# osmr/pytorchcv

Hardware: AMD Instinct MI355X
Metric: images/sec @224x224 (resnet50 bs=256/GPU) (higher is better)
Workload: dtype bf16; 1 GPU; resnet50_bs256; per_gpu_batch=256, global_batch=256, input=fp32 NCHW 224x224 resident in HBM, parallelism=batch-sharded replicas x1, launcher_choice=timed at capture on this GPU

## Files before the change

include/pcv_amd.h:

```cpp
#ifndef PCV_AMD_H
#define PCV_AMD_H

#include <stddef.h>
#include <stdint.h>

#ifdef __cplusplus
extern "C" {
#endif

#define PCV_ABI_VERSION 5

typedef struct pcv_ctx pcv_ctx;

typedef enum pcv_status {
    PCV_OK = 0,
    PCV_ERR_INVALID = -1,
    PCV_ERR_HIP = -2,
    PCV_ERR_NO_DEVICE = -3,
    PCV_ERR_TOO_LARGE = -4
} pcv_status;

typedef enum pcv_dtype { PCV_F32 = 0, PCV_BF16 = 1, PCV_F16 = 2 } pcv_dtype;

typedef enum pcv_act {
    PCV_ACT_NONE = 0, PCV_ACT_RELU = 1, PCV_ACT_RELU6 = 2, PCV_ACT_SIGMOID = 3,
    PCV_ACT_SWISH = 4, PCV_ACT_HSIGMOID = 5, PCV_ACT_HSWISH = 6
} pcv_act;

typedef struct pcv_conv_desc {
    int32_t struct_size;
    int32_t N, H, W;
    int32_t Cin, Cout;
    int32_t kh, kw;
    int32_t stride_h, stride_w;
    int32_t pad_t, pad_l, pad_b, pad_r;
    int32_t dil_h, dil_w;
    int32_t groups;
    int32_t act;
    int32_t post_act;
    int32_t has_residual;
    int32_t dtype;
    int32_t out_dtype;
    int32_t x_cpitch;
    int32_t x_wpitch;
    int32_t y_cpitch;
} pcv_conv_desc;

int pcv_abi_version(void);
size_t pcv_conv_desc_size(void);
int pcv_create(pcv_ctx** out, int device);
int pcv_destroy(pcv_ctx* ctx);
const char* pcv_last_error(const pcv_ctx* ctx);
int pcv_set_tuning(pcv_ctx* ctx, const char* key, int value);

int pcv_fp16_guard_begin(pcv_ctx* ctx, unsigned* slot, void* stream);
int pcv_fp16_guard_end(pcv_ctx* ctx, const unsigned* slot, float* y, long count, void* stream);
int pcv_fp16_overflow_count(pcv_ctx* ctx, unsigned* count, void* stream);

int pcv_nchw_to_nhwc(pcv_ctx* ctx, const float* x, void* y, int N, int C, int H, int W,
                     int cpitch, int wpitch, int dtype, void* stream);
int pcv_nhwc_to_nchw(pcv_ctx* ctx, const void* x, float* y, int N, int C, int H, int W, int cpitch, int dtype,
                     void* stream);

int pcv_preprocess_u8(pcv_ctx* ctx, const unsigned char* x, void* y, int N, int Hs, int Ws, int C, int top, int left,
                      int H, int W, int wpitch, const float* mean, const float* inv_std, int dtype, void* stream);

int pcv_resize_plan_bytes(int N, const int* hs, const int* ws, int C, int size, int H, int W, size_t* bytes);
int pcv_resize_plan(const void* const* frames, int N, const int* hs, const int* ws, int C, int size, int H, int W, void* blob,
                    size_t bytes);
int pcv_resize_crop_u8(pcv_ctx* ctx, const void* plan_host, const void* plan_dev, size_t bytes, void* y, int wpitch,
                       const float* mean, const float* inv_std, int dtype, void* stream);

int pcv_classify_f32(pcv_ctx* ctx, const float* logits, int N, int J, int k,
                     int* top_idx, float* top_val, float* top_prob,
                     const long long* labels, int* rank, float* nll,
                     void* stream);

int pcv_conv_packed_bytes(const pcv_conv_desc* d, size_t* bytes);
int pcv_conv_pack(pcv_ctx* ctx, const pcv_conv_desc* d, const float* w, void* packed, void* stream);
int pcv_dwconv_packed_bytes(const pcv_conv_desc* d, size_t* bytes);
int pcv_dwconv_pack(pcv_ctx* ctx, const pcv_conv_desc* d, const float* w, void* packed, void* stream);
int pcv_bn_fold(pcv_ctx* ctx, int C, const float* gamma, const float* beta, const float* mean, const float* var,
                float eps, const float* conv_bias, float* scale, float* shift, void* stream);

int pcv_conv2d_fused(pcv_ctx* ctx, const pcv_conv_desc* d, const void* x, const void* packed,
                     const float* scale, const float* shift, const void* residual, void* y, void* stream);

int pcv_conv2d_gated_fused(pcv_ctx* ctx, const pcv_conv_desc* d, const void* x, const void* packed, const float* scale,
                           const float* shift, const float* gate, const void* residual, void* y, void* stream);
int pcv_fc_f32(pcv_ctx* ctx, const float* in, const float* w, const float* b, float* out, int N, int K, int J, int act,
               void* stream);
int pcv_conv2d_maxpool_supported(const pcv_conv_desc* d, int k, int s, int p, int ceil_mode);
int pcv_conv2d_maxpool_fused(pcv_ctx* ctx, const pcv_conv_desc* d, const void* x, const void* packed, const float* scale,
                             const float* shift, void* y, int k, int s, int p, int ceil_mode, void* stream);

int pcv_conv2d_nchw_stem_supported(const pcv_conv_desc* d, int pool);
int pcv_conv2d_nchw_stem_fused(pcv_ctx* ctx, const pcv_conv_desc* d, const float* x_nchw, const void* packed, const float* scale,
                               const float* shift, void* y, int pool, void* stream);
int pcv_dwconv2d_fused(pcv_ctx* ctx, const pcv_conv_desc* d, const void* x, const void* packed,
                       const float* scale, const float* shift, const void* residual, void* y, void* stream);
int pcv_maxpool2d(pcv_ctx* ctx, const void* x, void* y, int N, int H, int W, int C, int k, int s, int p,
                  int ceil_mode, int dtype, void* stream);
int pcv_channel_slice(pcv_ctx* ctx, const void* x, void* y, long rows, int C, int offset, int x_cpitch, int y_cpitch,
                      int dtype, void* stream);
int pcv_channel_interleave2(pcv_ctx* ctx, const void* a, const void* b, void* y, long rows, int Ch, int a_cpitch,
                            int b_cpitch, int y_cpitch, int dtype, void* stream);
int pcv_channel_concat(pcv_ctx* ctx, const void* x, void* y, long rows, int C, int x_cpitch, int y_cpitch, int y_offset,
                       int dtype, void* stream);
int pcv_interpolate(pcv_ctx* ctx, const void* x, void* y, int N, int H, int W, int C, int Ho, int Wo, int bilinear,
                    int align_corners, int dtype, void* stream);
int pcv_avgpool2d(pcv_ctx* ctx, const void* x, void* y, int N, int H, int W, int C, int k, int s,
                  int dtype, int out_dtype, void* stream);
int pcv_global_avgpool(pcv_ctx* ctx, const void* x, void* y, int N, int HW, int C, int dtype, int out_dtype,
                       void* stream);
int pcv_gemm_bias(pcv_ctx* ctx, const void* x, const void* packed, const float* bias, void* y,
                  int N, int Cin, int Cout, int dtype, int out_dtype, void* stream);
int pcv_se_squeeze(pcv_ctx* ctx, const void* x, float* mean, int N, int HW, int C, int dtype, void* stream);
int pcv_se_excite(pcv_ctx* ctx, const float* mean, const float* w1, const float* b1, const float* w2,
                  const float* b2, float* mid, float* gate, int N, int C, int M, int mid_act, int out_act,
                  void* stream);
int pcv_se_scale(pcv_ctx* ctx, const void* x, const float* gate, const void* residual, void* y,
                 int N, int HW, int C, int post_act, int dtype, void* stream);

int pcv_splat_squeeze(pcv_ctx* ctx, const void* x, float* s, int N, int HW, int C, int radix, int dtype, void* stream);
int pcv_splat_excite(pcv_ctx* ctx, const float* s, const float* w1, const float* b1, const float* w2, const float* b2, float* mid,
                     float* logits, float* att, int N, int C, int M, int radix, int groups, void* stream);
int pcv_splat_combine(pcv_ctx* ctx, const void* x, const float* att, const void* residual, void* y, int N, int HW, int C, int radix,
                      int post_act, int dtype, void* stream);
int pcv_avgpool2d_pad(pcv_ctx* ctx, const void* x, void* y, int N, int H, int W, int C, int k, int s, int p, int ceil_mode,
                      int count_include_pad, int dtype, int out_dtype, void* stream);

int pcv_cbam_pool(pcv_ctx* ctx, const void* x, float* s, int N, int HW, int C, int dtype, void* stream);
int pcv_cbam_excite(pcv_ctx* ctx, const float* s, const float* w1, const float* b1, const float* w2, const float* b2, float* mid,
                    float* gate, int N, int C, int M, void* stream);
int pcv_cbam_spatial_pool(pcv_ctx* ctx, const void* x, const float* gate, float* p, int N, int HW, int C, int dtype, void* stream);
int pcv_cbam_apply(pcv_ctx* ctx, const void* x, const float* gate, const float* p, const float* w7, const float* scale,
                   const float* shift, const void* residual, void* y, int N, int H, int W, int C, int post_act, int dtype,
                   void* stream);

int pcv_conv1x1_pair_supported(const pcv_conv_desc* d1, const pcv_conv_desc* d2);
int pcv_conv1x1_pair_fused(pcv_ctx* ctx, const pcv_conv_desc* d1, const pcv_conv_desc* d2, const void* x,
                           const void* packed1, const float* scale1, const float* shift1, const void* residual, void* y1,
                           const void* packed2, const float* scale2, const float* shift2, void* y2, void* stream);

int pcv_conv1x1_pair_gated_supported(const pcv_conv_desc* d1, const pcv_conv_desc* d2);
int pcv_conv1x1_pair_gated_fused(pcv_ctx* ctx, const pcv_conv_desc* d1, const pcv_conv_desc* d2, const void* x,
                                 const void* packed1, const float* scale1, const float* shift1, const float* gate,
                                 const void* residual, void* y1, const void* packed2, const float* scale2, const float* shift2,
                                 void* y2, void* stream);

int pcv_conv1x1_pair_idconv_supported(const pcv_conv_desc* d_id, const pcv_conv_desc* d1, const pcv_conv_desc* d2);
int pcv_conv1x1_pair_idconv_fused(pcv_ctx* ctx, const pcv_conv_desc* d_id, const pcv_conv_desc* d1, const pcv_conv_desc* d2,
                                  const void* x0, const void* packed_id, const float* scale_id, const float* shift_id,
                                  const void* x, const void* packed1, const float* scale1, const float* shift1, void* y1,
                                  const void* packed2, const float* scale2, const float* shift2, void* y2, void* stream);

int pcv_mbconv_supported(const pcv_conv_desc* d_exp, const pcv_conv_desc* d_dw, const pcv_conv_desc* d_proj);
int pcv_mbconv_fused(pcv_ctx* ctx, const pcv_conv_desc* d_exp, const pcv_conv_desc* d_dw, const pcv_conv_desc* d_proj,
                     const void* x, const void* packed_exp, const float* scale_e, const float* shift_e,
                     const void* packed_dw, const float* scale_d, const float* shift_d, const void* packed_proj,
                     const float* scale_p, const float* shift_p, const void* residual, void* y, void* stream);

int pcv_bn_act(pcv_ctx* ctx, const void* x, const float* scale, const float* shift, void* y, long rows, int C,
               int x_cpitch, int act, int dtype, void* stream);

int pcv_rccl_available(void);
int pcv_rccl_broadcast(pcv_ctx* ctx, void* comm, void* const* bufs, const size_t* bytes, int count, int root, void* stream);
int pcv_rccl_allgather(pcv_ctx* ctx, void* comm, const void* send, void* recv, size_t bytes_per_rank, void* stream);

#ifdef __cplusplus
}
#endif
#endif
```

pytorchcv_amd/_lib.py:

```python

__all__ = ['lib', 'ctx_for', 'check', 'ConvDesc', 'LIB_PATH', 'PcvError', 'PCV_ERR_TOO_LARGE']

import os
import ctypes
import threading

LIB_PATH = os.path.join(os.path.dirname(os.path.abspath(__file__)), "csrc", "libpcv_amd.so")
PCV_ERR_TOO_LARGE = -4

_c = ctypes
_VP = ctypes.c_void_p
_I = ctypes.c_int


class PcvError(RuntimeError):
    def __init__(self, code, msg):
        super(PcvError, self).__init__("pcv_amd error {}: {}".format(code, msg))
        self.code = code


PCV_ABI_VERSION = 5


class ConvDesc(ctypes.Structure):
    _fields_ = [(n, ctypes.c_int32) for n in (
        "struct_size", "N", "H", "W", "Cin", "Cout", "kh", "kw", "stride_h", "stride_w", "pad_t", "pad_l", "pad_b", "pad_r",
        "dil_h", "dil_w", "groups", "act", "post_act", "has_residual", "dtype", "out_dtype", "x_cpitch", "x_wpitch",
        "y_cpitch")]


    def __init__(self, *args, **kw):
        super(ConvDesc, self).__init__(*args, **kw)
        self.struct_size = ctypes.sizeof(ConvDesc)


_SIGS = {
    "pcv_abi_version": (_I, []),
    "pcv_conv_desc_size": (ctypes.c_size_t, []),
    "pcv_create": (_I, [ctypes.POINTER(_VP), _I]),
    "pcv_destroy": (_I, [_VP]),
    "pcv_last_error": (ctypes.c_char_p, [_VP]),
    "pcv_set_tuning": (_I, [_VP, ctypes.c_char_p, _I]),
    "pcv_fp16_guard_begin": (_I, [_VP, _VP, _VP]),
    "pcv_fp16_guard_end": (_I, [_VP, _VP, _VP, ctypes.c_long, _VP]),
    "pcv_fp16_overflow_count": (_I, [_VP, ctypes.POINTER(ctypes.c_uint), _VP]),
    "pcv_rccl_available": (_I, []),
    "pcv_rccl_broadcast": (_I, [_VP, _VP, ctypes.POINTER(_VP), ctypes.POINTER(ctypes.c_size_t), _I, _I, _VP]),
    "pcv_rccl_allgather": (_I, [_VP, _VP, _VP, _VP, ctypes.c_size_t, _VP]),
    "pcv_nchw_to_nhwc": (_I, [_VP, _VP, _VP, _I, _I, _I, _I, _I, _I, _I, _VP]),
    "pcv_nhwc_to_nchw": (_I, [_VP, _VP, _VP, _I, _I, _I, _I, _I, _I, _VP]),
    "pcv_preprocess_u8": (_I, [_VP, _VP, _VP, _I, _I, _I, _I, _I, _I, _I, _I, _I, _VP, _VP, _I, _VP]),
    "pcv_resize_plan_bytes": (_I, [_I, ctypes.POINTER(_I), ctypes.POINTER(_I), _I, _I, _I, _I, ctypes.POINTER(ctypes.c_size_t)]),
    "pcv_resize_plan": (_I, [ctypes.POINTER(_VP), _I, ctypes.POINTER(_I), ctypes.POINTER(_I), _I, _I, _I, _I, _VP, ctypes.c_size_t]),
    "pcv_resize_crop_u8": (_I, [_VP, _VP, _VP, ctypes.c_size_t, _VP, _I, _VP, _VP, _I, _VP]),
    "pcv_classify_f32": (_I, [_VP, _VP, _I, _I, _I, _VP, _VP, _VP, _VP, _VP, _VP, _VP]),
    "pcv_conv_packed_bytes": (_I, [ctypes.POINTER(ConvDesc), ctypes.POINTER(ctypes.c_size_t)]),
    "pcv_conv_pack": (_I, [_VP, ctypes.POINTER(ConvDesc), _VP, _VP, _VP]),
    "pcv_dwconv_packed_bytes": (_I, [ctypes.POINTER(ConvDesc), ctypes.POINTER(ctypes.c_size_t)]),
    "pcv_dwconv_pack": (_I, [_VP, ctypes.POINTER(ConvDesc), _VP, _VP, _VP]),
    "pcv_bn_fold": (_I, [_VP, _I, _VP, _VP, _VP, _VP, ctypes.c_float, _VP, _VP, _VP, _VP]),
    "pcv_conv2d_fused": (_I, [_VP, ctypes.POINTER(ConvDesc), _VP, _VP, _VP, _VP, _VP, _VP, _VP]),
    "pcv_dwconv2d_fused": (_I, [_VP, ctypes.POINTER(ConvDesc), _VP, _VP, _VP, _VP, _VP, _VP, _VP]),
    "pcv_maxpool2d": (_I, [_VP, _VP, _VP, _I, _I, _I, _I, _I, _I, _I, _I, _I, _VP]),
    "pcv_channel_slice": (_I, [_VP, _VP, _VP, ctypes.c_long, _I, _I, _I, _I, _I, _VP]),
    "pcv_channel_interleave2": (_I, [_VP, _VP, _VP, _VP, ctypes.c_long, _I, _I, _I, _I, _I, _VP]),
    "pcv_channel_concat": (_I, [_VP, _VP, _VP, ctypes.c_long, _I, _I, _I, _I, _I, _VP]),
    "pcv_interpolate": (_I, [_VP, _VP, _VP, _I, _I, _I, _I, _I, _I, _I, _I, _I, _VP]),
    "pcv_avgpool2d": (_I, [_VP, _VP, _VP, _I, _I, _I, _I, _I, _I, _I, _I, _VP]),
    "pcv_global_avgpool": (_I, [_VP, _VP, _VP, _I, _I, _I, _I, _I, _VP]),
    "pcv_gemm_bias": (_I, [_VP, _VP, _VP, _VP, _VP, _I, _I, _I, _I, _I, _VP]),
    "pcv_se_squeeze": (_I, [_VP, _VP, _VP, _I, _I, _I, _I, _VP]),
    "pcv_se_excite": (_I, [_VP, _VP, _VP, _VP, _VP, _VP, _VP, _VP, _I, _I, _I, _I, _I, _VP]),
    "pcv_conv2d_gated_fused": (_I, [_VP, ctypes.POINTER(ConvDesc), _VP, _VP, _VP, _VP, _VP, _VP, _VP, _VP]),
    "pcv_fc_f32": (_I, [_VP, _VP, _VP, _VP, _VP, _I, _I, _I, _I, _VP]),
    "pcv_conv2d_maxpool_supported": (_I, [ctypes.POINTER(ConvDesc), _I, _I, _I, _I]),
    "pcv_conv2d_maxpool_fused": (_I, [_VP, ctypes.POINTER(ConvDesc), _VP, _VP, _VP, _VP, _VP, _I, _I, _I, _I, _VP]),
    "pcv_conv2d_nchw_stem_supported": (_I, [ctypes.POINTER(ConvDesc), _I]),
    "pcv_conv2d_nchw_stem_fused": (_I, [_VP, ctypes.POINTER(ConvDesc), _VP, _VP, _VP, _VP, _VP, _I, _VP]),
    "pcv_conv1x1_pair_supported": (_I, [ctypes.POINTER(ConvDesc), ctypes.POINTER(ConvDesc)]),
    "pcv_conv1x1_pair_fused": (_I, [_VP, ctypes.POINTER(ConvDesc), ctypes.POINTER(ConvDesc), _VP, _VP, _VP, _VP, _VP, _VP, _VP,
                                    _VP, _VP, _VP, _VP]),
    "pcv_conv1x1_pair_gated_supported": (_I, [ctypes.POINTER(ConvDesc), ctypes.POINTER(ConvDesc)]),
    "pcv_conv1x1_pair_gated_fused": (_I, [_VP, ctypes.POINTER(ConvDesc), ctypes.POINTER(ConvDesc), _VP, _VP, _VP, _VP, _VP, _VP, _VP,
                                          _VP, _VP, _VP, _VP, _VP]),
    "pcv_conv1x1_pair_idconv_supported": (_I, [ctypes.POINTER(ConvDesc), ctypes.POINTER(ConvDesc), ctypes.POINTER(ConvDesc)]),
    "pcv_conv1x1_pair_idconv_fused": (_I, [_VP, ctypes.POINTER(ConvDesc), ctypes.POINTER(ConvDesc), ctypes.POINTER(ConvDesc),
                                           _VP, _VP, _VP, _VP, _VP, _VP, _VP, _VP, _VP, _VP, _VP, _VP, _VP, _VP]),
    "pcv_mbconv_supported": (_I, [ctypes.POINTER(ConvDesc), ctypes.POINTER(ConvDesc), ctypes.POINTER(ConvDesc)]),
    "pcv_mbconv_fused": (_I, [_VP, ctypes.POINTER(ConvDesc), ctypes.POINTER(ConvDesc), ctypes.POINTER(ConvDesc), _VP, _VP, _VP, _VP,
                              _VP, _VP, _VP, _VP, _VP, _VP, _VP, _VP, _VP]),
    "pcv_bn_act": (_I, [_VP, _VP, _VP, _VP, _VP, ctypes.c_long, _I, _I, _I, _I, _VP]),
    "pcv_se_scale": (_I, [_VP, _VP, _VP, _VP, _VP, _I, _I, _I, _I, _I, _VP]),
    "pcv_splat_squeeze": (_I, [_VP, _VP, _VP, _I, _I, _I, _I, _I, _VP]),
    "pcv_splat_excite": (_I, [_VP, _VP, _VP, _VP, _VP, _VP, _VP, _VP, _VP, _I, _I, _I, _I, _I, _VP]),
    "pcv_splat_combine": (_I, [_VP, _VP, _VP, _VP, _VP, _I, _I, _I, _I, _I, _I, _VP]),
    "pcv_avgpool2d_pad": (_I, [_VP, _VP, _VP, _I, _I, _I, _I, _I, _I, _I, _I, _I, _I, _I, _VP]),
    "pcv_cbam_pool": (_I, [_VP, _VP, _VP, _I, _I, _I, _I, _VP]),
    "pcv_cbam_excite": (_I, [_VP, _VP, _VP, _VP, _VP, _VP, _VP, _VP, _I, _I, _I, _VP]),
    "pcv_cbam_spatial_pool": (_I, [_VP, _VP, _VP, _VP, _I, _I, _I, _I, _VP]),
    "pcv_cbam_apply": (_I, [_VP, _VP, _VP, _VP, _VP, _VP, _VP, _VP, _VP, _I, _I, _I, _I, _I, _I, _VP]),
}

_lib = None
_ctxs = {}
_lock = threading.RLock()


def lib():
    global _lib
    if _lib is None:
        with _lock:
            if _lib is None:
                if not os.path.exists(LIB_PATH):
                    raise RuntimeError(
                        "pytorchcv_amd: HIP extension {} is missing - build it with `python -c 'import __graft_entry__ as g; "
                        "g.build()'` or `make -C pytorchcv_amd/csrc`. There is no CPU fallback.".format(LIB_PATH))
                L = ctypes.CDLL(LIB_PATH)
                for name, (res, args) in _SIGS.items():
                    fn = getattr(L, name)
                    fn.restype = res
                    fn.argtypes = args
                if L.pcv_abi_version() != PCV_ABI_VERSION or L.pcv_conv_desc_size() != ctypes.sizeof(ConvDesc):
                    raise RuntimeError("pytorchcv_amd: {} has ABI version {} / a {}-byte pcv_conv_desc, this binding expects "
                                       "version {} / {} bytes - rebuild the library".format(
                                           LIB_PATH, L.pcv_abi_version(), L.pcv_conv_desc_size(), PCV_ABI_VERSION,
                                           ctypes.sizeof(ConvDesc)))
                _lib = L
    return _lib


def exported_symbols():
    return sorted(_SIGS.keys())


def ctx_for(device_index: int):
    c = _ctxs.get(device_index)
    if c is None:
        with _lock:
            c = _ctxs.get(device_index)
            if c is None:
                L = lib()
                h = _VP()
                rc = L.pcv_create(ctypes.byref(h), int(device_index))
                if rc != 0:
                    raise PcvError(rc, (L.pcv_last_error(None) or b"").decode())
                c = h
                _ctxs[device_index] = c
    return c


def check(rc: int, ctx):
    if rc != 0:
        raise PcvError(rc, (lib().pcv_last_error(ctx) or b"").decode())
```

pytorchcv_amd/csrc/pair1x1.hpp:

```cpp
#pragma once
#include "pcv_common.hpp"
#include <type_traits>
#include "igemm_conv.hpp"

struct PairParams {
    const void* x;
    const void* w1;
    const void* res;
    void* y1;
    const void* w2;
    void* y2;
    const float* scale1;
    const float* shift1;
    const float* scale2;
    const float* shift2;
    uint32_t x_bytes, res_bytes, y1_bytes, y2_bytes, w1_bytes, w2_bytes;
    int M, nTiles;
    int act1, post1, act2;
    const void* x0;
    const void* wid;
    const float* scale_id;
    const float* shift_id;
    uint32_t x0_bytes, wid_bytes;
    const float* gate;
    FastDiv div_hw;
    uint32_t* ovf;
};

template <int N> __device__ __forceinline__ void pair_wait_vmcnt() {
    asm volatile("s_waitcnt vmcnt(%0)" ::"n"(N) : "memory");
}

template <int DT, int PB, bool IDC = false, bool GATE = false>
__global__ __launch_bounds__(256, PB == 4 ? 1 : 2) void pair1x1_kernel(const PairParams p) {
#if defined(__HIP_DEVICE_COMPILE__)
    constexpr int K1 = 64, C1 = 256, C2 = 64, P = 16 * PB;
    constexpr int NXQ = PB / 2;
    constexpr int NIP = PB / 2;
    constexpr int XB = P * K1 * 2;
    typedef typename Mma<DT>::frag frag;
    extern __shared__ __attribute__((aligned(16))) char smem[];
    char* const x0ring = smem + 3 * XB;
    char* const red = smem + (IDC ? 6 : 3) * XB;

    const int tid = threadIdx.x;
    const int lane = tid & 63;
    const int wave = __builtin_amdgcn_readfirstlane(tid >> 6);
    const int fr = lane & 15, fq = lane >> 4;

    int tile = blockIdx.x;
    const int tstride = gridDim.x;
    if (tile >= p.nTiles) return;

    const __amdgpu_buffer_rsrc_t xrsrc = __builtin_amdgcn_make_buffer_rsrc(const_cast<void*>(p.x), 0, p.x_bytes, 0x00020000);
    const __amdgpu_buffer_rsrc_t rrsrc = __builtin_amdgcn_make_buffer_rsrc(const_cast<void*>(p.res), 0, p.res_bytes, 0x00020000);
    const __amdgpu_buffer_rsrc_t y1rsrc = __builtin_amdgcn_make_buffer_rsrc(p.y1, 0, p.y1_bytes, 0x00020000);
    const __amdgpu_buffer_rsrc_t y2rsrc = __builtin_amdgcn_make_buffer_rsrc(p.y2, 0, p.y2_bytes, 0x00020000);
    const __amdgpu_buffer_rsrc_t w1rsrc = __builtin_amdgcn_make_buffer_rsrc(const_cast<void*>(p.w1), 0, p.w1_bytes, 0x00020000);
    const __amdgpu_buffer_rsrc_t w2rsrc = __builtin_amdgcn_make_buffer_rsrc(const_cast<void*>(p.w2), 0, p.w2_bytes, 0x00020000);
    const __amdgpu_buffer_rsrc_t x0rsrc = __builtin_amdgcn_make_buffer_rsrc(const_cast<void*>(IDC ? p.x0 : p.x), 0, IDC ? p.x0_bytes : p.x_bytes, 0x00020000);
    const __amdgpu_buffer_rsrc_t widrsrc = __builtin_amdgcn_make_buffer_rsrc(const_cast<void*>(IDC ? p.wid : p.w1), 0, IDC ? p.wid_bytes : p.w1_bytes, 0x00020000);

    frag a1[4][2];
    frag a2[4][2];
#pragma unroll
    for (int i = 0; i < 4; ++i)
#pragma unroll
        for (int ks = 0; ks < 2; ++ks) {
            const u32x4 v1 = __builtin_amdgcn_raw_buffer_load_b128(
                w1rsrc, (uint32_t)(((64 * wave + 16 * i + fr) * K1 + ks * 32 + 8 * fq) * 2), 0, 0);
            const u32x4 v2 = __builtin_amdgcn_raw_buffer_load_b128(
                w2rsrc, (uint32_t)(((16 * i + fr) * C1 + (2 * wave + ks) * 32 + 8 * fq) * 2), 0, 0);
            a1[i][ks] = __builtin_bit_cast(frag, v1);
            a2[i][ks] = __builtin_bit_cast(frag, v2);
        }
    frag aid[IDC ? 4 : 1][2];
    if constexpr (IDC) {
#pragma unroll
        for (int i = 0; i < 4; ++i)
#pragma unroll
            for (int ks = 0; ks < 2; ++ks)
                aid[i][ks] = __builtin_bit_cast(frag, __builtin_amdgcn_raw_buffer_load_b128(
                    widrsrc, (uint32_t)(((64 * wave + 16 * i + fr) * K1 + ks * 32 + 8 * fq) * 2), 0, 0));
    }
    float sc1[2][8], sf1[2][8], sc2[NIP][8], sf2[NIP][8];
    float* const tscid = reinterpret_cast<float*>(red + 16 * 1024 * PB);
    float* const tsfid = tscid + C1;
    float* const tsc1 = tsfid + C1;
    float* const tsf1 = tsc1 + C1;
    if constexpr (IDC) {
        for (int i = tid; i < C1; i += 256) {
            tscid[i] = p.scale_id[i]; tsfid[i] = p.shift_id[i];
            tsc1[i] = p.scale1[i]; tsf1[i] = p.shift1[i];
        }
        __syncthreads();
    }
#pragma unroll
    for (int ip = 0; ip < 2; ++ip)
#pragma unroll
        for (int e = 0; e < 8; ++e) {
            const int c1 = 64 * wave + 32 * ip + 8 * fq + e;
            sc1[ip][e] = IDC ? 0.f : p.scale1[c1];
            sf1[ip][e] = IDC ? 0.f : p.shift1[c1];
        }
#pragma unroll
    for (int k = 0; k < NIP; ++k)
#pragma unroll
        for (int e = 0; e < 8; ++e) {
            const int c2 = 32 * ((wave / PB) * NIP + k) + 8 * fq + e;
            sc2[k][e] = p.scale2[c2];
            sf2[k][e] = p.shift2[c2];
        }
    const ActClamp act1 = make_act(p.act1), post1 = make_act(p.post1), act2 = make_act(p.act2);

    int xrow[NXQ], xchunk[NXQ];
#pragma unroll
    for (int q = 0; q < NXQ; ++q) {
        const int pc = NXQ * wave + q;
        xrow[q] = 8 * pc + (lane >> 3);
        xchunk[q] = (lane & 7) ^ ((xrow[q] >> 1) & 7);
    }
    auto issue_x = [&](int t, int slot) {
#pragma unroll
        for (int q = 0; q < NXQ; ++q) {
            const long pix = (long)t * P + xrow[q];
            const uint32_t off = (t < p.nTiles && pix < p.M) ? (uint32_t)((pix * K1 + xchunk[q] * 8) * 2) : 0x80000000u;
            __builtin_amdgcn_raw_ptr_buffer_load_lds(xrsrc, PCV_LDS(smem + slot * XB + (NXQ * wave + q) * 1024), 16, off, 0, 0, 0);
            if constexpr (IDC)
                __builtin_amdgcn_raw_ptr_buffer_load_lds(x0rsrc, PCV_LDS(x0ring + slot * XB + (NXQ * wave + q) * 1024), 16, off, 0, 0, 0);
        }
    };
    auto off_c1 = [&](int t, int ip, int j) -> uint32_t {
        const long pix = (long)t * P + 16 * j + fr;
        return (t < p.nTiles && pix < p.M) ? (uint32_t)((pix * C1 + 64 * wave + 32 * ip + 8 * fq) * 2) : 0x80000000u;
    };
    auto load_res = [&](int t, u32x4 (&r)[2][PB]) {
        if constexpr (IDC) return;
#pragma unroll
        for (int ip = 0; ip < 2; ++ip)
#pragma unroll
            for (int j = 0; j < PB; ++j) r[ip][j] = __builtin_amdgcn_raw_buffer_load_b128(rrsrc, off_c1(t, ip, j), 0, 0);
    };
    int xfrag[PB][2];
#pragma unroll
    for (int j = 0; j < PB; ++j)
#pragma unroll
        for (int ks = 0; ks < 2; ++ks) {
            const int row = 16 * j + fr;
            xfrag[j][ks] = row * 128 + (((4 * ks + fq) ^ ((row >> 1) & 7)) << 4);
        }

    u32x4 resr[3][2][PB];
    issue_x(tile, 0);
    issue_x(tile + tstride, 1);
    load_res(tile, resr[0]);
    load_res(tile + tstride, resr[1]);
    pair_wait_vmcnt<0>();
    bool first = true;

    F16Guard<DT> guard;
    auto step = [&](auto KC) -> bool {
        constexpr int slot = decltype(KC)::value;
        constexpr int slot2 = (slot + 2) % 3;
        u32x4 (&resc)[2][PB] = resr[slot];
        if (!first) pair_wait_vmcnt<IDC ? (7 * PB) / 2 : 5 * PB>();
        first = false;
        __syncthreads();

        if constexpr (IDC) {
            f32x4 accd[4][PB];
#pragma unroll
            for (int i = 0; i < 4; ++i)
#pragma unroll
                for (int j = 0; j < PB; ++j) accd[i][j] = (f32x4){0.f, 0.f, 0.f, 0.f};
            const char* x0b = x0ring + slot * XB;
#pragma unroll
            for (int ks = 0; ks < 2; ++ks) {
                frag b[PB];
#pragma unroll
                for (int j = 0; j < PB; ++j) b[j] = *reinterpret_cast<const frag*>(x0b + xfrag[j][ks]);
#pragma unroll
                for (int i = 0; i < 4; ++i)
#pragma unroll
                    for (int j = 0; j < PB; ++j) accd[i][j] = Mma<DT>::run(aid[i][ks], b[j], accd[i][j]);
            }
#pragma unroll
            for (int ip = 0; ip < 2; ++ip) {
                const int ch = 64 * wave + 32 * ip + 8 * fq;
                const f32x4 s0 = *reinterpret_cast<const f32x4*>(tscid + ch), s1 = *reinterpret_cast<const f32x4*>(tscid + ch + 4);
                const f32x4 h0 = *reinterpret_cast<const f32x4*>(tsfid + ch), h1 = *reinterpret_cast<const f32x4*>(tsfid + ch + 4);
#pragma unroll
                for (int j = 0; j < PB; ++j)
#pragma unroll
                    for (int e = 0; e < 2; ++e) {
                        const float a0 = accd[2 * ip][j][2 * e] * s0[2 * e] + h0[2 * e];
                        const float a1 = accd[2 * ip][j][2 * e + 1] * s0[2 * e + 1] + h0[2 * e + 1];
                        const float b0 = accd[2 * ip + 1][j][2 * e] * s1[2 * e] + h1[2 * e];
                        const float b1 = accd[2 * ip + 1][j][2 * e + 1] * s1[2 * e + 1] + h1[2 * e + 1];
                        guard.see2(a0, a1);
                        guard.see2(b0, b1);
                        resc[ip][j][e] = pack2<DT>(a0, a1);
                        resc[ip][j][2 + e] = pack2<DT>(b0, b1);
                    }
            }
        }

        f32x4 acc[4][PB];
#pragma unroll
        for (int i = 0; i < 4; ++i)
#pragma unroll
            for (int j = 0; j < PB; ++j) acc[i][j] = (f32x4){0.f, 0.f, 0.f, 0.f};
        const char* xb = smem + slot * XB;
#pragma unroll
        for (int ks = 0; ks < 2; ++ks) {
            frag b[PB];
#pragma unroll
            for (int j = 0; j < PB; ++j) b[j] = *reinterpret_cast<const frag*>(xb + xfrag[j][ks]);
#pragma unroll
            for (int i = 0; i < 4; ++i)
#pragma unroll
                for (int j = 0; j < PB; ++j) acc[i][j] = Mma<DT>::run(a1[i][ks], b[j], acc[i][j]);
        }

        issue_x(tile + 2 * tstride, slot2);
        load_res(tile + 2 * tstride, resr[slot2]);

        u32x4 o[2][PB];
#pragma unroll
        for (int ip = 0; ip < 2; ++ip)
#pragma unroll
            for (int j = 0; j < PB; ++j) {
                float v[8], r8[8];
                if constexpr (IDC) {
                    const int ch = 64 * wave + 32 * ip + 8 * fq;
                    const f32x4 s0 = *reinterpret_cast<const f32x4*>(tsc1 + ch), s1 = *reinterpret_cast<const f32x4*>(tsc1 + ch + 4);
                    const f32x4 h0 = *reinterpret_cast<const f32x4*>(tsf1 + ch), h1 = *reinterpret_cast<const f32x4*>(tsf1 + ch + 4);
#pragma unroll
                    for (int e = 0; e < 4; ++e) {
                        v[e] = acc[2 * ip][j][e] * s0[e] + h0[e];
                        v[4 + e] = acc[2 * ip + 1][j][e] * s1[e] + h1[e];
                    }
                } else {
#pragma unroll
                    for (int e = 0; e < 4; ++e) {
                        v[e] = acc[2 * ip][j][e] * sc1[ip][e] + sf1[ip][e];
                        v[4 + e] = acc[2 * ip + 1][j][e] * sc1[ip][4 + e] + sf1[ip][4 + e];
                    }
                }
                apply_act8(v, act1);
                if constexpr (GATE) {
#pragma clang fp contract(off)
                    const long pix = (long)tile * P + 16 * j + fr;
                    const uint32_t n = fastdiv((uint32_t)(pix < p.M ? pix : p.M - 1), p.div_hw);
                    const float* gp = p.gate + (size_t)n * C1 + 64 * wave + 32 * ip + 8 * fq;
                    const f32x4 g0 = *reinterpret_cast<const f32x4*>(gp), g1 = *reinterpret_cast<const f32x4*>(gp + 4);
#pragma unroll
                    for (int e = 0; e < 4; ++e) { v[e] *= g0[e]; v[4 + e] *= g1[e]; }
                }
#pragma unroll
                for (int e = 0; e < 4; ++e) unpack2<DT>(resc[ip][j][e], r8[2 * e], r8[2 * e + 1]);
#pragma unroll
                for (int e = 0; e < 8; ++e) v[e] += r8[e];
                apply_act8(v, post1);
                guard.see(v);
#pragma unroll
                for (int e = 0; e < 4; ++e) o[ip][j][e] = pack2<DT>(v[2 * e], v[2 * e + 1]);
            }
#pragma unroll
        for (int ip = 0; ip < 2; ++ip)
#pragma unroll
            for (int j = 0; j < PB; ++j) __builtin_amdgcn_raw_buffer_store_b128(o[ip][j], y1rsrc, off_c1(tile, ip, j), 0, 0);

#pragma unroll
        for (int i = 0; i < 4; ++i)
#pragma unroll
            for (int j = 0; j < PB; ++j) acc[i][j] = (f32x4){0.f, 0.f, 0.f, 0.f};
#pragma unroll
        for (int ip = 0; ip < 2; ++ip)
#pragma unroll
            for (int i = 0; i < 4; ++i)
#pragma unroll
                for (int j = 0; j < PB; ++j)
                    acc[i][j] = Mma<DT>::run(a2[i][ip], __builtin_bit_cast(frag, o[ip][j]), acc[i][j]);

#pragma unroll
        for (int i = 0; i < 4; ++i)
#pragma unroll
            for (int j = 0; j < PB; ++j)
                *reinterpret_cast<f32x4*>(red + (((wave * 4 + i) * PB + j) * 64 + lane) * 16) = acc[i][j];
        __syncthreads();
        const int jz = wave % PB, ip0 = (wave / PB) * NIP;
        f32x4 z[2 * NIP];
#pragma unroll
        for (int k = 0; k < 2 * NIP; ++k) {
            const int i = 2 * ip0 + k;
            z[k] = *reinterpret_cast<const f32x4*>(red + (((0 * 4 + i) * PB + jz) * 64 + lane) * 16);
#pragma unroll
            for (int v = 1; v < 4; ++v) {
                const f32x4 t = *reinterpret_cast<const f32x4*>(red + (((v * 4 + i) * PB + jz) * 64 + lane) * 16);
                z[k] += t;
            }
        }
        __syncthreads();

#pragma unroll
        for (int k = 0; k < NIP; ++k) {
            const int ip = ip0 + k;
            float v[8];
#pragma unroll
            for (int e = 0; e < 4; ++e) {
                v[e] = z[2 * k][e] * sc2[k][e] + sf2[k][e];
                v[4 + e] = z[2 * k + 1][e] * sc2[k][4 + e] + sf2[k][4 + e];
            }
            apply_act8(v, act2);
            guard.see(v);
            u32x4 q;
#pragma unroll
            for (int e = 0; e < 4; ++e) q[e] = pack2<DT>(v[2 * e], v[2 * e + 1]);
            const long pix = (long)tile * P + 16 * jz + fr;
            const uint32_t off = pix < p.M ? (uint32_t)((pix * C2 + 32 * ip + 8 * fq) * 2) : 0x80000000u;
            __builtin_amdgcn_raw_buffer_store_b128(q, y2rsrc, off, 0, 0);
        }
        guard.commit(p.ovf);
        tile += tstride;
        return tile < p.nTiles;
    };
    while (true) {
        if (!step(std::integral_constant<int, 0>{})) break;
        if (!step(std::integral_constant<int, 1>{})) break;
        if (!step(std::integral_constant<int, 2>{})) break;
    }
#endif
}
```

pytorchcv_amd/csrc/pcv_api.hip:

```cpp
#include <hip/hip_runtime.h>
#include <string>
#include <vector>
#include <cstring>
#include <algorithm>
#include <cstdio>
#include <cstdlib>
#include <dlfcn.h>
#include "pcv_common.hpp"
#include "igemm_inst.hpp"
#include "d3q_inst.hpp"
#include "d3w_inst.hpp"
#include "d3c_conv.hpp"
#include "d3k_conv.hpp"
#include "d3i_conv.hpp"
#include "d1i_conv.hpp"
#include "p1r_conv.hpp"
#include "stem_conv.hpp"
#include "pair1x1.hpp"
#include "wpair1x1.hpp"
#include "gconv3x3.hpp"
#include "gconv3x3r.hpp"
#include "mbconv.hpp"
#include "mbw_inst.hpp"
#include "mbr_inst.hpp"
MBW_SHAPES(MBW_DECLARE, PCV_BF16)
MBW_SHAPES(MBW_DECLARE, PCV_F16)
MBW2_SHAPES(MBW2_DECLARE, PCV_BF16)
MBW2_SHAPES(MBW2_DECLARE, PCV_F16)
MBW3_SHAPES(MBW3_DECLARE, PCV_BF16)
MBW3_SHAPES(MBW3_DECLARE, PCV_F16)
MBR_SHAPES(MBR_DECLARE, PCV_BF16)
MBR_SHAPES(MBR_DECLARE, PCV_F16)
#include "dwconv.hpp"
#include "aux_kernels.hpp"
#include "cbam_kernels.hpp"
#include "resize_kernel.hpp"
#include "classify_kernel.hpp"
#include "head_gemm.hpp"


IGEMM_INSTANCES(IGEMM_DECLARE, PCV_BF16)
IGEMM_INSTANCES(IGEMM_DECLARE, PCV_F16)
IGEMM_INSTANCES_SAMETYPE(IGEMM_DECLARE, PCV_F32)
D3Q_SHAPES(D3Q_DECLARE, PCV_BF16)
D3Q_SHAPES(D3Q_DECLARE, PCV_F16)
D3Q1_SHAPES(D3Q1_DECLARE, PCV_BF16)
D3Q1_SHAPES(D3Q1_DECLARE, PCV_F16)
D3W_SHAPES(D3W_DECLARE, PCV_BF16)
D3W_SHAPES(D3W_DECLARE, PCV_F16)
D3WT_SHAPES(D3WT_DECLARE, PCV_BF16)
D3WT_SHAPES(D3WT_DECLARE, PCV_F16)
extern template __global__ void d3c_kernel<PCV_BF16>(const D3Params);
extern template __global__ void d3c_kernel<PCV_F16>(const D3Params);
extern template __global__ void d3k_kernel<PCV_BF16>(const D3Params);
extern template __global__ void d3k_kernel<PCV_F16>(const D3Params);
extern template __global__ void d3i_kernel<PCV_BF16, 256>(const D3Params);
extern template __global__ void d3i_kernel<PCV_F16, 256>(const D3Params);
extern template __global__ void d3i_kernel<PCV_BF16, 512>(const D3Params);
extern template __global__ void d3i_kernel<PCV_F16, 512>(const D3Params);
extern template __global__ void d1i_kernel<PCV_BF16, 1024>(const D3Params);
extern template __global__ void d1i_kernel<PCV_F16, 1024>(const D3Params);
extern template __global__ void d1i_kernel<PCV_BF16, 2048>(const D3Params);
extern template __global__ void d1i_kernel<PCV_F16, 2048>(const D3Params);
#define P1R_DECLARE(CW, CIN)                                                       \
    extern template __global__ void p1r_kernel<PCV_BF16, CW, CIN>(const D3Params); \
    extern template __global__ void p1r_kernel<PCV_F16, CW, CIN>(const D3Params);
P1R_DECLARE(64, 256)
P1R_DECLARE(32, 512)
P1R_DECLARE(32, 256)

enum TileCfg { TILE_C32 = 0, TILE_C64 = 1, TILE_C128 = 2, TILE_C256 = 3, TILE_C64S = 4, TILE_C128S = 5, TILE_COUNT = 6 };

struct pcv_ctx {
    int device = 0;
    std::string err;
    int num_cu = 256;
    int persist_mode = 1;
    int force_tile = -1;
    int use_wstat = 1;
    int use_mbr = 1;
    int use_mbr_xl = 1;
    int use_mbw = 1;
    int use_gconvr = 1;
    int use_d1x1 = -1;
    int use_head = 1;
    int use_stem32 = 1;
    int use_d3x3 = -1;
    unsigned long long dbg_ptr = 0;
    int use_p1r = -1;
    int use_d3k = -1;
    int use_d3i = -1;
    int use_d1i = -1;
    int use_d3c = -1;
    int use_d3w = -1;
    int dbg_flags = 0;
    int dw_flags = 0;
    int dw_th = 0;
    int max_blocks = 0;
    int pair_pb = 2;
    int persist_max_nk = 4;
    uint32_t* ovf = nullptr;
    int igemm_bpc[3][2][TILE_COUNT][3] = {};
    int gconv_bpc[3] = {2, 2, 2};
    int stem_bpc[2] = {1, 1};
    int pair_bpc[2] = {1, 1};
    int pair_idc_bpc = 1;
    int wpair_bpc[4] = {1, 1, 1, 1};
};

static thread_local std::string g_create_err;

static int fail(pcv_ctx* ctx, int code, const std::string& msg) {
    if (ctx) ctx->err = msg; else g_create_err = msg;
    return code;
}
#define HIP_TRY(ctx, expr)                                                                          \
    do {                                                                                            \
        hipError_t e__ = (expr);                                                                    \
        if (e__ != hipSuccess)                                                                      \
            return fail(ctx, PCV_ERR_HIP, std::string(#expr) + ": " + hipGetErrorString(e__));      \
    } while (0)

struct DeviceGuard {
    int prev = -1;
    bool switched = false;
    explicit DeviceGuard(int want) {
        if (hipGetDevice(&prev) == hipSuccess && prev != want) switched = hipSetDevice(want) == hipSuccess;
    }
    ~DeviceGuard() {
        if (switched) (void)hipSetDevice(prev);
    }
};

static inline int round_up(int v, int m) { return (v + m - 1) / m * m; }
static inline long long block_slots(const pcv_ctx* ctx, int per_cu) {
    const long long n = (long long)ctx->num_cu * per_cu;
    return (ctx->max_blocks > 0 && ctx->max_blocks < n) ? ctx->max_blocks : n;
}
static inline int esize(int dt) { return dt == PCV_F32 ? 4 : 2; }
static inline bool dtype_ok(int dt) { return dt == PCV_F32 || dt == PCV_BF16 || dt == PCV_F16; }
static inline bool aligned16(const void* p) { return (reinterpret_cast<uintptr_t>(p) & 15u) == 0; }
static inline bool in_window(unsigned long long bytes) { return bytes < 0x80000000ull; }
static int too_large(pcv_ctx* ctx, const char* fn, const char* what) {
    return fail(ctx, PCV_ERR_TOO_LARGE, std::string(fn) + ": " + what + " exceeds the 2 GiB window of one launch; split the batch");
}
static const char* const kTensorTooLarge = "tensor exceeds the 2 GiB window";

struct Kernel { const void* fn; int threads, lds, BM, BP; };
template <class F> static Kernel kernel_of(F* fn, int threads, int lds, int BM = 0, int BP = 0) {
    return Kernel{reinterpret_cast<const void*>(fn), threads, lds, BM, BP};
}
template <class Params> static int launch(pcv_ctx* ctx, const Kernel& k, unsigned grid, hipStream_t stream, Params& q) {
    void* args[] = {&q};
    HIP_TRY(ctx, hipLaunchKernel(k.fn, dim3(grid), dim3((unsigned)k.threads), args, (size_t)k.lds, stream));
    return PCV_OK;
}
static int blocks_per_cu(pcv_ctx* ctx, const Kernel& k, int* nb) {
    HIP_TRY(ctx, hipOccupancyMaxActiveBlocksPerMultiprocessor(nb, k.fn, k.threads, k.lds));
    if (*nb < 1) *nb = 1;
    return PCV_OK;
}

struct ConvPlan {
    bool stem = false;
    bool conv3 = false;
    int ES = 2, CE = 8;
    bool pair = false;
    int Ho = 0, Wo = 0;
    int ngb = 1;
    int Cg_in = 0, Cg_out = 0;
    int cin_blk = 0, cout_blk = 0;
    int nR = 1, nQ = 1;
    int dy[IGEMM_MAX_TAPS], dx[IGEMM_MAX_TAPS];
    int nchunks = 0, nk = 0, Kpad = 0;
    int wrows = 0;
    size_t ktab_bytes = 0, w_bytes = 0, total_bytes = 0;
    int gconv_kt = 5;
    bool gconv = false;
    bool d3i = false;
    bool d1i = false;
    size_t d3i_off = 0;
    size_t gconv_off = 0;
    std::vector<uint32_t> ktab;
    std::vector<uint32_t> ksrc;
};

static const char* const kStaleDesc = "pcv_conv_desc.struct_size does not match this library (stale binding: compare pcv_conv_desc_size() / PCV_ABI_VERSION)";
static inline bool desc_stale(const pcv_conv_desc& d) { return d.struct_size != (int32_t)sizeof(pcv_conv_desc); }

static const char* plan_conv(const pcv_conv_desc& d, ConvPlan& P, bool tables) {
    if (desc_stale(d)) return kStaleDesc;
    if (!dtype_ok(d.dtype) || !dtype_ok(d.out_dtype)) return "unknown dtype";
    if (d.out_dtype != d.dtype && d.out_dtype != PCV_F32) return "out_dtype must equal dtype or be fp32";
    if (d.Cin <= 0 || d.Cout <= 0 || d.kh <= 0 || d.kw <= 0 || d.groups <= 0) return "non-positive conv dimension";
    constexpr int kMaxChannels = 1 << 20, kMaxExtent = 1 << 24, kMaxGeom = 1 << 12;
    if (d.Cin > kMaxChannels || d.Cout > kMaxChannels || d.groups > kMaxChannels) return "channel count out of range (> 2^20)";
    if (d.N < 0 || d.H < 0 || d.W < 0 || d.N > kMaxExtent || d.H > kMaxExtent || d.W > kMaxExtent) return "N / H / W out of range (> 2^24)";
    if (d.stride_h > kMaxGeom || d.stride_w > kMaxGeom || d.dil_h > kMaxGeom || d.dil_w > kMaxGeom) return "stride / dilation out of range";
    if (d.pad_t < 0 || d.pad_l < 0 || d.pad_b < 0 || d.pad_r < 0 || d.pad_t > kMaxGeom || d.pad_l > kMaxGeom || d.pad_b > kMaxGeom ||
        d.pad_r > kMaxGeom)
        return "padding out of range";
    if (d.x_cpitch < 0 || d.x_cpitch > 8 * kMaxChannels || d.x_wpitch < 0 || d.x_wpitch > 2 * kMaxExtent || d.y_cpitch < 0 ||
        d.y_cpitch > 8 * kMaxChannels)
        return "pitch out of range";
    if (d.kh >= IGEMM_MAX_TAPS || d.kw >= IGEMM_MAX_TAPS) return "kernel size > 15 unsupported";
    if (d.stride_h <= 0 || d.stride_w <= 0 || d.dil_h <= 0 || d.dil_w <= 0) return "non-positive stride/dilation";
    if (d.Cin % d.groups || d.Cout % d.groups) return "channels not divisible by groups";
    P.ES = esize(d.dtype);
    P.CE = 16 / P.ES;
    P.Cg_in = d.Cin / d.groups;
    P.Cg_out = d.Cout / d.groups;
    const int cpitch = d.x_cpitch > 0 ? d.x_cpitch : d.Cin;
    if (cpitch < d.Cin) return "x_cpitch < Cin";
    P.pair = (d.groups == 1 && cpitch == 4 && P.ES == 2);
    if (!P.pair && cpitch % P.CE != 0) return "x_cpitch must be a multiple of 16 bytes (or 4 for a padded 16-bit stem)";

    int gpb = 1;
    if (d.groups > 1) {
        while (gpb < d.groups && ((gpb * P.Cg_out) % 8 != 0 || (gpb * P.Cg_in) % P.CE != 0 || gpb * P.Cg_out < 32)) ++gpb;
        while (gpb < d.groups && d.groups % gpb != 0) ++gpb;
        if (d.groups % gpb != 0 || (gpb * P.Cg_out) % 8 != 0 || (gpb * P.Cg_in) % P.CE != 0)
            return "unsupported group shape (channels per group block not 16-byte aligned)";
    }
    P.ngb = d.groups / gpb;
    P.cin_blk = gpb * P.Cg_in;
    P.cout_blk = gpb * P.Cg_out;
    if (d.groups == 1) P.cin_blk = d.Cin;
    P.wrows = round_up(P.cout_blk, 32);

    P.conv3 = d.groups == 1 && d.kh == 3 && d.kw == 3 && d.stride_h == 1 && d.stride_w == 1 && d.dil_h == 1 && d.dil_w == 1 &&
              d.pad_t == 1 && d.pad_l == 1 && d.pad_b == 1 && d.pad_r == 1 && d.Cin % (8 * P.CE) == 0 && cpitch == d.Cin &&
              (d.x_wpitch <= 0 || d.x_wpitch == d.W) && d.out_dtype == d.dtype && d.Cout % 8 == 0;

    P.stem = P.pair && d.stride_h == 2 && d.stride_w == 2 && d.dil_h == 1 && d.Cout <= 64 && d.Cout % 8 == 0 && d.kh <= 7 &&
             d.kw + (d.pad_l & 1) <= 8 && d.out_dtype == d.dtype;

    if (P.pair) {
        if (d.stride_w % 2 != 0 || d.dil_w != 1) return "padded 4-channel stem needs even stride_w and dilation 1";
        const int wp = d.x_wpitch > 0 ? d.x_wpitch : d.W;
        if (wp % 2 != 0) return "padded 4-channel stem needs an even x_wpitch";
        const int dxs = -(d.pad_l & 1);
        P.nQ = (d.kw - dxs + 1) / 2;
        P.nR = d.kh;
        if (P.nQ >= IGEMM_MAX_TAPS) return "stem too wide";
        for (int r = 0; r < P.nR; ++r) P.dy[r] = r * d.dil_h;
        for (int q = 0; q < P.nQ; ++q) P.dx[q] = dxs + 2 * q;
        P.nchunks = P.nR * P.nQ;
    } else {
        P.nR = d.kh;
        P.nQ = d.kw;
        for (int r = 0; r < P.nR; ++r) P.dy[r] = r * d.dil_h;
        for (int q = 0; q < P.nQ; ++q) P.dx[q] = q * d.dil_w;
        const int cchunks = (P.cin_blk + P.CE - 1) / P.CE;
        if (d.groups == 1 && cchunks * P.CE > cpitch) return "x_cpitch too small for the channel chunks";
        P.nchunks = P.nR * P.nQ * cchunks;
    }
    for (int i = P.nR; i < IGEMM_MAX_TAPS; ++i) P.dy[i] = 0;
    for (int i = P.nQ; i < IGEMM_MAX_TAPS; ++i) P.dx[i] = 0;
    P.nk = (P.nchunks + 7) / 8;
// ... 87 lines not shown
struct TileInfo { int BM, BP, threads, lds; };
static const TileInfo kTiles[TILE_COUNT] = {
    {32, 256, 256, 2 * (32 + 256) * 128},
    {64, 256, 256, 2 * (64 + 256) * 128},
    {128, 128, 256, 2 * (128 + 128) * 128},
    {256, 64, 256, 2 * (256 + 64) * 128},
    {64, 128, 256, 2 * (64 + 128) * 128},
    {128, 64, 256, 2 * (128 + 64) * 128},
};
typedef void (*igemm_fn)(const IgemmParams);

template <int DT, int KHW> static igemm_fn igemm_for_tile(int tile) {
    switch (tile) {
        case TILE_C32: return igemm_conv_kernel<DT, DT, 2, 4, 1, 4, false, KHW>;
        case TILE_C64: return igemm_conv_kernel<DT, DT, 4, 4, 1, 4, false, KHW>;
        case TILE_C128: return igemm_conv_kernel<DT, DT, 4, 4, 2, 2, false, KHW>;
        case TILE_C256: return igemm_conv_kernel<DT, DT, 4, 4, 4, 1, false, KHW>;
        case TILE_C64S: if constexpr (KHW == 1) return igemm_conv_kernel<DT, DT, 4, 2, 1, 4, false, 1>; else return nullptr;
        case TILE_C128S: if constexpr (KHW == 1) return igemm_conv_kernel<DT, DT, 4, 2, 2, 2, false, 1>; else return nullptr;
        default: return nullptr;
    }
}
template <int DT> static igemm_fn igemm_for_taps(int tile, int khw) {
    if (khw == 1) return igemm_for_tile<DT, 1>(tile);
    if (khw == 9) return igemm_for_tile<DT, 9>(tile);
    return igemm_for_tile<DT, 0>(tile);
}
static igemm_fn igemm_fn_for(int dt, int ot, bool ragged, int tile, int khw) {
    if (!ragged && ot == dt) {
        if (dt == PCV_BF16) return igemm_for_taps<PCV_BF16>(tile, khw);
        if (dt == PCV_F16) return igemm_for_taps<PCV_F16>(tile, khw);
        return igemm_for_taps<PCV_F32>(tile, khw);
    }
    if (tile != TILE_C128) return nullptr;
    if (ot == PCV_F32) {
        if (dt == PCV_BF16) return igemm_conv_kernel<PCV_BF16, PCV_F32, 4, 4, 2, 2, true, 0>;
        if (dt == PCV_F16) return igemm_conv_kernel<PCV_F16, PCV_F32, 4, 4, 2, 2, true, 0>;
        return igemm_conv_kernel<PCV_F32, PCV_F32, 4, 4, 2, 2, true, 0>;
    }
    if (dt == PCV_BF16) return igemm_conv_kernel<PCV_BF16, PCV_BF16, 4, 4, 2, 2, true, 0>;
    if (dt == PCV_F16) return igemm_conv_kernel<PCV_F16, PCV_F16, 4, 4, 2, 2, true, 0>;
    return nullptr;
}

static Kernel igemm_kernel(int dt, int ot, bool ragged, int tile, int khw) {
    const TileInfo& T = kTiles[tile];
    return kernel_of(igemm_fn_for(dt, ot, ragged, tile, khw), T.threads, T.lds, T.BM, T.BP);
}
static inline int khw_slot(int khw) { return khw == 1 ? 1 : (khw == 9 ? 2 : 0); }

static inline int gconv_slot(int W) { return W + 1 <= 16 ? 0 : (W + 1 <= 32 ? 1 : 2); }
static Kernel gconv_kernel(int dt, int slot) {
    const bool bf = dt == PCV_BF16;
    if (slot == 0) return kernel_of(bf ? gconv3x3_kernel<PCV_BF16, 16> : gconv3x3_kernel<PCV_F16, 16>, 256, GConvCfg<16>::LDS);
    if (slot == 1) return kernel_of(bf ? gconv3x3_kernel<PCV_BF16, 32> : gconv3x3_kernel<PCV_F16, 32>, 256, GConvCfg<32>::LDS);
    return kernel_of(bf ? gconv3x3_kernel<PCV_BF16, 64> : gconv3x3_kernel<PCV_F16, 64>, 256, GConvCfg<64>::LDS);
}
static const int kGconvRMaxLds = 160 * 1024;
static Kernel gconvr_kernel(int dt, int stride, int kt, int lds = kGconvRMaxLds) {
    const bool bf = dt == PCV_BF16;
    if (stride == 2) {
        if (kt == 9) return kernel_of(bf ? gconv3x3r_kernel<PCV_BF16, 2, 9> : gconv3x3r_kernel<PCV_F16, 2, 9>, 256, lds);
        return kernel_of(bf ? gconv3x3r_kernel<PCV_BF16, 2, 5> : gconv3x3r_kernel<PCV_F16, 2, 5>, 256, lds);
    }
    return kernel_of(bf ? gconv3x3r_kernel<PCV_BF16, 1, 9> : gconv3x3r_kernel<PCV_F16, 1, 9>, 256, lds);
}
struct GConvRPlan { int R, XH, xl, win; };
static bool plan_gconvr(int stride, int H, int W, int Ho, int Wo, GConvRPlan& g) {
    if (stride == 2 && ((H | W) & 1)) return false;
    if (Wo > 64 || Ho <= 0) return false;
    for (int R = 64 / Wo; R >= 1; --R) {
        const int win = stride == 2 ? (2 * R + 1) * W + 2 : (R + 2) * W + 2;
        const int XH = stride == 2 ? ((win + 1) / 2 + 7) / 8 * 8 : 0;
        const int rows = ((stride == 2 ? 2 * XH : win) + 31) / 32 * 32;
        const int lds = 2 * rows * 128;
        if (lds * 2 <= kGconvRMaxLds || (R == 1 && lds <= kGconvRMaxLds)) {
            g.R = R; g.XH = XH; g.xl = rows / 32; g.win = win;
            return true;
        }
    }
    return false;
}
template <class Cfg, class F> static Kernel tile_kernel(F* fn, int threads) { return kernel_of(fn, threads, Cfg::LDS, Cfg::BM, Cfg::BP); }
#define D3Q_ROW(DT, WC, WP, CBW, PBW, KS)                                                                   \
    {tile_kernel<D3Cfg<WC, WP, CBW, PBW, KS>>(d3q_kernel<PCV_BF16, WC, WP, CBW, PBW, KS>, 768),             \
     tile_kernel<D3Cfg<WC, WP, CBW, PBW, KS>>(d3q_kernel<PCV_F16, WC, WP, CBW, PBW, KS>, 768)},
static const Kernel kD3[][2] = {D3Q_SHAPES(D3Q_ROW, 0)};
static const int kD3Count = (int)(sizeof(kD3) / sizeof(kD3[0]));
#define D3Q1_ROW(DT, WC, WP, CBW, PBW, KS)                                                                  \
    {tile_kernel<D3Cfg<WC, WP, CBW, PBW, KS, true>>(d3q_kernel<PCV_BF16, WC, WP, CBW, PBW, KS, true>, 768), \
     tile_kernel<D3Cfg<WC, WP, CBW, PBW, KS, true>>(d3q_kernel<PCV_F16, WC, WP, CBW, PBW, KS, true>, 768)},
static const Kernel kD1[][2] = {D3Q1_SHAPES(D3Q1_ROW, 0)};
static const int kD1Count = (int)(sizeof(kD1) / sizeof(kD1[0]));
#define D3W_ROW(DT, WC, WP, CBW, PBW, KS, NSA)                                                              \
    {tile_kernel<D3WCfg<WC, WP, CBW, PBW, KS, NSA>>(d3w_kernel<PCV_BF16, WC, WP, CBW, PBW, KS, NSA>, 512),  \
     tile_kernel<D3WCfg<WC, WP, CBW, PBW, KS, NSA>>(d3w_kernel<PCV_F16, WC, WP, CBW, PBW, KS, NSA>, 512)},
#define D3WT_ROW(DT, WC, WP, CBW, PBW, KS, NSA, TRIM)                                                                   \
    {tile_kernel<D3WCfg<WC, WP, CBW, PBW, KS, NSA, TRIM>>(d3w_kernel<PCV_BF16, WC, WP, CBW, PBW, KS, NSA, TRIM>, 512),  \
     tile_kernel<D3WCfg<WC, WP, CBW, PBW, KS, NSA, TRIM>>(d3w_kernel<PCV_F16, WC, WP, CBW, PBW, KS, NSA, TRIM>, 512)},
static const Kernel kD3W[][2] = {D3W_SHAPES(D3W_ROW, 0) D3WT_SHAPES(D3WT_ROW, 0)};
static const int kD3WCount = (int)(sizeof(kD3W) / sizeof(kD3W[0]));
static const Kernel kD3C[1][2] = {{tile_kernel<D3CCfg>(d3c_kernel<PCV_BF16>, 256), tile_kernel<D3CCfg>(d3c_kernel<PCV_F16>, 256)}};
static const Kernel kD3K[1][2] = {{tile_kernel<D3KCfg>(d3k_kernel<PCV_BF16>, 256), tile_kernel<D3KCfg>(d3k_kernel<PCV_F16>, 256)}};
#define D3I_ROW(CIN)                                                                              \
    {kernel_of(d3i_kernel<PCV_BF16, CIN>, D3ICfg::THREADS, D3ICfgT<CIN>::LDS, D3ICfg::BM),        \
     kernel_of(d3i_kernel<PCV_F16, CIN>, D3ICfg::THREADS, D3ICfgT<CIN>::LDS, D3ICfg::BM)}
static const Kernel kD3I[2][2] = {D3I_ROW(256), D3I_ROW(512)};
static const Kernel kD1I[2][2] = {
    {tile_kernel<D1ICfgT<1024>>(d1i_kernel<PCV_BF16, 1024>, 256), tile_kernel<D1ICfgT<1024>>(d1i_kernel<PCV_F16, 1024>, 256)},
    {tile_kernel<D1ICfgT<1024>>(d1i_kernel<PCV_BF16, 2048>, 256), tile_kernel<D1ICfgT<1024>>(d1i_kernel<PCV_F16, 2048>, 256)}};
#define P1R_ROW(CW, CIN) \
    {tile_kernel<P1RCfg<CW, CIN>>(p1r_kernel<PCV_BF16, CW, CIN>, 512), tile_kernel<P1RCfg<CW, CIN>>(p1r_kernel<PCV_F16, CW, CIN>, 512)}
static const Kernel kP1R[3][2] = {P1R_ROW(64, 256), P1R_ROW(32, 512), P1R_ROW(32, 256)};
static const struct { const Kernel (*rows)[2]; int n; } kD3Tables[] = {{kD3, kD3Count}, {kD1, kD1Count}, {kD3W, kD3WCount}, {kD3C, 1},
                                                                       {kD3K, 1},       {kD3I, 2},       {kD1I, 2},         {kP1R, 3}};
static int pick_d1x1(long long M, int Cout, int Cin, long long slots) {
    if (Cin < 256 || Cout < 128) return -1;
    const int shape = Cout % 256 == 0 ? 1 : 0;
    const long long tiles = (long long)((Cout + kD1[shape][0].BM - 1) / kD1[shape][0].BM) * ((M + kD1[shape][0].BP - 1) / kD1[shape][0].BP);
    return tiles * 2 >= slots ? shape : -1;
}
static int pick_d3x3(long long M, int Cout, int nk, long long slots) {
    (void)nk;
    const int wide = Cout <= 64 ? 2 : 1, narrow = Cout <= 64 ? 5 : 4;
    auto tiles = [&](int i) { return ((Cout + kD3[i][0].BM - 1) / kD3[i][0].BM) * ((M + kD3[i][0].BP - 1) / kD3[i][0].BP); };
    if (Cout % 256 == 0 && tiles(0) * 2 >= slots) return 0;
    if (tiles(wide) * 2 >= slots) return wide;
    if (tiles(narrow) * 4 >= slots) return narrow;
    return -1;
}
static int pick_d3w(long long M, int Cout, long long slots) {
    const int shape = Cout % 256 == 0 ? 1 : (Cout % 128 == 0 ? 2 : -1);
    if (shape < 0) return -1;
    const long long tiles = (long long)(Cout / kD3W[shape][0].BM) * ((M + kD3W[shape][0].BP - 1) / kD3W[shape][0].BP);
    return tiles * 4 >= slots * 3 ? shape : -1;
}

static const int kStemLds = 7 * 64 * 64 + 2 * 768 * 16 + 3 * 2 * 64 * 16;
enum StemForm { STEM_PLAIN = 0, STEM_POOLED = 1, STEM_NARROW = 2 };
#define STEM_ROWS(DT)                                                                                                          \
    {{kernel_of(stem_conv_kernel<DT, false>, 256, kStemLds), kernel_of(stem_conv_kernel<DT, true>, 256, kStemLds),             \
      kernel_of(stem_conv_kernel<DT, false, false, 2>, 256, kStemLds)},                                                        \
     {kernel_of(stem_conv_kernel<DT, false, true>, 256, kStemLds + kStemStageBytes),                                           \
      kernel_of(stem_conv_kernel<DT, true, true>, 256, kStemLds + kStemStageBytes),                                            \
      kernel_of(stem_conv_kernel<DT, false, true, 2>, 256, kStemLds + kStemStageBytes)}}
static const Kernel kStem[2][2][3] = {STEM_ROWS(PCV_BF16), STEM_ROWS(PCV_F16)};

static int pair_lds(int pb, bool idc = false) { return (idc ? 6 : 3) * 16 * pb * 64 * 2 + 16 * 1024 * pb + (idc ? 4096 : 0); }
enum PairForm { PAIR_PB4 = 0, PAIR_PB2 = 1, PAIR_GATED = 2, PAIR_IDCONV = 3 };
#define PAIR_ROW(DT)                                                                                                          \
    {kernel_of(pair1x1_kernel<DT, 4>, 256, pair_lds(4)), kernel_of(pair1x1_kernel<DT, 2>, 256, pair_lds(2)),                  \
     kernel_of(pair1x1_kernel<DT, 2, false, true>, 256, pair_lds(2)), kernel_of(pair1x1_kernel<DT, 2, true>, 256, pair_lds(2, true))}
static const Kernel kPair[2][4] = {PAIR_ROW(PCV_BF16), PAIR_ROW(PCV_F16)};
static int g_wpair_mask = 3;
static int g_mbw_wide = 1;
struct WPairLaunch { Kernel k; int tileP; bool gate_in_lds; };
template <int CM, int C1> static WPairLaunch wpair_launch_for(int dt, bool gated) {
    typedef WPairCfg<CM, C1> G;
    const bool bf = dt == PCV_BF16;
    const int lds = gated ? G::LDS_GATED : G::LDS;
    const Kernel k = gated ? kernel_of(bf ? wpair1x1_kernel<PCV_BF16, CM, C1, true> : wpair1x1_kernel<PCV_F16, CM, C1, true>, 64 * G::NW, lds)
                           : kernel_of(bf ? wpair1x1_kernel<PCV_BF16, CM, C1, false> : wpair1x1_kernel<PCV_F16, CM, C1, false>, 64 * G::NW, lds);
    return WPairLaunch{k, G::P, gated && G::GATE_LDS};
}
static WPairLaunch wpair_launch(int cfg, int dt, bool gated = false) {
    switch (cfg) {
        case 0: return wpair_launch_for<128, 512>(dt, gated);
        case 1: return wpair_launch_for<256, 1024>(dt, gated);
        case 2: return wpair_launch_for<128, 256>(dt, gated);
        default: return wpair_launch_for<256, 512>(dt, gated);
    }
}
static int wpair_cfg(int cm, int c1) {
    if (cm == 128 && c1 == 512) return 0;
    if (cm == 256 && c1 == 1024) return 1;
    if (cm == 128 && c1 == 256) return 2;
    if (cm == 256 && c1 == 512) return 3;
    return -1;
}
static bool plain_1x1(const pcv_conv_desc& d) {
    return d.kh == 1 && d.kw == 1 && d.stride_h == 1 && d.stride_w == 1 && d.pad_t == 0 && d.pad_l == 0 && d.pad_b == 0 &&
           d.pad_r == 0 && d.groups == 1 && d.dil_h == 1 && d.dil_w == 1 && d.out_dtype == d.dtype &&
           (d.x_cpitch == 0 || d.x_cpitch == d.Cin) && (d.x_wpitch == 0 || d.x_wpitch == d.W) &&
           (d.y_cpitch == 0 || d.y_cpitch == d.Cout);
}
static const char* pair_unsupported(const pcv_conv_desc& a, const pcv_conv_desc& b) {
    if (desc_stale(a) || desc_stale(b)) return kStaleDesc;
    if (!plain_1x1(a) || !plain_1x1(b)) return "both convolutions must be plain 1x1 stride 1";
    if (a.dtype != b.dtype || (a.dtype != PCV_BF16 && a.dtype != PCV_F16)) return "16-bit storage only";
    if (a.N != b.N || a.H != b.H || a.W != b.W || a.Cout != b.Cin) return "shapes do not chain";
    const bool narrow = a.Cin == 64 && a.Cout == 256 && b.Cout == 64;
    const bool wide = ((a.Cin == 128 && (g_wpair_mask & 1)) || (a.Cin == 256 && (g_wpair_mask & 2))) &&
                      wpair_cfg(a.Cin, a.Cout) >= 0 && b.Cout == a.Cin;
    if (!narrow && !wide) return "only 64 -> 256 -> 64, 128 -> 512|256 -> 128 and 256 -> 1024|512 -> 256 are instantiated";
    if (!a.has_residual || b.has_residual || b.post_act != PCV_ACT_NONE) return "first conv must carry the residual, second must not";
    if ((long)a.N * a.H * a.W * a.Cout * 2 >= (1L << 31)) return kTensorTooLarge;
    return nullptr;
}

typedef void (*mbconv_fn)(const MbParams);
template <int DT, int RT> static mbconv_fn mbconv_for(int stride, bool expand) {
    if (stride == 1) return expand ? mbconv_kernel<DT, 1, true, RT> : mbconv_kernel<DT, 1, false, RT>;
    return expand ? mbconv_kernel<DT, 2, true, RT> : mbconv_kernel<DT, 2, false, RT>;
}
static const int kMbMaxLds = 150 * 1024, kMbwMaxLds = 160 * 1024;
static Kernel mbconv_kernel(int dt, int stride, bool expand, int nrowt, int lds = kMbMaxLds) {
    if (dt == PCV_BF16) return kernel_of(nrowt <= 2 ? mbconv_for<PCV_BF16, 2>(stride, expand) : mbconv_for<PCV_BF16, 6>(stride, expand), 256, lds);
    return kernel_of(nrowt <= 2 ? mbconv_for<PCV_F16, 2>(stride, expand) : mbconv_for<PCV_F16, 6>(stride, expand), 256, lds);
}
struct MbwEntry { int dt, s, nrt, act, tw, ka, rb; mbconv_fn fn; };
#define MBW_ROW(DT, S, NRT, ACT, TW) {DT, S, NRT, ACT, TW, 1, 0, mbw_kernel<DT, S, NRT, ACT, TW>},
#define MBW2_ROW(DT, S, NRT, ACT, TW, KA) {DT, S, NRT, ACT, TW, KA, 0, mbw_kernel<DT, S, NRT, ACT, TW, KA>},
#define MBW3_ROW(DT, S, NRT, ACT, TW, KA, RB) {DT, S, NRT, ACT, TW, KA, RB, mbw_kernel<DT, S, NRT, ACT, TW, KA, RB>},
static const MbwEntry kMbw[] = {MBW_SHAPES(MBW_ROW, PCV_BF16) MBW_SHAPES(MBW_ROW, PCV_F16) MBW2_SHAPES(MBW2_ROW, PCV_BF16)
                                MBW2_SHAPES(MBW2_ROW, PCV_F16) MBW3_SHAPES(MBW3_ROW, PCV_BF16) MBW3_SHAPES(MBW3_ROW, PCV_F16)};
static const MbwEntry* pick_mbw(int dt, int stride, int nrt, int act, int tw, int ka, int rb) {
    if (act != PCV_ACT_RELU && act != PCV_ACT_RELU6) act = -1;
    for (const MbwEntry& e : kMbw)
        if (e.dt == dt && e.s == stride && e.nrt == nrt && e.act == act && e.tw == tw && e.ka == ka && e.rb == rb) return &e;
    return nullptr;
}
static Kernel mbw_kernel_of(const MbwEntry& e, int waves = 8, int lds = kMbwMaxLds) { return kernel_of(e.fn, 64 * waves, lds); }
struct MbrEntry { int dt, nrt, act, ro, s, ka; bool afl; int waves; bool wel, xl; mbconv_fn fn; };
#define MBR_ROW(DT, NRT, ACT, RO, S, KA, AFL, WV, WEL, XL) {DT, NRT, ACT, RO, S, KA, AFL, WV, WEL, XL, mbr_kernel<DT, NRT, ACT, RO, S, KA, AFL, WV, WEL, XL>},
static int mbr_entry_lds(const MbrEntry& e, int nChunks) {
    const int nr = e.s == 1 ? e.ro + 2 : 2 * e.ro + 1;
    return mbr_lds_layout(e.nrt, nChunks, e.ka, e.afl, e.wel, e.xl ? nr : 0, e.waves).total;
}
static const MbrEntry kMbr[] = {MBR_SHAPES(MBR_ROW, PCV_BF16) MBR_SHAPES(MBR_ROW, PCV_F16)};
static Kernel mbr_kernel_of(const MbrEntry& e, int lds = kMbwMaxLds) { return kernel_of(e.fn, 64 * e.waves, lds); }
static const MbrEntry* pick_mbr(const pcv_ctx* ctx, int dt, int nrt, int act, int stride, int ka, int nChunks) {
    if (act != PCV_ACT_RELU && act != PCV_ACT_RELU6) return nullptr;
    for (const MbrEntry& e : kMbr)
        if (e.dt == dt && e.nrt == nrt && e.act == act && e.s == stride && e.ka == ka &&
            mbr_entry_lds(e, nChunks) <= kMbwMaxLds && (!e.xl || ctx->use_mbr_xl))
            return &e;
    return nullptr;
}
static int mbw_waves(int stride, int nrt, int nChunks, int tw, int ka, int rb) {
    for (int nw = 8; nw >= 4; nw -= 2)
        if (mbw_lds_layout(stride, nrt, nChunks, nw, tw, ka, rb).total <= kMbwMaxLds) return nw;
    return 0;
}
static MbLds mbconv_plan(int stride, bool expand, int ka, int nChunks, int nRowT, int* nbufX) {
    MbLds two = mb_lds_layout(stride, expand, ka, nChunks, nRowT, 2);
    if (!expand || two.total <= 80 * 1024) { *nbufX = 2; return two; }
    MbLds one = mb_lds_layout(stride, expand, ka, nChunks, nRowT, 1);
    if (one.total <= 80 * 1024 || two.total > kMbMaxLds) { *nbufX = 1; return one; }
    *nbufX = 2;
    return two;
}

static Kernel classify_kernel_of(int J) {
    const int lds = kClassifyRedBytes + J * 4;
    return J <= 1024 ? kernel_of(classify_kernel<64>, 64, lds) : kernel_of(classify_kernel<256>, 256, lds);
}

static int enable_kernel(pcv_ctx* ctx, const Kernel& k, int* bpc) {
    HIP_TRY(ctx, hipFuncSetAttribute(k.fn, hipFuncAttributeMaxDynamicSharedMemorySize, k.lds));
    return bpc ? blocks_per_cu(ctx, k, bpc) : PCV_OK;
}
static int enable_kernels(pcv_ctx* ctx) {
    int rc = PCV_OK;
    auto on = [&](const Kernel& k, int* bpc = nullptr) {
        if (rc == PCV_OK && k.fn != nullptr) rc = enable_kernel(ctx, k, bpc);
    };
    auto report = [&](const Kernel& k, int dt, int tile, int khw, int variant) {
        int nb = 0;
        if (rc == PCV_OK && k.fn != nullptr && std::getenv("PCV_AMD_DEBUG") && blocks_per_cu(ctx, k, &nb) == PCV_OK)
            std::fprintf(stderr, "[pcv] igemm dt=%d tile=%d khw=%d variant=%d: %d blocks/CU\n", dt, tile, khw, variant, nb);
    };
    static const int khws[3] = {0, 1, 9};
    for (int dt = 0; dt < 3; ++dt)
        for (int tile = 0; tile < TILE_COUNT; ++tile) {
            for (int ks = 0; ks < 3; ++ks) {
                const Kernel k = igemm_kernel(dt, dt, false, tile, khws[ks]);
                on(k, &ctx->igemm_bpc[dt][0][tile][ks]);
                report(k, dt, tile, khws[ks], 0);
            }
            const Kernel f32out = igemm_kernel(dt, PCV_F32, true, tile, 0), same = igemm_kernel(dt, dt, true, tile, 0);
            on(f32out);
            report(f32out, dt, tile, 0, 1);
            on(same, &ctx->igemm_bpc[dt][1][tile][0]);
            report(same, dt, tile, 0, 2);
        }
    for (const auto& T : kD3Tables)
        for (int i = 0; i < T.n; ++i)
            for (int t = 0; t < 2; ++t) on(T.rows[i][t]);
    for (int slot = 0; slot < 3; ++slot) {
        on(gconv_kernel(PCV_BF16, slot));
        on(gconv_kernel(PCV_F16, slot), &ctx->gconv_bpc[slot]);
    }
    for (int dt = PCV_BF16; dt <= PCV_F16; ++dt)
        for (int s = 1; s <= 2; ++s)
            for (int kt = 5; kt <= 9; kt += 4) on(gconvr_kernel(dt, s, kt));
    for (int t = 0; t < 2; ++t)
        for (int nchw = 0; nchw < 2; ++nchw)
            for (int form = 0; form < 3; ++form) on(kStem[t][nchw][form], (nchw == 0 && form == STEM_PLAIN) ? &ctx->stem_bpc[t] : nullptr);
    for (int form = 0; form < 4; ++form) {
        on(kPair[0][form]);
        on(kPair[1][form], form == PAIR_GATED ? nullptr : form == PAIR_IDCONV ? &ctx->pair_idc_bpc : &ctx->pair_bpc[form]);
    }
    for (int cfg = 0; cfg < 4; ++cfg)
        for (int gated = 0; gated < 2; ++gated) {
            on(wpair_launch(cfg, PCV_BF16, gated != 0).k);
            on(wpair_launch(cfg, PCV_F16, gated != 0).k, gated ? nullptr : &ctx->wpair_bpc[cfg]);
        }
    for (int dt = PCV_BF16; dt <= PCV_F16; ++dt)
        for (int s = 1; s <= 2; ++s)
            for (int e = 0; e < 2; ++e)
                for (int rt = 2; rt <= 6; rt += 4) on(mbconv_kernel(dt, s, e != 0, rt));
    for (const MbwEntry& e : kMbw) on(mbw_kernel_of(e));
    for (const MbrEntry& e : kMbr) on(mbr_kernel_of(e));
    on(classify_kernel_of(1024));
    on(classify_kernel_of(kClassifyMaxJ));
    return rc;
}
static bool mbw_shape(int Cin, int Cout, int stride, int H, int W, int* ka_out, int* nrt_out, int* rb_out = nullptr) {
    const int ka = (Cin + 31) / 32, nrt = Cout <= 32 ? 2 : (Cout <= 64 ? 4 : 6);
    if (ka_out) *ka_out = ka;
    if (nrt_out) *nrt_out = nrt;
    if (rb_out) *rb_out = nrt == 6 ? 2 : 0;
    if (H > 250 || W > 250 || Cout > 96) return false;
    if (nrt == 6) return g_mbw_wide != 0 && stride == 1 && (ka == 2 || ka == 3);
    return ka == 1 || (ka == 2 && stride == 1 && nrt == 4);
}
static const char* mbconv_unsupported(const pcv_conv_desc* de, const pcv_conv_desc& dd, const pcv_conv_desc& dp) {
    if ((de && desc_stale(*de)) || desc_stale(dd) || desc_stale(dp)) return kStaleDesc;
    if (dd.dtype != PCV_BF16 && dd.dtype != PCV_F16) return "16-bit storage only";
    if (dd.kh != 3 || dd.kw != 3 || dd.dil_h != 1 || dd.dil_w != 1 || dd.pad_t != 1 || dd.pad_l != 1 || dd.pad_b != 1 ||
        dd.pad_r != 1 || dd.stride_h != dd.stride_w || (dd.stride_h != 1 && dd.stride_h != 2) || dd.groups != dd.Cin ||
        dd.Cin != dd.Cout || dd.has_residual || dd.out_dtype != dd.dtype || (dd.x_cpitch != 0 && dd.x_cpitch != dd.Cin) ||
        (dd.x_wpitch != 0 && dd.x_wpitch != dd.W))
        return "depthwise stage must be 3x3, pad 1, stride 1 or 2, no residual";
    const int Cmid = dd.Cin;
    if (Cmid % 8 != 0) return "expanded channels must be a multiple of 8";
    if (!plain_1x1(dp) || dp.dtype != dd.dtype || dp.Cin != Cmid || dp.Cout % 8 != 0 || dp.Cout > 96) return "project stage must be a plain 1x1 with at most 96 channels";
    const bool wave_tiles = de && mbw_shape(de->Cin, dp.Cout, dd.stride_h, dd.H, dd.W, nullptr, nullptr);
    if (dp.Cout > (wave_tiles ? 96 : 32)) return "fused unit only pays for narrow projections";
    const int Ho = (dd.H - 1) / dd.stride_h + 1, Wo = (dd.W - 1) / dd.stride_w + 1;
    if (dp.N != dd.N || dp.H != Ho || dp.W != Wo) return "shapes do not chain";
    if (Wo < (wave_tiles ? 14 : 24) || Ho < 8) return "map too small for the fused unit to pay";
    int ka = 0;
    if (de) {
        if (!plain_1x1(*de) || de->dtype != dd.dtype || de->Cout != Cmid || de->Cin % 8 != 0 || de->has_residual ||
            de->N != dd.N || de->H != dd.H || de->W != dd.W)
            return "expand stage must be a plain 1x1 onto the depthwise input";
        ka = (de->Cin + 31) / 32;
        if (ka > 3) return "expand stage input wider than 96 channels";
    }
    int nbuf = 0;
    if (wave_tiles) {
        if (mbw_waves(dd.stride_h, dp.Cout <= 32 ? 2 : (dp.Cout <= 64 ? 4 : 6), (Cmid + 31) / 32, 16, ka, dp.Cout > 64 ? 2 : 0) == 0)
            return "tiles do not fit the LDS budget";
    } else if (mbconv_plan(dd.stride_h, de != nullptr, ka, (Cmid + 31) / 32, (dp.Cout + 31) / 32 * 2, &nbuf).total > kMbMaxLds)
        return "weights + tiles do not fit the LDS budget";
    const long cin = de ? de->Cin : Cmid;
    if ((long)dd.N * dd.H * dd.W * cin * 2 >= (1L << 31) || (long)dd.N * Ho * Wo * dp.Cout * 2 >= (1L << 31)) return kTensorTooLarge;
    return nullptr;
}

template <int DT, bool FAST> static void launch_dw2(const pcv_conv_desc& d, const DwParams& p, unsigned grid, hipStream_t s) {
    if (d.kh == 3 && d.stride_h == 1) dwconv_kernel<DT, 3, 1, FAST><<<grid, 256, 0, s>>>(p);
    else if (d.kh == 3) dwconv_kernel<DT, 3, 2, FAST><<<grid, 256, 0, s>>>(p);
    else if (d.stride_h == 1) dwconv5_kernel<DT, 1, FAST><<<grid, 256, 0, s>>>(p);
    else dwconv5_kernel<DT, 2, FAST><<<grid, 256, 0, s>>>(p);
}
template <int DT> static void launch_dw(const pcv_conv_desc& d, const DwParams& p, unsigned grid, hipStream_t s) {
    if (d.act <= PCV_ACT_RELU6 && d.post_act <= PCV_ACT_RELU6) launch_dw2<DT, true>(d, p, grid, s);
    else launch_dw2<DT, false>(d, p, grid, s);
}
template <int DT> static void launch_mean(const void* x, void* y, int N, int HW, int C, int ot, hipStream_t s, int radix = 1) {
    dim3 grid((unsigned)N, (unsigned)((C / 8 + 511) / 512));
    if (ot == PCV_F32) spatial_mean_kernel<DT, PCV_F32><<<grid, 512, 0, s>>>(x, y, HW, C, radix);
    else spatial_mean_kernel<DT, DT><<<grid, 512, 0, s>>>(x, y, HW, C, radix);
}
template <int DT> static void launch_avg(const void* x, void* y, int N, int H, int W, int C, int Ho, int Wo, int k, int s,
                                         int ot, hipStream_t st, int pad = 0, int count_pad = 1, uint32_t* ovf = nullptr) {
    const long total = (long)N * Ho * Wo * (C / 8);
    const unsigned grid = (unsigned)((total + 255) / 256);
    if (ot == PCV_F32) avgpool_kernel<DT, PCV_F32><<<grid, 256, 0, st>>>(x, y, N, H, W, C, Ho, Wo, k, s, pad, count_pad, ovf);
    else avgpool_kernel<DT, DT><<<grid, 256, 0, st>>>(x, y, N, H, W, C, Ho, Wo, k, s, pad, count_pad, ovf);
}


extern "C" {

int pcv_abi_version(void) { return PCV_ABI_VERSION; }

size_t pcv_conv_desc_size(void) { return sizeof(pcv_conv_desc); }

const char* pcv_last_error(const pcv_ctx* ctx) { return ctx ? ctx->err.c_str() : g_create_err.c_str(); }

int pcv_create(pcv_ctx** out, int device) {
    if (out == nullptr) return fail(nullptr, PCV_ERR_INVALID, "pcv_create: out is NULL");
    *out = nullptr;
    int count = 0;
    if (hipGetDeviceCount(&count) != hipSuccess || count <= 0)
        return fail(nullptr, PCV_ERR_NO_DEVICE, "pcv_create: no HIP device visible");
    if (device < 0 || device >= count) return fail(nullptr, PCV_ERR_INVALID, "pcv_create: bad device index");
    hipDeviceProp_t prop;
    HIP_TRY(nullptr, hipGetDeviceProperties(&prop, device));
    if (std::strncmp(prop.gcnArchName, "gfx950", 6) != 0)
        return fail(nullptr, PCV_ERR_NO_DEVICE,
                    std::string("pcv_create: device is ") + prop.gcnArchName + ", this library is built for gfx950 only");
    int prev = 0;
    HIP_TRY(nullptr, hipGetDevice(&prev));
    HIP_TRY(nullptr, hipSetDevice(device));
    pcv_ctx* ctx = new (std::nothrow) pcv_ctx();
    if (ctx == nullptr) return fail(nullptr, PCV_ERR_INVALID, "pcv_create: out of host memory");
    ctx->device = device;
    ctx->num_cu = prop.multiProcessorCount;
    if (const char* e = std::getenv("PCV_AMD_PERSIST")) ctx->persist_mode = std::atoi(e);
    if (const char* e = std::getenv("PCV_AMD_PERSIST_NK")) ctx->persist_max_nk = std::atoi(e);
    int rc = enable_kernels(ctx);
    if (rc == PCV_OK) {
        hipError_t e = hipMalloc(reinterpret_cast<void**>(&ctx->ovf), 256);
        if (e == hipSuccess) e = hipMemset(ctx->ovf, 0, 256);
        if (e != hipSuccess) rc = fail(ctx, PCV_ERR_HIP, std::string("pcv_create: overflow counter: ") + hipGetErrorString(e));
    }
    if (rc != PCV_OK) {
        g_create_err = ctx->err;
        if (ctx->ovf) (void)hipFree(ctx->ovf);
        delete ctx;
        (void)hipSetDevice(prev);
        return rc;
    }
    (void)hipSetDevice(prev);
    *out = ctx;
    return PCV_OK;
}

static const struct { const char* key; int pcv_ctx::*field; } kTuningKeys[] = {
    {"persist", &pcv_ctx::persist_mode}, {"persist_nk", &pcv_ctx::persist_max_nk}, {"tile", &pcv_ctx::force_tile},
    {"pair_pb", &pcv_ctx::pair_pb},      {"max_blocks", &pcv_ctx::max_blocks},     {"d3x3", &pcv_ctx::use_d3x3},
    {"d3w", &pcv_ctx::use_d3w},          {"d3c", &pcv_ctx::use_d3c},               {"d3k", &pcv_ctx::use_d3k},
    {"d3i", &pcv_ctx::use_d3i},          {"d1i", &pcv_ctx::use_d1i},               {"p1r", &pcv_ctx::use_p1r},
    {"head", &pcv_ctx::use_head},        {"stem32", &pcv_ctx::use_stem32},         {"d1x1", &pcv_ctx::use_d1x1},
    {"gconvr", &pcv_ctx::use_gconvr},    {"mbw", &pcv_ctx::use_mbw},               {"mbr", &pcv_ctx::use_mbr},
    {"mbr_xl", &pcv_ctx::use_mbr_xl},    {"dw_th", &pcv_ctx::dw_th},               {"dw_flags", &pcv_ctx::dw_flags},
    {"wstat", &pcv_ctx::use_wstat},
};
int pcv_set_tuning(pcv_ctx* ctx, const char* key, int value) {
    if (!ctx || !key) return PCV_ERR_INVALID;
    const std::string k(key);
    for (const auto& t : kTuningKeys)
        if (k == t.key) {
            ctx->*t.field = value;
            return PCV_OK;
        }
    if (k == "mbw_wide") g_mbw_wide = value;
    else if (k == "wpair") g_wpair_mask = value;
    else if (k == "dbg") {
#ifdef PCV_DBG_FLAGS
        ctx->dbg_flags = value;
#else
        if (value != 0)
            return fail(ctx, PCV_ERR_INVALID, "pcv_set_tuning: \"dbg\" (timing experiments that produce wrong results) needs a -DPCV_DBG_FLAGS build");
#endif
    }
    else if (k == "dbg_lo") ctx->dbg_ptr = (ctx->dbg_ptr & 0xFFFFFFFF00000000ull) | (unsigned)value;
    else if (k == "dbg_hi") ctx->dbg_ptr = (ctx->dbg_ptr & 0xFFFFFFFFull) | ((unsigned long long)(unsigned)value << 32);
    else return fail(ctx, PCV_ERR_INVALID, "pcv_set_tuning: unknown key " + k);
    return PCV_OK;
}

int pcv_destroy(pcv_ctx* ctx) {
    if (ctx && ctx->ovf) {
        DeviceGuard device_guard(ctx->device);
        (void)hipFree(ctx->ovf);
    }
    delete ctx;
    return PCV_OK;
}

int pcv_fp16_guard_begin(pcv_ctx* ctx, unsigned* slot, void* stream) {
    if (!ctx) return PCV_ERR_INVALID;
    DeviceGuard device_guard(ctx->device);
    if (!slot) return fail(ctx, PCV_ERR_INVALID, "pcv_fp16_guard_begin: slot is NULL");
    f16_guard_begin_kernel<<<1, 1, 0, (hipStream_t)stream>>>(ctx->ovf, slot);
    HIP_TRY(ctx, hipGetLastError());
    return PCV_OK;
}

int pcv_fp16_guard_end(pcv_ctx* ctx, const unsigned* slot, float* y, long count, void* stream) {
    if (!ctx) return PCV_ERR_INVALID;
    DeviceGuard device_guard(ctx->device);
    if (!slot || !y || count <= 0) return fail(ctx, PCV_ERR_INVALID, "pcv_fp16_guard_end: bad argument");
    const unsigned grid = (unsigned)std::min<long>((count + 255) / 256, 1024);
    f16_guard_end_kernel<<<grid, 256, 0, (hipStream_t)stream>>>(ctx->ovf, slot, y, count);
    HIP_TRY(ctx, hipGetLastError());
    return PCV_OK;
}

extern "C++" {
namespace {
typedef int (*nccl_group_fn)(void);
typedef int (*nccl_bcast_fn)(const void*, void*, size_t, int, int, void*, hipStream_t);
typedef int (*nccl_gather_fn)(const void*, void*, size_t, int, void*, hipStream_t);
typedef const char* (*nccl_err_fn)(int);
struct RcclApi {
    nccl_group_fn group_start = nullptr, group_end = nullptr;
    nccl_bcast_fn broadcast = nullptr;
    nccl_gather_fn allgather = nullptr;
    nccl_err_fn error_string = nullptr;
    bool ok = false;
};
const RcclApi& rccl_api() {
    static const RcclApi api = [] {
        RcclApi a;
        void* h = dlopen("librccl.so.1", RTLD_NOW | RTLD_NOLOAD);
        if (!h) h = dlopen("librccl.so.1", RTLD_NOW);
        if (!h) h = dlopen("librccl.so", RTLD_NOW);
        if (!h) return a;
        a.group_start = reinterpret_cast<nccl_group_fn>(dlsym(h, "ncclGroupStart"));
        a.group_end = reinterpret_cast<nccl_group_fn>(dlsym(h, "ncclGroupEnd"));
        a.broadcast = reinterpret_cast<nccl_bcast_fn>(dlsym(h, "ncclBroadcast"));
        a.allgather = reinterpret_cast<nccl_gather_fn>(dlsym(h, "ncclAllGather"));
        a.error_string = reinterpret_cast<nccl_err_fn>(dlsym(h, "ncclGetErrorString"));
        a.ok = a.group_start && a.group_end && a.broadcast && a.allgather;
        return a;
    }();
    return api;
}
const int kNcclUint8 = 1;
int rccl_fail(pcv_ctx* ctx, const char* what, int rc) {
    const RcclApi& R = rccl_api();
    return fail(ctx, PCV_ERR_HIP, std::string(what) + ": " + (R.error_string ? R.error_string(rc) : "RCCL error") + " (" + std::to_string(rc) + ")");
}
}
}

int pcv_rccl_available(void) { return rccl_api().ok ? 1 : 0; }

int pcv_rccl_broadcast(pcv_ctx* ctx, void* comm, void* const* bufs, const size_t* bytes, int count, int root, void* stream) {
    if (!ctx) return PCV_ERR_INVALID;
    DeviceGuard device_guard(ctx->device);
    if (!comm || !bufs || !bytes || count <= 0 || root < 0) return fail(ctx, PCV_ERR_INVALID, "pcv_rccl_broadcast: bad argument");
    for (int i = 0; i < count; ++i)
        if (!bufs[i] || bytes[i] == 0) return fail(ctx, PCV_ERR_INVALID, "pcv_rccl_broadcast: NULL or empty buffer");
    const RcclApi& R = rccl_api();
    if (!R.ok) return fail(ctx, PCV_ERR_INVALID, "pcv_rccl_broadcast: no RCCL in this process (librccl.so.1 not found)");
    int rc = R.group_start();
    if (rc != 0) return rccl_fail(ctx, "ncclGroupStart", rc);
    for (int i = 0; i < count && rc == 0; ++i) rc = R.broadcast(bufs[i], bufs[i], bytes[i], kNcclUint8, root, comm, (hipStream_t)stream);
    const int rc_end = R.group_end();
    if (rc != 0) return rccl_fail(ctx, "ncclBroadcast", rc);
    if (rc_end != 0) return rccl_fail(ctx, "ncclGroupEnd", rc_end);
    return PCV_OK;
}

int pcv_rccl_allgather(pcv_ctx* ctx, void* comm, const void* send, void* recv, size_t bytes_per_rank, void* stream) {
    if (!ctx) return PCV_ERR_INVALID;
    DeviceGuard device_guard(ctx->device);
    if (!comm || !send || !recv || bytes_per_rank == 0) return fail(ctx, PCV_ERR_INVALID, "pcv_rccl_allgather: bad argument");
    const RcclApi& R = rccl_api();
    if (!R.ok) return fail(ctx, PCV_ERR_INVALID, "pcv_rccl_allgather: no RCCL in this process (librccl.so.1 not found)");
    const int rc = R.allgather(send, recv, bytes_per_rank, kNcclUint8, comm, (hipStream_t)stream);
    if (rc != 0) return rccl_fail(ctx, "ncclAllGather", rc);
    return PCV_OK;
}

int pcv_fp16_overflow_count(pcv_ctx* ctx, unsigned* count, void* stream) {
    if (!ctx) return PCV_ERR_INVALID;
    DeviceGuard device_guard(ctx->device);
    if (!count) return fail(ctx, PCV_ERR_INVALID, "pcv_fp16_overflow_count: count is NULL");
    HIP_TRY(ctx, hipMemcpyAsync(count, ctx->ovf, sizeof(unsigned), hipMemcpyDeviceToHost, (hipStream_t)stream));
    HIP_TRY(ctx, hipStreamSynchronize((hipStream_t)stream));
    return PCV_OK;
}

int pcv_nchw_to_nhwc(pcv_ctx* ctx, const float* x, void* y, int N, int C, int H, int W, int cpitch, int wpitch,
                     int dtype, void* stream) {
    if (!ctx) return PCV_ERR_INVALID;
    DeviceGuard device_guard(ctx->device);
    if (!x || !y || N <= 0 || C <= 0 || H <= 0 || W <= 0 || cpitch < C || wpitch < W || !dtype_ok(dtype))
        return fail(ctx, PCV_ERR_INVALID, "pcv_nchw_to_nhwc: bad argument");
    if (!(cpitch == 4 || cpitch % 8 == 0) && !(dtype == PCV_F32 && cpitch % 4 == 0))
        return fail(ctx, PCV_ERR_INVALID, "pcv_nchw_to_nhwc: cpitch must be 4 or a multiple of 8");
    const long npix = (long)N * H * wpitch;
    dim3 grid((unsigned)((npix + 255) / 256), (unsigned)((cpitch + 7) / 8));
    hipStream_t s = (hipStream_t)stream;
    if (dtype == PCV_BF16) nchw_to_nhwc_kernel<PCV_BF16><<<grid, 256, 0, s>>>(x, y, N, C, H, W, cpitch, wpitch, ctx->ovf);
    else if (dtype == PCV_F16) nchw_to_nhwc_kernel<PCV_F16><<<grid, 256, 0, s>>>(x, y, N, C, H, W, cpitch, wpitch, ctx->ovf);
    else nchw_to_nhwc_kernel<PCV_F32><<<grid, 256, 0, s>>>(x, y, N, C, H, W, cpitch, wpitch, ctx->ovf);
    HIP_TRY(ctx, hipGetLastError());
    return PCV_OK;
}

int pcv_nhwc_to_nchw(pcv_ctx* ctx, const void* x, float* y, int N, int C, int H, int W, int cpitch, int dtype, void* stream) {
    if (!ctx) return PCV_ERR_INVALID;
    DeviceGuard device_guard(ctx->device);
    if (cpitch <= 0) cpitch = C;
    if (!x || !y || N <= 0 || C <= 0 || H <= 0 || W <= 0 || cpitch < C || !dtype_ok(dtype))
        return fail(ctx, PCV_ERR_INVALID, "pcv_nhwc_to_nchw: bad argument");
    const long total = (long)N * C * H * W;
    const unsigned grid = (unsigned)((total + 255) / 256);
    hipStream_t s = (hipStream_t)stream;
    if (dtype == PCV_BF16) nhwc_to_nchw_kernel<PCV_BF16><<<grid, 256, 0, s>>>(x, y, N, C, H, W, cpitch);
    else if (dtype == PCV_F16) nhwc_to_nchw_kernel<PCV_F16><<<grid, 256, 0, s>>>(x, y, N, C, H, W, cpitch);
    else nhwc_to_nchw_kernel<PCV_F32><<<grid, 256, 0, s>>>(x, y, N, C, H, W, cpitch);
    HIP_TRY(ctx, hipGetLastError());
    return PCV_OK;
}

// ... 940 lines not shown
    if (H + 2 * p < k || W + 2 * p < k) return fail(ctx, PCV_ERR_INVALID, "pcv_avgpool2d_pad: window wider than the padded map");
    const int Ho = pool_out(H, k, s, p, ceil_mode), Wo = pool_out(W, k, s, p, ceil_mode);
    if (Ho <= 0 || Wo <= 0) return fail(ctx, PCV_ERR_INVALID, "pcv_avgpool2d_pad: empty output");
    hipStream_t st = (hipStream_t)stream;
    const int cp = count_include_pad ? 1 : 0;
    if (dtype == PCV_BF16) launch_avg<PCV_BF16>(x, y, N, H, W, C, Ho, Wo, k, s, out_dtype, st, p, cp, ctx->ovf);
    else if (dtype == PCV_F16) launch_avg<PCV_F16>(x, y, N, H, W, C, Ho, Wo, k, s, out_dtype, st, p, cp, ctx->ovf);
    else launch_avg<PCV_F32>(x, y, N, H, W, C, Ho, Wo, k, s, out_dtype, st, p, cp, ctx->ovf);
    HIP_TRY(ctx, hipGetLastError());
    return PCV_OK;
}

int pcv_conv1x1_pair_supported(const pcv_conv_desc* d1, const pcv_conv_desc* d2) {
    return (d1 && d2 && pair_unsupported(*d1, *d2) == nullptr) ? 1 : 0;
}

static int pair_impl(pcv_ctx* ctx, const pcv_conv_desc* d1, const pcv_conv_desc* d2, const void* x, const void* packed1,
                     const float* scale1, const float* shift1, const float* gate, const void* residual, void* y1,
                     const void* packed2, const float* scale2, const float* shift2, void* y2, void* stream);

int pcv_conv1x1_pair_fused(pcv_ctx* ctx, const pcv_conv_desc* d1, const pcv_conv_desc* d2, const void* x, const void* packed1,
                           const float* scale1, const float* shift1, const void* residual, void* y1, const void* packed2,
                           const float* scale2, const float* shift2, void* y2, void* stream) {
    return pair_impl(ctx, d1, d2, x, packed1, scale1, shift1, nullptr, residual, y1, packed2, scale2, shift2, y2, stream);
}

int pcv_conv1x1_pair_gated_supported(const pcv_conv_desc* d1, const pcv_conv_desc* d2) {
    if (!d1 || !d2 || pair_unsupported(*d1, *d2) != nullptr) return 0;
    const int cfg = wpair_cfg(d1->Cin, d1->Cout);
    if (cfg >= 0 && wpair_launch(cfg, d1->dtype, true).gate_in_lds && d1->H * d1->W < wpair_launch(cfg, d1->dtype, true).tileP) return 0;
    return 1;
}

int pcv_conv1x1_pair_gated_fused(pcv_ctx* ctx, const pcv_conv_desc* d1, const pcv_conv_desc* d2, const void* x,
                                 const void* packed1, const float* scale1, const float* shift1, const float* gate,
                                 const void* residual, void* y1, const void* packed2, const float* scale2, const float* shift2,
                                 void* y2, void* stream) {
    if (!ctx) return PCV_ERR_INVALID;
    if (!gate || !aligned16(gate) || !pcv_conv1x1_pair_gated_supported(d1, d2))
        return fail(ctx, PCV_ERR_INVALID, "pcv_conv1x1_pair_gated_fused: unsupported pair or missing gate");
    return pair_impl(ctx, d1, d2, x, packed1, scale1, shift1, gate, residual, y1, packed2, scale2, shift2, y2, stream);
}

static int pair_impl(pcv_ctx* ctx, const pcv_conv_desc* d1, const pcv_conv_desc* d2, const void* x, const void* packed1,
                     const float* scale1, const float* shift1, const float* gate, const void* residual, void* y1,
                     const void* packed2, const float* scale2, const float* shift2, void* y2, void* stream) {
    if (!ctx) return PCV_ERR_INVALID;
    DeviceGuard device_guard(ctx->device);
    if (!d1 || !d2 || !x || !packed1 || !scale1 || !shift1 || !residual || !y1 || !packed2 || !scale2 || !shift2 || !y2)
        return fail(ctx, PCV_ERR_INVALID, "pcv_conv1x1_pair_fused: NULL argument");
    if (const char* why = pair_unsupported(*d1, *d2)) return fail(ctx, PCV_ERR_INVALID, std::string("pcv_conv1x1_pair_fused: ") + why);
    if (!aligned16(x) || !aligned16(packed1) || !aligned16(packed2) || !aligned16(residual) || !aligned16(y1) || !aligned16(y2))
        return fail(ctx, PCV_ERR_INVALID, "pcv_conv1x1_pair_fused: pointers must be 16-byte aligned");
    ConvPlan P1, P2;
    const char* why = plan_conv(*d1, P1, false);
    if (!why) why = plan_conv(*d2, P2, false);
    if (why) return fail(ctx, PCV_ERR_INVALID, std::string("pcv_conv1x1_pair_fused: ") + why);
    const long M = (long)d1->N * d1->H * d1->W;
    hipStream_t st = (hipStream_t)stream;
    if (d1->Cin >= 128) {
        const int CM = d1->Cin, C1 = d1->Cout, cfg = wpair_cfg(CM, C1);
        if (cfg < 0 || P1.wrows != C1 || P1.Kpad != CM || P2.wrows != CM || P2.Kpad != C1 || P1.ngb != 1 || P2.ngb != 1)
            return fail(ctx, PCV_ERR_INVALID, "pcv_conv1x1_pair_fused: unexpected packed layout");
        WPairParams q;
        std::memset(&q, 0, sizeof(q));
        q.x = x; q.res = residual; q.y1 = y1; q.y2 = y2; q.ovf = ctx->ovf;
        q.w1 = static_cast<const char*>(packed1) + P1.ktab_bytes;
        q.w2 = static_cast<const char*>(packed2) + P2.ktab_bytes;
        q.scale1 = scale1; q.shift1 = shift1; q.scale2 = scale2; q.shift2 = shift2;
        q.x_bytes = q.y2_bytes = (uint32_t)(M * CM * 2); q.res_bytes = q.y1_bytes = (uint32_t)(M * C1 * 2);
        q.w1_bytes = q.w2_bytes = (uint32_t)(C1 * CM * 2);
        const WPairLaunch L = wpair_launch(cfg, d1->dtype, gate != nullptr);
        q.gate = gate;
        q.div_hw = make_fastdiv((uint32_t)(d1->H * d1->W));
        q.hw = (uint32_t)(d1->H * d1->W);
        q.M = (int)M; q.nTiles = (int)((M + L.tileP - 1) / L.tileP);
        q.act1 = d1->act; q.post1 = d1->post_act; q.act2 = d2->act;
        const unsigned grid = (unsigned)std::min<long>(q.nTiles, (long)block_slots(ctx, ctx->wpair_bpc[cfg]));
        return launch(ctx, L.k, grid, st, q);
    }
    if (P1.wrows != 256 || P1.Kpad != 64 || P2.wrows != 64 || P2.Kpad != 256 || P1.ngb != 1 || P2.ngb != 1)
        return fail(ctx, PCV_ERR_INVALID, "pcv_conv1x1_pair_fused: unexpected packed layout");
    PairParams p;
    std::memset(&p, 0, sizeof(p));
    p.x = x; p.res = residual; p.y1 = y1; p.y2 = y2; p.ovf = ctx->ovf;
    p.w1 = static_cast<const char*>(packed1) + P1.ktab_bytes;
    p.w2 = static_cast<const char*>(packed2) + P2.ktab_bytes;
    p.scale1 = scale1; p.shift1 = shift1; p.scale2 = scale2; p.shift2 = shift2;
    p.x_bytes = (uint32_t)(M * 64 * 2); p.res_bytes = p.y1_bytes = (uint32_t)(M * 256 * 2); p.y2_bytes = (uint32_t)(M * 64 * 2);
    p.w1_bytes = 256 * 64 * 2; p.w2_bytes = 64 * 256 * 2;
    const int pb = ctx->pair_pb == 4 ? 4 : 2;
    p.M = (int)M; p.nTiles = (int)((M + 16 * pb - 1) / (16 * pb));
    p.act1 = d1->act; p.post1 = d1->post_act; p.act2 = d2->act;
    p.gate = gate;
    p.div_hw = make_fastdiv((uint32_t)(d1->H * d1->W));
    const PairForm form = gate ? PAIR_GATED : (pb == 4 ? PAIR_PB4 : PAIR_PB2);
    if (gate) p.nTiles = (int)((M + 31) / 32);
    const unsigned grid = (unsigned)std::min<long>(p.nTiles, (long)block_slots(ctx, ctx->pair_bpc[form == PAIR_PB4 ? 0 : 1]));
    return launch(ctx, kPair[d1->dtype == PCV_BF16 ? 0 : 1][form], grid, st, p);
}

static const char* pair_idconv_unsupported(const pcv_conv_desc& di, const pcv_conv_desc& a, const pcv_conv_desc& b) {
    if (desc_stale(di)) return kStaleDesc;
    if (const char* why = pair_unsupported(a, b)) return why;
    if (a.Cin != 64) return "identity-convolution variant: only the 64 -> 256 -> 64 pair is instantiated";
    if (!plain_1x1(di) || di.dtype != a.dtype) return "identity convolution must be a plain 1x1 stride 1 of the same dtype";
    if (di.N != a.N || di.H != a.H || di.W != a.W || di.Cin != 64 || di.Cout != a.Cout) return "identity convolution shapes do not match";
    if (di.act != PCV_ACT_NONE || di.has_residual || di.post_act != PCV_ACT_NONE) return "identity convolution must have no activation";
    return nullptr;
}

int pcv_conv1x1_pair_idconv_supported(const pcv_conv_desc* d_id, const pcv_conv_desc* d1, const pcv_conv_desc* d2) {
    return (d_id && d1 && d2 && pair_idconv_unsupported(*d_id, *d1, *d2) == nullptr) ? 1 : 0;
}

int pcv_conv1x1_pair_idconv_fused(pcv_ctx* ctx, const pcv_conv_desc* d_id, const pcv_conv_desc* d1, const pcv_conv_desc* d2,
                                  const void* x0, const void* packed_id, const float* scale_id, const float* shift_id,
                                  const void* x, const void* packed1, const float* scale1, const float* shift1, void* y1,
                                  const void* packed2, const float* scale2, const float* shift2, void* y2, void* stream) {
    if (!ctx) return PCV_ERR_INVALID;
    DeviceGuard device_guard(ctx->device);
    if (!d_id || !d1 || !d2 || !x0 || !packed_id || !scale_id || !shift_id || !x || !packed1 || !scale1 || !shift1 || !y1 ||
        !packed2 || !scale2 || !shift2 || !y2)
        return fail(ctx, PCV_ERR_INVALID, "pcv_conv1x1_pair_idconv_fused: NULL argument");
    if (const char* why = pair_idconv_unsupported(*d_id, *d1, *d2))
        return fail(ctx, PCV_ERR_INVALID, std::string("pcv_conv1x1_pair_idconv_fused: ") + why);
    if (!aligned16(x0) || !aligned16(packed_id) || !aligned16(x) || !aligned16(packed1) || !aligned16(packed2) || !aligned16(y1) ||
        !aligned16(y2))
        return fail(ctx, PCV_ERR_INVALID, "pcv_conv1x1_pair_idconv_fused: pointers must be 16-byte aligned");
    ConvPlan Pi, P1, P2;
    const char* why = plan_conv(*d_id, Pi, false);
    if (!why) why = plan_conv(*d1, P1, false);
    if (!why) why = plan_conv(*d2, P2, false);
    if (why) return fail(ctx, PCV_ERR_INVALID, std::string("pcv_conv1x1_pair_idconv_fused: ") + why);
    if (P1.wrows != 256 || P1.Kpad != 64 || P2.wrows != 64 || P2.Kpad != 256 || Pi.wrows != 256 || Pi.Kpad != 64 || P1.ngb != 1 ||
        P2.ngb != 1 || Pi.ngb != 1)
        return fail(ctx, PCV_ERR_INVALID, "pcv_conv1x1_pair_idconv_fused: unexpected packed layout");
    PairParams p;
    std::memset(&p, 0, sizeof(p));
    const long M = (long)d1->N * d1->H * d1->W;
    p.x = x; p.res = nullptr; p.y1 = y1; p.y2 = y2; p.x0 = x0; p.ovf = ctx->ovf;
    p.w1 = static_cast<const char*>(packed1) + P1.ktab_bytes;
    p.w2 = static_cast<const char*>(packed2) + P2.ktab_bytes;
    p.wid = static_cast<const char*>(packed_id) + Pi.ktab_bytes;
    p.scale1 = scale1; p.shift1 = shift1; p.scale2 = scale2; p.shift2 = shift2; p.scale_id = scale_id; p.shift_id = shift_id;
    p.x_bytes = p.x0_bytes = (uint32_t)(M * 64 * 2); p.res_bytes = 0; p.y1_bytes = (uint32_t)(M * 256 * 2); p.y2_bytes = (uint32_t)(M * 64 * 2);
    p.w1_bytes = p.wid_bytes = 256 * 64 * 2; p.w2_bytes = 64 * 256 * 2;
    p.M = (int)M; p.nTiles = (int)((M + 31) / 32);
    p.act1 = d1->act; p.post1 = d1->post_act; p.act2 = d2->act;
    const unsigned grid = (unsigned)std::min<long>(p.nTiles, (long)block_slots(ctx, ctx->pair_idc_bpc));
    return launch(ctx, kPair[d1->dtype == PCV_BF16 ? 0 : 1][PAIR_IDCONV], grid, (hipStream_t)stream, p);
}

int pcv_channel_slice(pcv_ctx* ctx, const void* x, void* y, long rows, int C, int offset, int x_cpitch, int y_cpitch, int dtype,
                      void* stream) {
    if (!ctx) return PCV_ERR_INVALID;
    DeviceGuard device_guard(ctx->device);
    if (!x || !y || rows <= 0 || C <= 0 || offset < 0 || x_cpitch < offset + C || y_cpitch < C || y_cpitch % 8 != 0 || !dtype_ok(dtype))
        return fail(ctx, PCV_ERR_INVALID, "pcv_channel_slice: bad argument (y_cpitch must be a multiple of 8 and hold C channels)");
    const long total = rows * (y_cpitch / 8);
    const unsigned grid = (unsigned)((total + 255) / 256);
    hipStream_t st = (hipStream_t)stream;
    if (dtype == PCV_BF16) channel_slice_kernel<PCV_BF16><<<grid, 256, 0, st>>>(x, y, rows, C, offset, x_cpitch, y_cpitch);
    else if (dtype == PCV_F16) channel_slice_kernel<PCV_F16><<<grid, 256, 0, st>>>(x, y, rows, C, offset, x_cpitch, y_cpitch);
    else channel_slice_kernel<PCV_F32><<<grid, 256, 0, st>>>(x, y, rows, C, offset, x_cpitch, y_cpitch);
    HIP_TRY(ctx, hipGetLastError());
    return PCV_OK;
}

int pcv_channel_concat(pcv_ctx* ctx, const void* x, void* y, long rows, int C, int x_cpitch, int y_cpitch, int y_offset, int dtype,
                       void* stream) {
    if (!ctx) return PCV_ERR_INVALID;
    DeviceGuard device_guard(ctx->device);
    if (!x || !y || rows <= 0 || C <= 0 || C % 8 != 0 || x_cpitch < C || x_cpitch % 8 != 0 || y_offset < 0 || y_offset % 8 != 0 ||
        y_cpitch < y_offset + C || y_cpitch % 8 != 0 || !dtype_ok(dtype) || !aligned16(x) || !aligned16(y))
        return fail(ctx, PCV_ERR_INVALID, "pcv_channel_concat: bad argument (C, offset and pitches must be multiples of 8, y must hold the slice)");
    const long total = rows * (C / 8);
    const unsigned grid = (unsigned)((total + 255) / 256);
    hipStream_t st = (hipStream_t)stream;
    if (dtype == PCV_BF16) channel_concat_kernel<PCV_BF16><<<grid, 256, 0, st>>>(x, y, rows, C, x_cpitch, y_cpitch, y_offset);
    else if (dtype == PCV_F16) channel_concat_kernel<PCV_F16><<<grid, 256, 0, st>>>(x, y, rows, C, x_cpitch, y_cpitch, y_offset);
    else channel_concat_kernel<PCV_F32><<<grid, 256, 0, st>>>(x, y, rows, C, x_cpitch, y_cpitch, y_offset);
    HIP_TRY(ctx, hipGetLastError());
    return PCV_OK;
}

int pcv_interpolate(pcv_ctx* ctx, const void* x, void* y, int N, int H, int W, int C, int Ho, int Wo, int bilinear,
                    int align_corners, int dtype, void* stream) {
    if (!ctx) return PCV_ERR_INVALID;
    DeviceGuard device_guard(ctx->device);
    if (!x || !y || N <= 0 || H <= 0 || W <= 0 || C <= 0 || C % 8 != 0 || Ho <= 0 || Wo <= 0 || !dtype_ok(dtype))
        return fail(ctx, PCV_ERR_INVALID, "pcv_interpolate: bad argument (C must be a multiple of 8)");
    const long total = (long)N * Ho * Wo * (C / 8);
    const unsigned grid = (unsigned)((total + 255) / 256);
    hipStream_t st = (hipStream_t)stream;
    if (dtype == PCV_BF16) interpolate_kernel<PCV_BF16><<<grid, 256, 0, st>>>(x, y, N, H, W, C, Ho, Wo, bilinear, align_corners);
    else if (dtype == PCV_F16) interpolate_kernel<PCV_F16><<<grid, 256, 0, st>>>(x, y, N, H, W, C, Ho, Wo, bilinear, align_corners);
    else interpolate_kernel<PCV_F32><<<grid, 256, 0, st>>>(x, y, N, H, W, C, Ho, Wo, bilinear, align_corners);
    HIP_TRY(ctx, hipGetLastError());
    return PCV_OK;
}

int pcv_channel_interleave2(pcv_ctx* ctx, const void* a, const void* b, void* y, long rows, int Ch, int a_cpitch, int b_cpitch,
                            int y_cpitch, int dtype, void* stream) {
    if (!ctx) return PCV_ERR_INVALID;
    DeviceGuard device_guard(ctx->device);
    if (!a || !b || !y || rows <= 0 || Ch <= 0 || a_cpitch < Ch || b_cpitch < Ch || y_cpitch < 2 * Ch || y_cpitch % 8 != 0 ||
        !dtype_ok(dtype))
        return fail(ctx, PCV_ERR_INVALID, "pcv_channel_interleave2: bad argument (y_cpitch must be a multiple of 8 and hold 2*Ch channels)");
    const long total = rows * (y_cpitch / 8);
    const unsigned grid = (unsigned)((total + 255) / 256);
    hipStream_t st = (hipStream_t)stream;
    if (dtype == PCV_BF16) channel_interleave2_kernel<PCV_BF16><<<grid, 256, 0, st>>>(a, b, y, rows, Ch, a_cpitch, b_cpitch, y_cpitch);
    else if (dtype == PCV_F16) channel_interleave2_kernel<PCV_F16><<<grid, 256, 0, st>>>(a, b, y, rows, Ch, a_cpitch, b_cpitch, y_cpitch);
    else channel_interleave2_kernel<PCV_F32><<<grid, 256, 0, st>>>(a, b, y, rows, Ch, a_cpitch, b_cpitch, y_cpitch);
    HIP_TRY(ctx, hipGetLastError());
    return PCV_OK;
}

int pcv_preprocess_u8(pcv_ctx* ctx, const unsigned char* x, void* y, int N, int Hs, int Ws, int C, int top, int left, int H,
                      int W, int wpitch, const float* mean, const float* inv_std, int dtype, void* stream) {
    if (!ctx) return PCV_ERR_INVALID;
    DeviceGuard device_guard(ctx->device);
    if (!x || !y || !mean || !inv_std || N <= 0 || Hs <= 0 || Ws <= 0 || C <= 0 || C > 4 || H <= 0 || W <= 0 || top < 0 ||
        left < 0 || top + H > Hs || left + W > Ws || wpitch < W || !dtype_ok(dtype))
        return fail(ctx, PCV_ERR_INVALID, "pcv_preprocess_u8: bad argument (C <= 4, crop inside the frame, wpitch >= W)");
    const long total = (long)N * H * wpitch;
    const unsigned grid = (unsigned)((total + 255) / 256);
    hipStream_t st = (hipStream_t)stream;
    if (dtype == PCV_BF16) preprocess_u8_kernel<PCV_BF16><<<grid, 256, 0, st>>>(x, y, N, Hs, Ws, C, top, left, H, W, 4, wpitch, mean, inv_std, ctx->ovf);
    else if (dtype == PCV_F16) preprocess_u8_kernel<PCV_F16><<<grid, 256, 0, st>>>(x, y, N, Hs, Ws, C, top, left, H, W, 4, wpitch, mean, inv_std, ctx->ovf);
    else preprocess_u8_kernel<PCV_F32><<<grid, 256, 0, st>>>(x, y, N, Hs, Ws, C, top, left, H, W, 4, wpitch, mean, inv_std, ctx->ovf);
    HIP_TRY(ctx, hipGetLastError());
    return PCV_OK;
}

int pcv_resize_plan_bytes(int N, const int* hs, const int* ws, int C, int size, int H, int W, size_t* bytes) {
    if (!bytes) return fail(nullptr, PCV_ERR_INVALID, "pcv_resize_plan_bytes: bytes is NULL");
    *bytes = 0;
    if (const char* why = pcv_resize::plan_bytes(N, hs, ws, C, size, H, W, bytes))
        return fail(nullptr, PCV_ERR_INVALID, std::string("pcv_resize_plan_bytes: ") + why);
    return PCV_OK;
}

int pcv_resize_plan(const void* const* frames, int N, const int* hs, const int* ws, int C, int size, int H, int W, void* blob,
                    size_t bytes) {
    if (const char* why = pcv_resize::plan(frames, N, hs, ws, C, size, H, W, blob, bytes))
        return fail(nullptr, PCV_ERR_INVALID, std::string("pcv_resize_plan: ") + why);
    return PCV_OK;
}

int pcv_resize_crop_u8(pcv_ctx* ctx, const void* plan_host, const void* plan_dev, size_t bytes, void* y, int wpitch,
                       const float* mean, const float* inv_std, int dtype, void* stream) {
    if (!ctx) return PCV_ERR_INVALID;
    DeviceGuard device_guard(ctx->device);
    if (!plan_host || !plan_dev || !y || !mean || !inv_std || !dtype_ok(dtype) || !aligned16(plan_dev) || !aligned16(y))
        return fail(ctx, PCV_ERR_INVALID, "pcv_resize_crop_u8: bad argument (NULL pointer, dtype, or plan_dev / y not 16-byte aligned)");
    if (const char* why = pcv_resize::validate(plan_host, bytes)) return fail(ctx, PCV_ERR_INVALID, std::string("pcv_resize_crop_u8: ") + why);
    pcv_resize::ResizeHeader hd;
    std::memcpy(&hd, plan_host, sizeof(hd));
    if (wpitch < hd.W) return fail(ctx, PCV_ERR_INVALID, "pcv_resize_crop_u8: wpitch < W");
    if (!in_window((unsigned long long)hd.N * hd.H * wpitch * 4 * esize(dtype))) return too_large(ctx, "pcv_resize_crop_u8", "y");
    int blocks = hd.items;
    if (ctx->max_blocks > 0 && blocks > ctx->max_blocks) blocks = ctx->max_blocks;
    const char* pd = static_cast<const char*>(plan_dev);
    hipStream_t st = (hipStream_t)stream;
    const unsigned lds = (unsigned)hd.stage_bytes;
    if (dtype == PCV_BF16) resize_crop_u8_kernel<PCV_BF16><<<blocks, 256, lds, st>>>(pd, y, wpitch, mean, inv_std, ctx->ovf);
    else if (dtype == PCV_F16) resize_crop_u8_kernel<PCV_F16><<<blocks, 256, lds, st>>>(pd, y, wpitch, mean, inv_std, ctx->ovf);
    else resize_crop_u8_kernel<PCV_F32><<<blocks, 256, lds, st>>>(pd, y, wpitch, mean, inv_std, ctx->ovf);
    HIP_TRY(ctx, hipGetLastError());
    return PCV_OK;
}

int pcv_classify_f32(pcv_ctx* ctx, const float* logits, int N, int J, int k, int* top_idx, float* top_val, float* top_prob,
                     const long long* labels, int* rank, float* nll, void* stream) {
    if (!ctx) return PCV_ERR_INVALID;
    DeviceGuard device_guard(ctx->device);
    if (!logits) return fail(ctx, PCV_ERR_INVALID, "pcv_classify_f32: logits is NULL");
    if (N < 1) return fail(ctx, PCV_ERR_INVALID, "pcv_classify_f32: N = " + std::to_string(N) + " is outside the limit N >= 1");
    if (J < 1 || J > kClassifyMaxJ)
        return fail(ctx, PCV_ERR_INVALID, "pcv_classify_f32: J = " + std::to_string(J) + " is outside the limit 1 <= J <= 16384 (a row is staged in 64 KB of LDS)");
    if (k < 0 || k > std::min(J, kClassifyMaxK))
        return fail(ctx, PCV_ERR_INVALID, "pcv_classify_f32: k = " + std::to_string(k) + " is outside the limit 0 <= k <= min(J, 32) (J = " + std::to_string(J) + ")");
    if (k == 0 && (top_idx || top_val || top_prob))
        return fail(ctx, PCV_ERR_INVALID, "pcv_classify_f32: k = 0 is allowed only when top_idx, top_val and top_prob are all NULL");
    if ((rank || nll) && !labels) return fail(ctx, PCV_ERR_INVALID, "pcv_classify_f32: rank and nll need labels");
    long long blocks = N;
    if (ctx->max_blocks > 0 && blocks > ctx->max_blocks) blocks = ctx->max_blocks;
    const Kernel K = classify_kernel_of(J);
    void* args[] = {&logits, &N, &J, &k, &top_idx, &top_val, &top_prob, &labels, &rank, &nll};
    HIP_TRY(ctx, hipLaunchKernel(K.fn, dim3((unsigned)blocks), dim3((unsigned)K.threads), args, (size_t)K.lds, (hipStream_t)stream));
    return PCV_OK;
}

int pcv_mbconv_supported(const pcv_conv_desc* d_exp, const pcv_conv_desc* d_dw, const pcv_conv_desc* d_proj) {
    return (d_dw && d_proj && mbconv_unsupported(d_exp, *d_dw, *d_proj) == nullptr) ? 1 : 0;
}

int pcv_mbconv_fused(pcv_ctx* ctx, const pcv_conv_desc* d_exp, const pcv_conv_desc* d_dw, const pcv_conv_desc* d_proj,
                     const void* x, const void* packed_exp, const float* scale_e, const float* shift_e, const void* packed_dw,
                     const float* scale_d, const float* shift_d, const void* packed_proj, const float* scale_p,
                     const float* shift_p, const void* residual, void* y, void* stream) {
    if (!ctx) return PCV_ERR_INVALID;
    DeviceGuard device_guard(ctx->device);
    if (!d_dw || !d_proj || !x || !packed_dw || !scale_d || !shift_d || !packed_proj || !scale_p || !shift_p || !y ||
// ... 105 lines not shown
```

pytorchcv_amd/engine.py:

```python

__all__ = ['NHWC', 'DTYPES', 'default_dtype', 'set_compute_dtype', 'compute_dtype_of', 'Fp16Guard', 'fp16_overflow_count', 'from_nchw', 'to_nchw', 'ConvRunner',
           'BnActRunner', 'maxpool2d', 'avgpool2d', 'avgpool2d_pad', 'global_avgpool', 'se_forward', 'splat_forward', 'cbam_forward', 'channel_slice', 'cat_shuffle2', 'act_code',
           'boundary', 'round8', 'channel_concat_into', 'interpolate', 'add', 'classify']

import os
import ctypes
import torch
import torch.nn as nn
import torch.nn.functional as F
from . import _lib
from ._lib import ConvDesc

DTYPES = {"fp32": (0, torch.float32), "bf16": (1, torch.bfloat16), "fp16": (2, torch.float16)}
_CODE_OF_TORCH = {torch.float32: 0, torch.bfloat16: 1, torch.float16: 2}
_NAME_OF_TORCH = {torch.float32: "fp32", torch.bfloat16: "bf16", torch.float16: "fp16"}


def default_dtype() -> str:
    d = os.environ.get("PCV_AMD_DTYPE", "auto")
    if d not in DTYPES and d != "auto":
        raise ValueError("PCV_AMD_DTYPE must be one of {}".format(sorted(DTYPES) + ["auto"]))
    return d


def set_compute_dtype(net: nn.Module, dtype: str) -> nn.Module:
    if dtype not in DTYPES and dtype != "auto":
        raise ValueError("dtype must be one of {}".format(sorted(DTYPES) + ["auto"]))
    for m in net.modules():
        m._pcv_dtype = dtype
    return net


def stamp_family_dtype(net: nn.Module) -> nn.Module:
    mode = getattr(net, "pcv_16bit", None)
    if mode is not None:
        for m in net.modules():
            if m is not net:
                m.pcv_16bit = mode
    return net


def compute_dtype_of(module: nn.Module) -> str:
    d = getattr(module, "_pcv_dtype", None) or default_dtype()
    if d == "auto":
        d = getattr(module, "pcv_16bit", None) or "bf16"
    return d


class Fp16Guard(object):
    __slots__ = ("slot", "device")

    def __init__(self, device, torch_dtype):
        self.slot = None
        self.device = device
        if torch_dtype == torch.float16:
            self.slot = torch.empty(1, dtype=torch.int32, device=device)
            ctx = _ctx(device)
            _lib.check(_lib.lib().pcv_fp16_guard_begin(ctx, _ptr(self.slot), _stream(device)), ctx)

    def finish(self, y: torch.Tensor) -> torch.Tensor:
        if self.slot is not None:
            if y.dtype != torch.float32 or not y.is_contiguous():
                raise RuntimeError("the fp16 guard poisons a contiguous fp32 result")
            ctx = _ctx(self.device)
            _lib.check(_lib.lib().pcv_fp16_guard_end(ctx, _ptr(self.slot), _ptr(y), y.numel(), _stream(self.device)), ctx)
        return y


def fp16_overflow_count(device) -> int:
    ctx = _ctx(device)
    n = ctypes.c_uint(0)
    _lib.check(_lib.lib().pcv_fp16_overflow_count(ctx, ctypes.byref(n), _stream(device)), ctx)
    return int(n.value)


def round8(c: int) -> int:
    return (int(c) + 7) // 8 * 8


class NHWC(object):
    __slots__ = ("t", "N", "H", "W", "C", "wpitch", "cpitch")

    def __init__(self, t, N, H, W, C, wpitch=None, cpitch=None):
        self.t, self.N, self.H, self.W, self.C = t, N, H, W, C
        self.wpitch = W if wpitch is None else wpitch
        self.cpitch = C if cpitch is None else cpitch

    @property
    def dtype(self):
        return self.t.dtype

    @property
    def device(self):
        return self.t.device

    @property
    def dense(self) -> bool:
        return self.wpitch == self.W and self.cpitch == round8(self.C)

    def size(self, dim=None):
        s = (self.N, self.C, self.H, self.W)
        return s if dim is None else s[dim]


class _ShapeOnly(object):
    __slots__ = ("N", "H", "W", "C", "dtype", "wpitch", "cpitch")

    def __init__(self, N, H, W, C, dtype):
        self.N, self.H, self.W, self.C, self.dtype, self.wpitch, self.cpitch = N, H, W, C, dtype, W, round8(C)


def _stream(device) -> ctypes.c_void_p:
    return ctypes.c_void_p(torch.cuda.current_stream(device).cuda_stream)


def _ctx(device):
    if device.type != "cuda":
        raise RuntimeError("pytorchcv_amd runs on MI355X (gfx950) only: got a tensor on '{}'. Move the model and the input "
                           "to a CUDA/HIP device; there is no CPU path in this package.".format(device))
    idx = device.index if device.index is not None else torch.cuda.current_device()
    return _lib.ctx_for(idx)


def _ptr(t):
    return ctypes.c_void_p(t.data_ptr()) if t is not None else None


class LazyNCHW(NHWC):
    __slots__ = ("src", "_conv", "_dtype_name")

    def __init__(self, x: torch.Tensor, dtype: str):
        N, C, H, W = x.shape
        self.src, self._conv, self._dtype_name = x, None, dtype
        self.N, self.H, self.W, self.C = N, H, W, C
        self.wpitch, self.cpitch = (W + 1) // 2 * 2, 4

    @property
    def t(self):
        if self._conv is None:
            self._conv = from_nchw(self.src, self._dtype_name, stem=True).t
        return self._conv

    @property
    def materialized(self) -> bool:
        return self._conv is not None

    @property
    def dtype(self):
        return DTYPES[self._dtype_name][1]

    @property
    def device(self):
        return self.src.device


def network_input(x: torch.Tensor, dtype: str) -> NHWC:
    if x.dim() != 4:
        raise ValueError("expected a 4-D NCHW tensor")
    if x.shape[1] <= 3 and x.shape[3] % 4 == 0 and STEM_FROM_NCHW:
        return LazyNCHW(x.contiguous().float(), dtype)
    return from_nchw(x, dtype, stem=True)


def from_nchw(x: torch.Tensor, dtype: str, stem: bool = True) -> NHWC:
    if x.dim() != 4:
        raise ValueError("expected a 4-D NCHW tensor")
    x = x.contiguous().float()
    N, C, H, W = x.shape
    code, tdt = DTYPES[dtype]
    if C <= 4 and stem:
        cp, wp = 4, (W + 1) // 2 * 2
    else:
        cp, wp = (C + 7) // 8 * 8, W
    y = torch.empty((N, H, wp, cp), dtype=tdt, device=x.device)
    ctx = _ctx(x.device)
    _lib.check(_lib.lib().pcv_nchw_to_nhwc(ctx, _ptr(x), _ptr(y), N, C, H, W, cp, wp, code, _stream(x.device)), ctx)
    return NHWC(y, N, H, W, C, wpitch=wp, cpitch=cp)


def to_nchw(a: NHWC) -> torch.Tensor:
    if a.wpitch != a.W:
        raise RuntimeError("cannot convert a row-padded input handle back to NCHW")
    y = torch.empty((a.N, a.C, a.H, a.W), dtype=torch.float32, device=a.device)
    ctx = _ctx(a.device)
    _lib.check(_lib.lib().pcv_nhwc_to_nchw(ctx, _ptr(a.t), _ptr(y), a.N, a.C, a.H, a.W, a.cpitch, _CODE_OF_TORCH[a.dtype],
                                           _stream(a.device)), ctx)
    return y


def boundary(module: nn.Module, x, fn, stem: bool = False):
    if isinstance(x, NHWC):
        return fn(x)
    if not torch.is_tensor(x):
        raise TypeError("expected a torch.Tensor or an NHWC handle")
    dtype = compute_dtype_of(module)
    guard = Fp16Guard(x.device, DTYPES[dtype][1])
    y = fn(from_nchw(x, dtype, stem=stem))
    if isinstance(y, tuple):
        return tuple(guard.finish(to_nchw(v)) if isinstance(v, NHWC) else v for v in y)
    y = to_nchw(y) if isinstance(y, NHWC) else y
    return guard.finish(y) if torch.is_tensor(y) and y.dtype == torch.float32 else y


def act_code(activ) -> int:
    from .models.common.activ import Swish, HSigmoid, HSwish
    if activ is None:
        return 0
    if isinstance(activ, nn.ReLU):
        return 1
    if isinstance(activ, nn.ReLU6):
        return 2
    if isinstance(activ, nn.Sigmoid):
        return 3
    if isinstance(activ, Swish):
        return 4
    if isinstance(activ, HSigmoid):
        return 5
    if isinstance(activ, HSwish):
        return 6
    raise NotImplementedError("activation {} has no fused MI355X epilogue yet".format(type(activ).__name__))


def _pair(v):
    return (int(v[0]), int(v[1])) if isinstance(v, (tuple, list)) else (int(v), int(v))


class ConvRunner(object):
    def __init__(self, conv: nn.Conv2d, bn, pad4=None):
        self.conv, self.bn, self.pad4 = conv, bn, pad4
        self._key = None
        self._foreign = False
        self.packed = self.scale = self.shift = None
        self.depthwise = (conv.groups > 1 and conv.groups == conv.in_channels == conv.out_channels)
        if 1 < conv.groups and not self.depthwise and (conv.in_channels % 8 or conv.out_channels % 8):
            raise NotImplementedError("grouped convolution with channel counts that are not multiples of 8")

    def _phys(self, x_cpitch: int, out_fp32: bool):
        c = self.conv
        cin = c.in_channels if x_cpitch == 4 and c.in_channels <= 4 else round8(c.in_channels)
        cout = c.out_channels if out_fp32 else round8(c.out_channels)
        groups = cin if self.depthwise else c.groups
        return cin, cout, groups

    def _sources(self):
        ts = [self.conv.weight, self.conv.bias]
        if self.bn is not None:
            ts += [self.bn.weight, self.bn.bias, self.bn.running_mean, self.bn.running_var]
        return ts

    def _state_key(self, dtype, cpitch, d: ConvDesc):
        return (dtype, cpitch, d.Cin, d.Cout, d.groups, d.out_dtype, d.pad_l & 1) + \
            tuple((t.data_ptr(), t._version) if t is not None else None for t in self._sources())

    def desc(self, x: NHWC, act, post_act, has_res, out_code=None, logits=False, pad4=None) -> ConvDesc:
        c = self.conv
        kh, kw = _pair(c.kernel_size)
        sh, sw = _pair(c.stride)
        dh, dw = _pair(c.dilation)
        pad4 = pad4 if pad4 is not None else self.pad4
        if pad4 is not None:
            pl, pr, pt, pb = [int(v) for v in pad4]
        else:
# ... 34 lines not shown
                {f[0]: getattr(d, f[0]) for f in d._fields_}))
        packed = torch.empty((nbytes.value + 15) // 16 * 16, dtype=torch.uint8, device=dev)
        w32 = w.detach().float()
        if w32.dim() == 2:
            w32 = w32[:, :, None, None]
        C, Cl = d.Cout, self.conv.out_channels
        cin_g = d.Cin // d.groups
        if w32.shape[0] != C or w32.shape[1] != cin_g:
            w32 = F.pad(w32, (0, 0, 0, 0, 0, cin_g - w32.shape[1], 0, C - w32.shape[0]))
        w32 = w32.contiguous()
        fn_pack = L.pcv_dwconv_pack if self.depthwise else L.pcv_conv_pack
        _lib.check(fn_pack(ctx, ctypes.byref(d), _ptr(w32), _ptr(packed), st), ctx)

        def padded(t, fill):
            t = t.detach().float()
            return (F.pad(t, (0, C - Cl), value=fill) if C != Cl else t).contiguous()
        scale = torch.empty(C, dtype=torch.float32, device=dev)
        shift = torch.empty(C, dtype=torch.float32, device=dev)
        bias = padded(self.conv.bias, 0.0) if self.conv.bias is not None else None
        if self.bn is not None:
            if not isinstance(self.bn, nn.BatchNorm2d):
                raise NotImplementedError("only BatchNorm2d folds into the conv epilogue, got {}".format(type(self.bn).__name__))
            g = padded(self.bn.weight, 0.0) if self.bn.weight is not None else padded(torch.ones(Cl, device=dev), 0.0)
            b = padded(self.bn.bias, 0.0) if self.bn.bias is not None else torch.zeros(C, device=dev)
            m = padded(self.bn.running_mean, 0.0)
            v = padded(self.bn.running_var, 1.0)
            _lib.check(L.pcv_bn_fold(ctx, C, _ptr(g), _ptr(b), _ptr(m), _ptr(v), ctypes.c_float(self.bn.eps), _ptr(bias),
                                     _ptr(scale), _ptr(shift), st), ctx)
        else:
            _lib.check(L.pcv_bn_fold(ctx, C, None, None, None, None, ctypes.c_float(0.0), _ptr(bias), _ptr(scale),
                                     _ptr(shift), st), ctx)
        torch.cuda.current_stream(dev).synchronize()
        self.packed, self.scale, self.shift, self._key = packed, scale, shift, key

    def adopt_foreign_state(self):
        self._foreign = True
        self._sq_key = None

    def local_state_restored(self):
        self._foreign = False
        self._key = None

    def run(self, x: NHWC, act=0, residual: NHWC | None = None, post_act=0, out_fp32=False, pad4=None, out=None, gate=None) -> NHWC:
        if self.bn is not None and self.bn.training:
            raise RuntimeError("pytorchcv_amd is an inference path: call net.eval() first (BatchNorm is folded)")
        if isinstance(x, LazyNCHW) and not x.materialized and residual is None and out is None and gate is None and not out_fp32 \
                and post_act == 0 and pad4 is None:
            y = self._stem_from_nchw(x, act, pool=False)
            if y is not None:
                return y
        d = self.desc(x, act, post_act, residual is not None, out_code=0 if out_fp32 else None, logits=out_fp32, pad4=pad4)
        self.prepare(x, d)
        return self._launch(x, d, residual, out, gate)

    def _stem_from_nchw(self, x: "LazyNCHW", act: int, pool: bool):
        if self.depthwise or self.pad4 is not None or x.src.numel() * 4 >= (1 << 31):
            return None
        d = self.desc(x, act, 0, False)
        L, ctx = _lib.lib(), _ctx(x.device)
        if not L.pcv_conv2d_nchw_stem_supported(ctypes.byref(d), 1 if pool else 0):
            return None
        self.prepare(x, d)
        Ho = (x.H + d.pad_t + d.pad_b - d.dil_h * (d.kh - 1) - 1) // d.stride_h + 1
        Wo = (x.W + d.pad_l + d.pad_r - d.dil_w * (d.kw - 1) - 1) // d.stride_w + 1
        if pool:
            Ho, Wo = (Ho + 2 - 3) // 2 + 1, (Wo + 2 - 3) // 2 + 1
        if Ho <= 0 or Wo <= 0:
            return None
        y = torch.empty((x.N, Ho, Wo, d.Cout), dtype=x.dtype, device=x.device)
        _lib.check(L.pcv_conv2d_nchw_stem_fused(ctx, ctypes.byref(d), _ptr(x.src), _ptr(self.packed), _ptr(self.scale), _ptr(self.shift),
                                                _ptr(y), 1 if pool else 0, _stream(x.device)), ctx)
        return NHWC(y, x.N, Ho, Wo, self.conv.out_channels, cpitch=d.Cout)

    def run_maxpool(self, x: NHWC, act: int, k: int, s: int, p: int, ceil_mode: bool = False):
        if not FUSE_UNITS or self.depthwise or self.pad4 is not None:
            return None
        if self.bn is not None and self.bn.training:
            raise RuntimeError("pytorchcv_amd is an inference path: call net.eval() first (BatchNorm is folded)")
        if isinstance(x, LazyNCHW) and not x.materialized and (k, s, p) == (3, 2, 1) and not ceil_mode:
            y = self._stem_from_nchw(x, act, pool=True)
            if y is not None:
                return y
        d = self.desc(x, act, 0, False)
        L, ctx = _lib.lib(), _ctx(x.device)
        if not L.pcv_conv2d_maxpool_supported(ctypes.byref(d), k, s, p, 1 if ceil_mode else 0):
            return None
        self.prepare(x, d)
        Ho = (x.H + d.pad_t + d.pad_b - d.dil_h * (d.kh - 1) - 1) // d.stride_h + 1
        Wo = (x.W + d.pad_l + d.pad_r - d.dil_w * (d.kw - 1) - 1) // d.stride_w + 1
        Hq, Wq = (Ho + 2 * p - k) // s + 1, (Wo + 2 * p - k) // s + 1
        if Hq <= 0 or Wq <= 0:
            return None
        y = torch.empty((x.N, Hq, Wq, d.Cout), dtype=x.dtype, device=x.device)
        _lib.check(L.pcv_conv2d_maxpool_fused(ctx, ctypes.byref(d), _ptr(x.t), _ptr(self.packed), _ptr(self.scale), _ptr(self.shift),
                                              _ptr(y), k, s, p, 1 if ceil_mode else 0, _stream(x.device)), ctx)
        return NHWC(y, x.N, Hq, Wq, self.conv.out_channels, cpitch=d.Cout)

    def run_pair(self, x: NHWC, residual: NHWC, act: int, post_act: int, nxt: "ConvRunner", nxt_act: int, gate=None):
        if not FUSE_UNITS or residual is None or self.depthwise or nxt.depthwise or self.pad4 is not None or nxt.pad4 is not None:
            return None
        if (self.bn is not None and self.bn.training) or (nxt.bn is not None and nxt.bn.training):
            raise RuntimeError("pytorchcv_amd is an inference path: call net.eval() first (BatchNorm is folded)")
        c = self.conv
        L, ctx, st = _lib.lib(), _ctx(x.device), _stream(x.device)
        d1 = self.desc(x, act, post_act, True)
        d2 = nxt.desc(_ShapeOnly(x.N, x.H, x.W, c.out_channels, x.dtype), nxt_act, 0, False)
        supported = L.pcv_conv1x1_pair_gated_supported if gate is not None else L.pcv_conv1x1_pair_supported
        if not supported(ctypes.byref(d1), ctypes.byref(d2)):
            return None
        if not residual.dense or residual.dtype != x.dtype or tuple(residual.t.shape) != (x.N, x.H, x.W, d1.Cout):
            raise RuntimeError("residual shape/dtype mismatch")
        if gate is not None and (gate.dtype != torch.float32 or tuple(gate.shape) != (x.N, d1.Cout) or not gate.is_contiguous()):
            raise RuntimeError("gate must be a contiguous fp32 [N, {}] tensor".format(d1.Cout))
        t1 = torch.empty((x.N, x.H, x.W, d1.Cout), dtype=x.dtype, device=x.device)
        t2 = torch.empty((x.N, x.H, x.W, d2.Cout), dtype=x.dtype, device=x.device)
        y1 = NHWC(t1, x.N, x.H, x.W, c.out_channels, cpitch=d1.Cout)
        self.prepare(x, d1)
        nxt.prepare(y1, d2)
        if gate is not None:
            _lib.check(L.pcv_conv1x1_pair_gated_fused(ctx, ctypes.byref(d1), ctypes.byref(d2), _ptr(x.t), _ptr(self.packed),
                                                      _ptr(self.scale), _ptr(self.shift), _ptr(gate), _ptr(residual.t), _ptr(t1),
                                                      _ptr(nxt.packed), _ptr(nxt.scale), _ptr(nxt.shift), _ptr(t2), st), ctx)
        else:
            _lib.check(L.pcv_conv1x1_pair_fused(ctx, ctypes.byref(d1), ctypes.byref(d2), _ptr(x.t), _ptr(self.packed),
                                                _ptr(self.scale), _ptr(self.shift), _ptr(residual.t), _ptr(t1), _ptr(nxt.packed),
                                                _ptr(nxt.scale), _ptr(nxt.shift), _ptr(t2), st), ctx)
        return y1, NHWC(t2, x.N, x.H, x.W, nxt.conv.out_channels, cpitch=d2.Cout)

    def run_pair_idconv(self, x: NHWC, x0: NHWC, idr: "ConvRunner", act: int, post_act: int, nxt: "ConvRunner", nxt_act: int):
        if not FUSE_UNITS or any(r.depthwise or r.pad4 is not None for r in (self, idr, nxt)):
            return None
        if any(r.bn is not None and r.bn.training for r in (self, idr, nxt)):
            raise RuntimeError("pytorchcv_amd is an inference path: call net.eval() first (BatchNorm is folded)")
        if not x0.dense or x0.dtype != x.dtype or (x0.N, x0.H, x0.W) != (x.N, x.H, x.W):
            return None
        c = self.conv
        L, ctx, st = _lib.lib(), _ctx(x.device), _stream(x.device)
        di = idr.desc(x0, 0, 0, False)
        d1 = self.desc(x, act, post_act, True)
        d2 = nxt.desc(_ShapeOnly(x.N, x.H, x.W, c.out_channels, x.dtype), nxt_act, 0, False)
        if not L.pcv_conv1x1_pair_idconv_supported(ctypes.byref(di), ctypes.byref(d1), ctypes.byref(d2)):
            return None
        t1 = torch.empty((x.N, x.H, x.W, d1.Cout), dtype=x.dtype, device=x.device)
        t2 = torch.empty((x.N, x.H, x.W, d2.Cout), dtype=x.dtype, device=x.device)
        y1 = NHWC(t1, x.N, x.H, x.W, c.out_channels, cpitch=d1.Cout)
        idr.prepare(x0, di)
        self.prepare(x, d1)
        nxt.prepare(y1, d2)
        _lib.check(L.pcv_conv1x1_pair_idconv_fused(ctx, ctypes.byref(di), ctypes.byref(d1), ctypes.byref(d2), _ptr(x0.t),
                                                   _ptr(idr.packed), _ptr(idr.scale), _ptr(idr.shift), _ptr(x.t), _ptr(self.packed),
                                                   _ptr(self.scale), _ptr(self.shift), _ptr(t1), _ptr(nxt.packed), _ptr(nxt.scale),
                                                   _ptr(nxt.shift), _ptr(t2), st), ctx)
        return y1, NHWC(t2, x.N, x.H, x.W, nxt.conv.out_channels, cpitch=d2.Cout)

    def _launch(self, x: NHWC, d: ConvDesc, residual, out=None, gate=None):
        c = self.conv
        kh, kw = d.kh, d.kw
        Ho = (x.H + d.pad_t + d.pad_b - d.dil_h * (kh - 1) - 1) // d.stride_h + 1
        Wo = (x.W + d.pad_l + d.pad_r - d.dil_w * (kw - 1) - 1) // d.stride_w + 1
        if Ho <= 0 or Wo <= 0:
            raise RuntimeError("convolution output would be empty")
        out_dt = torch.float32 if d.out_dtype == 0 else x.dtype
        if out is not None:
            buf, coff = out
            if self.depthwise or tuple(buf.shape[:3]) != (x.N, Ho, Wo) or buf.dtype != out_dt or not buf.is_contiguous() or \
                    coff % 8 != 0 or c.out_channels % 8 != 0 or coff + c.out_channels > buf.shape[3] or buf.device != x.device:
                raise RuntimeError("bad concatenation slice for a convolution output (channel counts must be multiples of 8)")
            d.y_cpitch = int(buf.shape[3])
            y = buf[:, :, :, coff:]
        else:
            y = torch.empty((x.N, Ho, Wo, d.Cout), dtype=out_dt, device=x.device)
        if residual is not None:
            if not residual.dense or tuple(residual.t.shape) != (x.N, Ho, Wo, d.Cout) or residual.dtype != x.dtype:
                raise RuntimeError("residual shape/dtype mismatch: {} vs {}".format(
                    tuple(residual.t.shape), (x.N, Ho, Wo, d.Cout)))
        if gate is not None:
            if self.depthwise or gate.dtype != torch.float32 or tuple(gate.shape) != (x.N, d.Cout) or not gate.is_contiguous():
                raise RuntimeError("gate must be a contiguous fp32 [N, {}] tensor of a dense convolution".format(d.Cout))
        self._launch_range(x, d, residual, y, 0, x.N, gate)
        return None if out is not None else NHWC(y, x.N, Ho, Wo, c.out_channels, cpitch=d.Cout)

    def _launch_range(self, x, d, residual, y, n0, n1, gate=None):
        L, ctx, st = _lib.lib(), _ctx(x.device), _stream(x.device)
        d.N = n1 - n0
        rp = _ptr(residual.t[n0:n1]) if residual is not None else None
        if gate is not None:
            rc = L.pcv_conv2d_gated_fused(ctx, ctypes.byref(d), _ptr(x.t[n0:n1]), _ptr(self.packed), _ptr(self.scale),
                                          _ptr(self.shift), _ptr(gate[n0:n1]), rp, _ptr(y[n0:n1]), st)
        else:
            fn = L.pcv_dwconv2d_fused if self.depthwise else L.pcv_conv2d_fused
            rc = fn(ctx, ctypes.byref(d), _ptr(x.t[n0:n1]), _ptr(self.packed), _ptr(self.scale), _ptr(self.shift), rp, _ptr(y[n0:n1]), st)
        if rc == _lib.PCV_ERR_TOO_LARGE and n1 - n0 > 1:
            mid = (n0 + n1) // 2
            self._launch_range(x, d, residual, y, n0, mid, gate)
            self._launch_range(x, d, residual, y, mid, n1, gate)
            return
        _lib.check(rc, ctx)

    def squeezed_excite(self, z: NHWC, w1, b1, w2, b2, mid_act: int, out_act: int) -> torch.Tensor:
        c = self.conv
        if self.depthwise or c.groups != 1 or tuple(_pair(c.kernel_size)) != (1, 1) or tuple(_pair(c.stride)) != (1, 1) or \
                self.pad4 is not None or tuple(_pair(c.padding)) != (0, 0):
            raise RuntimeError("squeezed_excite needs a plain 1x1 stride-1 convolution")
        d = self.desc(z, 0, 0, False)
        self.prepare(z, d)
        key = ("sq", self._key) + tuple((t.data_ptr(), t._version) for t in (w1, w2, b1, b2))
        if getattr(self, "_sq_key", None) != key:
            Cl, CP = c.out_channels, d.Cout
            w = c.weight.detach().float().reshape(Cl, -1)
            w = F.pad(w, (0, d.Cin - w.shape[1], 0, CP - Cl)) * self.scale[:, None]
            w1p = F.pad(w1.float(), (0, CP - Cl))
            self._sq_w1 = (w1p @ w).contiguous()
            self._sq_b1 = (w1p @ self.shift + b1.float()).contiguous()
            self._sq_w2 = F.pad(w2.float(), (0, 0, 0, CP - Cl)).contiguous()
            self._sq_b2 = F.pad(b2.float(), (0, CP - Cl)).contiguous()
            self._sq_key = key
        L, ctx, st = _lib.lib(), _ctx(z.device), _stream(z.device)
        M = self._sq_w1.shape[0]
        mean = torch.empty((z.N, d.Cin), dtype=torch.float32, device=z.device)
        _lib.check(L.pcv_se_squeeze(ctx, _ptr(z.t), _ptr(mean), z.N, z.H * z.W, d.Cin, _CODE_OF_TORCH[z.dtype], st), ctx)
        mid = torch.empty((z.N, M), dtype=torch.float32, device=z.device)
        gate = torch.empty((z.N, d.Cout), dtype=torch.float32, device=z.device)
        _lib.check(L.pcv_fc_f32(ctx, _ptr(mean), _ptr(self._sq_w1), _ptr(self._sq_b1), _ptr(mid), z.N, d.Cin, M, mid_act, st), ctx)
        _lib.check(L.pcv_fc_f32(ctx, _ptr(mid), _ptr(self._sq_w2), _ptr(self._sq_b2), _ptr(gate), z.N, M, d.Cout, out_act, st), ctx)
        return gate


def _pool_out(n: int, k: int, s: int, p: int, ceil_mode: bool) -> int:
    o = (n + 2 * p - k + (s - 1 if ceil_mode else 0)) // s + 1
    if ceil_mode and (o - 1) * s >= n + p:
        o -= 1
    return o


def channel_slice(x: NHWC, offset: int, count: int) -> NHWC:
    if x.wpitch != x.W or offset < 0 or offset + count > x.C:
        raise RuntimeError("bad channel slice")
    cp = round8(count)
    y = torch.empty((x.N, x.H, x.W, cp), dtype=x.dtype, device=x.device)
    ctx = _ctx(x.device)
    _lib.check(_lib.lib().pcv_channel_slice(ctx, _ptr(x.t), _ptr(y), x.N * x.H * x.W, count, offset, x.cpitch, cp,
                                            _CODE_OF_TORCH[x.dtype], _stream(x.device)), ctx)
    return NHWC(y, x.N, x.H, x.W, count, cpitch=cp)


def channel_concat_into(x: NHWC, buf: torch.Tensor, coff: int):
    if x.wpitch != x.W or x.C % 8 or coff % 8 or tuple(buf.shape[:3]) != (x.N, x.H, x.W) or buf.dtype != x.dtype or \
            coff + x.C > buf.shape[3] or not buf.is_contiguous():
        raise RuntimeError("channel concatenation needs channel counts / offsets that are multiples of 8 and equal maps")
    ctx = _ctx(x.device)
    _lib.check(_lib.lib().pcv_channel_concat(ctx, _ptr(x.t), _ptr(buf), x.N * x.H * x.W, x.C, x.cpitch, int(buf.shape[3]), coff,
                                             _CODE_OF_TORCH[x.dtype], _stream(x.device)), ctx)


def interpolate(x: NHWC, out_size, bilinear: bool, align_corners: bool) -> NHWC:
    if not x.dense:
        raise RuntimeError("interpolation on a padded handle")
    Ho, Wo = int(out_size[0]), int(out_size[1])
    y = torch.empty((x.N, Ho, Wo, x.cpitch), dtype=x.dtype, device=x.device)
    ctx = _ctx(x.device)
    _lib.check(_lib.lib().pcv_interpolate(ctx, _ptr(x.t), _ptr(y), x.N, x.H, x.W, x.cpitch, Ho, Wo, 1 if bilinear else 0,
                                          1 if align_corners else 0, _CODE_OF_TORCH[x.dtype], _stream(x.device)), ctx)
    return NHWC(y, x.N, Ho, Wo, x.C, cpitch=x.cpitch)


def add(a: NHWC, b: NHWC, post_act: int = 0) -> NHWC:
    if a.t.shape != b.t.shape or a.dtype != b.dtype or not a.dense:
        raise RuntimeError("add: operands do not match")
    ones = torch.ones((a.N, a.cpitch), dtype=torch.float32, device=a.device)
    y = torch.empty_like(a.t)
    ctx = _ctx(a.device)
    _lib.check(_lib.lib().pcv_se_scale(ctx, _ptr(a.t), _ptr(ones), _ptr(b.t), _ptr(y), a.N, a.H * a.W, a.cpitch, post_act,
                                       _CODE_OF_TORCH[a.dtype], _stream(a.device)), ctx)
    return NHWC(y, a.N, a.H, a.W, a.C, cpitch=a.cpitch)


def cat_shuffle2(a: NHWC, b: NHWC, half: int) -> NHWC:
    if (a.N, a.H, a.W) != (b.N, b.H, b.W) or a.dtype != b.dtype or a.wpitch != a.W or b.wpitch != b.W or half > a.C or half > b.C:
        raise RuntimeError("cat/shuffle operands do not match")
    cp = round8(2 * half)
    y = torch.empty((a.N, a.H, a.W, cp), dtype=a.dtype, device=a.device)
    ctx = _ctx(a.device)
    _lib.check(_lib.lib().pcv_channel_interleave2(ctx, _ptr(a.t), _ptr(b.t), _ptr(y), a.N * a.H * a.W, half, a.cpitch, b.cpitch,
                                                  cp, _CODE_OF_TORCH[a.dtype], _stream(a.device)), ctx)
    return NHWC(y, a.N, a.H, a.W, 2 * half, cpitch=cp)


def maxpool2d(x: NHWC, k: int, s: int, p: int, ceil_mode: bool = False) -> NHWC:
    if not x.dense:
        raise RuntimeError("max-pool on a padded handle")
    Ho, Wo = _pool_out(x.H, k, s, p, ceil_mode), _pool_out(x.W, k, s, p, ceil_mode)
    if Ho <= 0 or Wo <= 0:
        raise RuntimeError("MaxPool2d({}, {}, {}) output of a {}x{} map would be empty".format(k, s, p, x.H, x.W))
    y = torch.empty((x.N, Ho, Wo, x.cpitch), dtype=x.dtype, device=x.device)
    ctx = _ctx(x.device)
    _lib.check(_lib.lib().pcv_maxpool2d(ctx, _ptr(x.t), _ptr(y), x.N, x.H, x.W, x.cpitch, k, s, p, 1 if ceil_mode else 0,
                                        _CODE_OF_TORCH[x.dtype], _stream(x.device)), ctx)
    return NHWC(y, x.N, Ho, Wo, x.C, cpitch=x.cpitch)


def avgpool2d(x: NHWC, k: int, s: int, out_fp32: bool = False) -> NHWC:
    if not x.dense:
        raise RuntimeError("avg-pool on a padded handle")
    if k > x.H or k > x.W:
        raise RuntimeError("AvgPool2d kernel {} larger than the {}x{} map".format(k, x.H, x.W))
    Ho, Wo = (x.H - k) // s + 1, (x.W - k) // s + 1
# ... 250 lines not shown
```

pytorchcv_amd/models/common/conv.py:

```python

__all__ = ['conv1x1', 'conv3x3', 'depthwise_conv3x3', 'ConvBlock', 'conv1x1_block', 'conv3x3_block', 'conv5x5_block',
           'conv7x7_block', 'dwconv_block', 'dwconv3x3_block', 'dwconv5x5_block', 'DwsConvBlock', 'dwsconv3x3_block', 'BareConv', 'PreConvBlock',
           'pre_conv1x1_block', 'pre_conv3x3_block', 'conv_block_pair', 'conv_block_maxpool', 'mbconv_chain']

import torch.nn as nn
from .activ import lambda_relu, create_activation_layer
from .norm import lambda_batchnorm2d, create_normalization_layer
from ... import engine


class BareConv(nn.Conv2d):
    def forward(self, x, out_fp32: bool = False, act: int = 0):
        if getattr(self, "_pcv_runner", None) is None:
            self._pcv_runner = engine.ConvRunner(self, None)
        return engine.boundary(self, x, lambda a: self._pcv_runner.run(a, act=act, out_fp32=out_fp32))


def conv1x1(in_channels, out_channels, stride=1, groups=1, bias=False):
    return BareConv(in_channels=in_channels, out_channels=out_channels, kernel_size=1, stride=stride, groups=groups, bias=bias)


def conv3x3(in_channels, out_channels, stride=1, padding=1, dilation=1, groups=1, bias=False):
    return BareConv(in_channels=in_channels, out_channels=out_channels, kernel_size=3, stride=stride, padding=padding,
                    dilation=dilation, groups=groups, bias=bias)


def depthwise_conv3x3(channels, stride=1, padding=1, dilation=1, bias=False):
    return BareConv(in_channels=channels, out_channels=channels, kernel_size=3, stride=stride, padding=padding,
                    dilation=dilation, groups=channels, bias=bias)


class ConvBlock(nn.Module):
    def __init__(self, in_channels, out_channels, kernel_size, stride=1, padding=0, dilation=1, groups=1, bias=False,
                 normalization=lambda_batchnorm2d(), activation=lambda_relu()):
        super(ConvBlock, self).__init__()
        self.normalize = (normalization is not None)
        self.activate = (activation is not None)
        self.use_pad = (isinstance(padding, (list, tuple)) and (len(padding) == 4))
        self._pad4 = tuple(int(p) for p in padding) if self.use_pad else None
        self.conv = nn.Conv2d(in_channels=in_channels, out_channels=out_channels, kernel_size=kernel_size, stride=stride,
                              padding=(0 if self.use_pad else padding), dilation=dilation, groups=groups, bias=bias)
        if self.normalize:
            self.bn = create_normalization_layer(normalization=normalization, num_features=out_channels)
            if self.bn is None:
                self.normalize = False
            else:
                assert isinstance(self.bn, nn.Module)
        if self.activate:
            self.activ = create_activation_layer(activation)
            if self.activ is None:
                self.activate = False
            else:
                assert isinstance(self.activ, nn.Module)
        self._pcv_runner = None

    def forward(self, x, residual=None, post_act=None, pad4=None, out=None):
        if self._pcv_runner is None:
            self._pcv_runner = engine.ConvRunner(self.conv, self.bn if self.normalize else None, pad4=self._pad4)
        act = engine.act_code(self.activ) if self.activate else 0
        pact = engine.act_code(post_act)
        return engine.boundary(self, x, lambda a: self._pcv_runner.run(a, act=act, residual=residual, post_act=pact,
                                                                       pad4=pad4, out=out))


def conv_block_maxpool(block, x, pool):
    if isinstance(block, ConvBlock) and isinstance(x, engine.NHWC) and not block.use_pad:
        if block._pcv_runner is None:
            block._pcv_runner = engine.ConvRunner(block.conv, block.bn if block.normalize else None, pad4=block._pad4)
        y = block._pcv_runner.run_maxpool(x, engine.act_code(block.activ) if block.activate else 0, pool.kernel_size,
                                          pool.stride, pool.padding, pool.ceil_mode)
        if y is not None:
            return y
    return pool(block(x))


def conv_block_pair(first, x, residual, post_act, second, id_block=None, x0=None):
    if not (isinstance(first, ConvBlock) and isinstance(second, ConvBlock) and isinstance(x, engine.NHWC)):
        return None
    for blk in (first, second) + ((id_block,) if id_block is not None else ()):
        if not isinstance(blk, ConvBlock):
            return None
        if blk._pcv_runner is None:
            blk._pcv_runner = engine.ConvRunner(blk.conv, blk.bn if blk.normalize else None, pad4=blk._pad4)
    if id_block is not None:
        if id_block.activate or not isinstance(x0, engine.NHWC):
            return None
        return first._pcv_runner.run_pair_idconv(x, x0, id_block._pcv_runner, engine.act_code(first.activ) if first.activate else 0,
                                                 engine.act_code(post_act), second._pcv_runner,
                                                 engine.act_code(second.activ) if second.activate else 0)
    return first._pcv_runner.run_pair(x, residual, engine.act_code(first.activ) if first.activate else 0,
                                      engine.act_code(post_act), second._pcv_runner,
                                      engine.act_code(second.activ) if second.activate else 0)


def mbconv_chain(exp_block, dw_block, proj_block, x, residual=None, post_act=None):
    blocks = [b for b in (exp_block, dw_block, proj_block) if b is not None]
    if not isinstance(x, engine.NHWC) or not all(isinstance(b, ConvBlock) for b in blocks):
        return None
    for blk in blocks:
        if blk._pcv_runner is None:
            blk._pcv_runner = engine.ConvRunner(blk.conv, blk.bn if blk.normalize else None, pad4=blk._pad4)

    def code(blk):
        return engine.act_code(blk.activ) if blk.activate else 0
    return engine.mbconv_fused(exp_block._pcv_runner if exp_block is not None else None,
                               code(exp_block) if exp_block is not None else 0, dw_block._pcv_runner, code(dw_block),
                               proj_block._pcv_runner, code(proj_block), x, residual, engine.act_code(post_act))


def conv1x1_block(padding=0, **kwargs):
    return ConvBlock(kernel_size=1, padding=padding, **kwargs)


def conv3x3_block(padding=1, **kwargs):
    return ConvBlock(kernel_size=3, padding=padding, **kwargs)


def conv5x5_block(padding=2, **kwargs):
    return ConvBlock(kernel_size=5, padding=padding, **kwargs)


def conv7x7_block(padding=3, **kwargs):
    return ConvBlock(kernel_size=7, padding=padding, **kwargs)


def dwconv_block(out_channels, padding=1, **kwargs):
    return ConvBlock(out_channels=out_channels, padding=padding, groups=out_channels, **kwargs)


def dwconv3x3_block(padding=1, **kwargs):
    return dwconv_block(kernel_size=3, padding=padding, **kwargs)


def dwconv5x5_block(padding=2, **kwargs):
    return dwconv_block(kernel_size=5, padding=padding, **kwargs)


class DwsConvBlock(nn.Module):
    def __init__(self, in_channels, out_channels, kernel_size, stride=1, padding=0, dilation=1, bias=False,
                 dw_normalization=lambda_batchnorm2d(), pw_normalization=lambda_batchnorm2d(), dw_activation=lambda_relu(),
                 pw_activation=lambda_relu()):
        super(DwsConvBlock, self).__init__()
        self.dw_conv = dwconv_block(in_channels=in_channels, out_channels=in_channels, kernel_size=kernel_size, stride=stride,
                                    padding=padding, dilation=dilation, bias=bias, normalization=dw_normalization,
                                    activation=dw_activation)
        self.pw_conv = conv1x1_block(in_channels=in_channels, out_channels=out_channels, bias=bias,
                                     normalization=pw_normalization, activation=pw_activation)

    def _run(self, a):
        y = mbconv_chain(None, self.dw_conv, self.pw_conv, a)
        return y if y is not None else self.pw_conv(self.dw_conv(a))

    def forward(self, x):
        return engine.boundary(self, x, self._run)


def dwsconv3x3_block(padding=1, **kwargs):
    return DwsConvBlock(kernel_size=3, padding=padding, **kwargs)


class PreConvBlock(nn.Module):
    def __init__(self, in_channels, out_channels, kernel_size, stride, padding, dilation=1, bias=False,
                 normalization=lambda_batchnorm2d(), activation=lambda_relu(), return_preact=False):
        super(PreConvBlock, self).__init__()
        self.normalize = (normalization is not None)
        self.activate = (activation is not None)
        self.return_preact = return_preact
        if self.normalize:
            self.bn = create_normalization_layer(normalization=normalization, num_features=in_channels)
            if self.bn is None:
                self.normalize = False
            else:
                assert isinstance(self.bn, nn.BatchNorm2d)
        if self.activate:
            self.activ = create_activation_layer(activation)
            if self.activ is None:
                self.activate = False
            else:
                assert isinstance(self.activ, nn.Module)
        self.conv = nn.Conv2d(in_channels=in_channels, out_channels=out_channels, kernel_size=kernel_size, stride=stride,
                              padding=padding, dilation=dilation, bias=bias)
        self._pcv_pre = None
        self._pcv_runners = {}

    def act_code(self):
        return engine.act_code(self.activ) if self.activate else 0

    def preact(self, a):
        if not self.normalize:
            raise NotImplementedError("PreConvBlock without normalization on the MI355X path")
        if self._pcv_pre is None:
            self._pcv_pre = engine.BnActRunner(self.bn)
        return self._pcv_pre.run(a, self.act_code())

    def conv_then(self, a, next_block=None, residual=None, out=None, se=None):
        key = id(next_block)
        if key not in self._pcv_runners:
            bn = next_block.bn if (next_block is not None and next_block.normalize) else None
            self._pcv_runners[key] = engine.ConvRunner(self.conv, bn)
        act = next_block.act_code() if next_block is not None else 0
        runner = self._pcv_runners[key]
        gate = None
        c = self.conv
        if se is not None and next_block is None and out is None and engine.FUSE_UNITS and tuple(c.kernel_size) == (1, 1) and \
                tuple(c.stride) == (1, 1) and tuple(c.padding) == (0, 0) and a.dense:
            w1, b1, w2, b2 = se._mlp()
            gate = runner.squeezed_excite(a, w1, b1, w2, b2, engine.act_code(se.activ), engine.act_code(se.sigmoid))
        elif se is not None:
            return se(runner.run(a, act=act, out=out), residual=residual)
        return runner.run(a, act=act, residual=residual, out=out, gate=gate)

    def _run(self, a):
        pre = self.preact(a) if (self.normalize or self.activate) else a
        y = self.conv_then(pre)
        return (y, pre) if self.return_preact else y

    def forward(self, x):
        return engine.boundary(self, x, self._run)


def pre_conv1x1_block(stride=1, padding=0, **kwargs):
    return PreConvBlock(kernel_size=1, stride=stride, padding=padding, **kwargs)


def pre_conv3x3_block(stride=1, padding=1, **kwargs):
    return PreConvBlock(kernel_size=3, stride=stride, padding=padding, **kwargs)
```

pytorchcv_amd/models/resnet.py:

```python

__all__ = ['ResNet', 'resnet10', 'resnet12', 'resnet14', 'resnetbc14b', 'resnet16', 'resnet18', 'resnet26', 'resnetbc26b',
           'resnet34', 'resnetbc38b', 'resnet50', 'resnet50b', 'resnet101', 'resnet101b', 'resnet152', 'resnet152b',
           'ResBlock', 'ResBottleneck', 'ResUnit', 'ResStage', 'ResInitBlock', 'get_resnet']

import torch.nn as nn
from .common.activ import lambda_relu
from .common.norm import lambda_batchnorm2d
from .common.conv import conv1x1_block, conv3x3_block, conv7x7_block, conv_block_pair, conv_block_maxpool
from ._tail import MaxPool2dNHWC, AvgPool2dNHWC, LinearHead, run_net, maybe_load_pretrained, init_conv_params, DEFAULT_ROOT
from .. import engine


class ResBlock(nn.Module):
    def __init__(self, in_channels, out_channels, stride, bias=False, normalization=lambda_batchnorm2d(),
                 activation=lambda_relu(), final_activation=None):
        super(ResBlock, self).__init__()
        self.conv1 = conv3x3_block(in_channels=in_channels, out_channels=out_channels, stride=stride, bias=bias,
                                   normalization=normalization, activation=activation)
        self.conv2 = conv3x3_block(in_channels=out_channels, out_channels=out_channels, bias=bias,
                                   normalization=normalization, activation=final_activation)

    def forward(self, x, residual=None, post_act=None):
        return engine.boundary(self, x, lambda a: self.conv2(self.conv1(a), residual=residual, post_act=post_act))


class ResBottleneck(nn.Module):
    def __init__(self, in_channels, out_channels, stride, padding=1, dilation=1, bias=False,
                 normalization=lambda_batchnorm2d(), conv1_stride=False, bottleneck_factor=4, activation=lambda_relu(),
                 final_activation=None):
        super(ResBottleneck, self).__init__()
        mid_channels = out_channels // bottleneck_factor
        self.conv1 = conv1x1_block(in_channels=in_channels, out_channels=mid_channels, stride=(stride if conv1_stride else 1),
                                   bias=bias, normalization=normalization, activation=activation)
        self.conv2 = conv3x3_block(in_channels=mid_channels, out_channels=mid_channels,
                                   stride=(1 if conv1_stride else stride), padding=padding, dilation=dilation, bias=bias,
                                   normalization=normalization, activation=activation)
        self.conv3 = conv1x1_block(in_channels=mid_channels, out_channels=out_channels, bias=bias,
                                   normalization=normalization, activation=final_activation)

    def forward(self, x, residual=None, post_act=None):
        return engine.boundary(self, x, lambda a: self.conv3(self.conv2(self.conv1(a)), residual=residual, post_act=post_act))


class ResUnit(nn.Module):
    def __init__(self, in_channels, out_channels, stride=1, padding=1, dilation=1, bias=False,
                 normalization=lambda_batchnorm2d(), bottleneck=True, conv1_stride=False, activation=lambda_relu(),
                 final_body_activation=None, final_activation=lambda_relu()):
        super(ResUnit, self).__init__()
        self.resize_identity = (in_channels != out_channels) or (stride != 1)
        if bottleneck:
            self.body = ResBottleneck(in_channels=in_channels, out_channels=out_channels, stride=stride, padding=padding,
                                      dilation=dilation, bias=bias, normalization=normalization, conv1_stride=conv1_stride,
                                      activation=activation, final_activation=final_body_activation)
        else:
            self.body = ResBlock(in_channels=in_channels, out_channels=out_channels, stride=stride, bias=bias,
                                 normalization=normalization, activation=activation, final_activation=final_body_activation)
        if self.resize_identity:
            self.identity_conv = conv1x1_block(in_channels=in_channels, out_channels=out_channels, stride=stride, bias=bias,
                                               normalization=normalization, activation=None)
        self.activ = final_activation()

    def _run(self, a):
        identity = self.identity_conv(a) if self.resize_identity else a
        return self.body(a, residual=identity, post_act=self.activ)

    def run_chained(self, a, conv1_out=None, next_unit=None):
        body = self.body
        y = body.conv2(conv1_out if conv1_out is not None else body.conv1(a))
        if next_unit is not None and self.resize_identity:
            pair = conv_block_pair(body.conv3, y, None, self.activ, next_unit.body.conv1, id_block=self.identity_conv, x0=a)
            if pair is not None:
                return pair
        identity = self.identity_conv(a) if self.resize_identity else a
        if next_unit is not None:
            pair = conv_block_pair(body.conv3, y, identity, self.activ, next_unit.body.conv1)
            if pair is not None:
                return pair
        return body.conv3(y, residual=identity, post_act=self.activ), None

    def forward(self, x):
        return engine.boundary(self, x, self._run)


class ResStage(nn.Sequential):
    def forward(self, x):
        units = list(self.children())
        chainable = all((isinstance(u, ResUnit) and isinstance(u.body, ResBottleneck)) or getattr(u, "pcv_chainable", False) for u in units)
        if not isinstance(x, engine.NHWC) or not chainable:
            return super(ResStage, self).forward(x)
        conv1_out = None
        for i, unit in enumerate(units):
            x, conv1_out = unit.run_chained(x, conv1_out, units[i + 1] if i + 1 < len(units) else None)
        return x


class ResInitBlock(nn.Module):
    def __init__(self, in_channels, out_channels, normalization=lambda_batchnorm2d()):
        super(ResInitBlock, self).__init__()
        self.conv = conv7x7_block(in_channels=in_channels, out_channels=out_channels, stride=2, normalization=normalization)
        self.pool = MaxPool2dNHWC(kernel_size=3, stride=2, padding=1)

    def forward(self, x):
        return engine.boundary(self, x, lambda a: conv_block_maxpool(self.conv, a, self.pool), stem=True)


class ResNet(nn.Module):
    def __init__(self, channels, init_block_channels, bottleneck, conv1_stride, in_channels=3, in_size=(224, 224),
                 num_classes=1000):
        super(ResNet, self).__init__()
        self.in_size = in_size
        self.num_classes = num_classes
        self.features = nn.Sequential()
        self.features.add_module("init_block", ResInitBlock(in_channels=in_channels, out_channels=init_block_channels))
        in_channels = init_block_channels
        for i, channels_per_stage in enumerate(channels):
            stage = ResStage()
            for j, out_channels in enumerate(channels_per_stage):
                stride = 2 if (j == 0) and (i != 0) else 1
                stage.add_module("unit{}".format(j + 1), ResUnit(in_channels=in_channels, out_channels=out_channels,
                                                                 stride=stride, bottleneck=bottleneck,
                                                                 conv1_stride=conv1_stride))
                in_channels = out_channels
            self.features.add_module("stage{}".format(i + 1), stage)
        self.features.add_module("final_pool", AvgPool2dNHWC(kernel_size=7, stride=1, fp32_out=True))
        self.output = LinearHead(in_features=in_channels, out_features=num_classes)
        init_conv_params(self)

    def forward(self, x):
        return run_net(self, x, self.output)


_LAYERS = {10: [1, 1, 1, 1], 12: [2, 1, 1, 1], 16: [2, 2, 2, 1], 18: [2, 2, 2, 2], 34: [3, 4, 6, 3], 50: [3, 4, 6, 3],
           101: [3, 4, 23, 3], 152: [3, 8, 36, 3], 200: [3, 24, 36, 3]}


def resnet_layers(blocks, bottleneck, what="ResNet"):
    if blocks == 14:
        layers = [1, 1, 1, 1] if bottleneck else [2, 2, 1, 1]
    elif blocks == 26:
        layers = [2, 2, 2, 2] if bottleneck else [3, 3, 3, 3]
    elif blocks == 38 and bottleneck:
        layers = [3, 3, 3, 3]
    elif blocks in _LAYERS:
        layers = _LAYERS[blocks]
    else:
        raise ValueError("Unsupported {} with number of blocks: {}".format(what, blocks))
    assert (sum(layers) * (3 if bottleneck else 2) + 2 == blocks)
    return layers


def get_resnet(blocks, bottleneck=None, conv1_stride=True, width_scale=1.0, model_name=None, pretrained=False,
               root=DEFAULT_ROOT, **kwargs):
    if bottleneck is None:
        bottleneck = (blocks >= 50)
    layers = resnet_layers(blocks, bottleneck)
    init_block_channels = 64
    widths = [64, 128, 256, 512]
    if bottleneck:
        widths = [w * 4 for w in widths]
    channels = [[w] * n for (w, n) in zip(widths, layers)]
    if width_scale != 1.0:
        last = (len(channels) - 1, len(channels[-1]) - 1)
        channels = [[int(c * width_scale) if (i, j) != last else c for j, c in enumerate(ci)] for i, ci in enumerate(channels)]
        init_block_channels = int(init_block_channels * width_scale)
    net = ResNet(channels=channels, init_block_channels=init_block_channels, bottleneck=bottleneck, conv1_stride=conv1_stride,
                 **kwargs)
    return maybe_load_pretrained(net, model_name, pretrained, root)


def resnet10(**kwargs):
    return get_resnet(blocks=10, model_name="resnet10", **kwargs)


def resnet12(**kwargs):
    return get_resnet(blocks=12, model_name="resnet12", **kwargs)


def resnet14(**kwargs):
    return get_resnet(blocks=14, model_name="resnet14", **kwargs)


def resnetbc14b(**kwargs):
    return get_resnet(blocks=14, bottleneck=True, conv1_stride=False, model_name="resnetbc14b", **kwargs)


def resnet16(**kwargs):
    return get_resnet(blocks=16, model_name="resnet16", **kwargs)


def resnet18(**kwargs):
    return get_resnet(blocks=18, model_name="resnet18", **kwargs)


def resnet26(**kwargs):
    return get_resnet(blocks=26, bottleneck=False, model_name="resnet26", **kwargs)


def resnetbc26b(**kwargs):
    return get_resnet(blocks=26, bottleneck=True, conv1_stride=False, model_name="resnetbc26b", **kwargs)


def resnet34(**kwargs):
    return get_resnet(blocks=34, model_name="resnet34", **kwargs)


def resnetbc38b(**kwargs):
    return get_resnet(blocks=38, bottleneck=True, conv1_stride=False, model_name="resnetbc38b", **kwargs)


def resnet50(**kwargs):
    return get_resnet(blocks=50, model_name="resnet50", **kwargs)


def resnet50b(**kwargs):
    return get_resnet(blocks=50, conv1_stride=False, model_name="resnet50b", **kwargs)


def resnet101(**kwargs):
    return get_resnet(blocks=101, model_name="resnet101", **kwargs)


def resnet101b(**kwargs):
    return get_resnet(blocks=101, conv1_stride=False, model_name="resnet101b", **kwargs)


def resnet152(**kwargs):
    return get_resnet(blocks=152, model_name="resnet152", **kwargs)


def resnet152b(**kwargs):
    return get_resnet(blocks=152, conv1_stride=False, model_name="resnet152b", **kwargs)
```

Measured before the change: 93150 images/sec.

## Rematerialize residual skip chains inside fused conv1x1 pair kernel for ResNet stages

```diff
diff --git a/include/pcv_amd.h b/include/pcv_amd.h
--- a/include/pcv_amd.h
+++ b/include/pcv_amd.h
@@ -155,6 +155,21 @@
                                   const void* x, const void* packed1, const float* scale1, const float* shift1, void* y1,
                                   const void* packed2, const float* scale2, const float* shift2, void* y2, void* stream);
 
+typedef struct pcv_pair_link {
+    const pcv_conv_desc* d;
+    const void* x;
+    const void* packed;
+    const float* scale;
+    const float* shift;
+} pcv_pair_link;
+int pcv_conv1x1_pair_chain_supported(const pcv_conv_desc* d_id, const pcv_conv_desc* const* d_links, int n_links,
+                                     const pcv_conv_desc* d1, const pcv_conv_desc* d2, int store_y1);
+int pcv_conv1x1_pair_chain_fused(pcv_ctx* ctx, const pcv_conv_desc* d_id, const void* x0, const void* packed_id, const float* scale_id,
+                                 const float* shift_id, const void* residual, const pcv_pair_link* links, int n_links,
+                                 const pcv_conv_desc* d1, const void* x, const void* packed1, const float* scale1, const float* shift1,
+                                 void* y1, const pcv_conv_desc* d2, const void* packed2, const float* scale2, const float* shift2,
+                                 void* y2, void* stream);
+
 int pcv_mbconv_supported(const pcv_conv_desc* d_exp, const pcv_conv_desc* d_dw, const pcv_conv_desc* d_proj);
 int pcv_mbconv_fused(pcv_ctx* ctx, const pcv_conv_desc* d_exp, const pcv_conv_desc* d_dw, const pcv_conv_desc* d_proj,
                      const void* x, const void* packed_exp, const float* scale_e, const float* shift_e,
diff --git a/pytorchcv_amd/_lib.py b/pytorchcv_amd/_lib.py
--- a/pytorchcv_amd/_lib.py
+++ b/pytorchcv_amd/_lib.py
@@ -32,6 +32,10 @@
     def __init__(self, *args, **kw):
         super(ConvDesc, self).__init__(*args, **kw)
         self.struct_size = ctypes.sizeof(ConvDesc)
+
+
+class PairLink(ctypes.Structure):
+    _fields_ = [("d", ctypes.POINTER(ConvDesc)), ("x", _VP), ("packed", _VP), ("scale", _VP), ("shift", _VP)]
 
 
 _SIGS = {
@@ -86,6 +90,11 @@
     "pcv_conv1x1_pair_idconv_supported": (_I, [ctypes.POINTER(ConvDesc), ctypes.POINTER(ConvDesc), ctypes.POINTER(ConvDesc)]),
     "pcv_conv1x1_pair_idconv_fused": (_I, [_VP, ctypes.POINTER(ConvDesc), ctypes.POINTER(ConvDesc), ctypes.POINTER(ConvDesc),
                                            _VP, _VP, _VP, _VP, _VP, _VP, _VP, _VP, _VP, _VP, _VP, _VP, _VP, _VP]),
+    "pcv_conv1x1_pair_chain_supported": (_I, [ctypes.POINTER(ConvDesc), ctypes.POINTER(ctypes.POINTER(ConvDesc)), _I,
+                                              ctypes.POINTER(ConvDesc), ctypes.POINTER(ConvDesc), _I]),
+    "pcv_conv1x1_pair_chain_fused": (_I, [_VP, ctypes.POINTER(ConvDesc), _VP, _VP, _VP, _VP, _VP, ctypes.POINTER(PairLink), _I,
+                                          ctypes.POINTER(ConvDesc), _VP, _VP, _VP, _VP, _VP, ctypes.POINTER(ConvDesc), _VP, _VP, _VP,
+                                          _VP, _VP]),
     "pcv_mbconv_supported": (_I, [ctypes.POINTER(ConvDesc), ctypes.POINTER(ConvDesc), ctypes.POINTER(ConvDesc)]),
     "pcv_mbconv_fused": (_I, [_VP, ctypes.POINTER(ConvDesc), ctypes.POINTER(ConvDesc), ctypes.POINTER(ConvDesc), _VP, _VP, _VP, _VP,
                               _VP, _VP, _VP, _VP, _VP, _VP, _VP, _VP, _VP]),
diff --git a/pytorchcv_amd/csrc/pair1x1.hpp b/pytorchcv_amd/csrc/pair1x1.hpp
--- a/pytorchcv_amd/csrc/pair1x1.hpp
+++ b/pytorchcv_amd/csrc/pair1x1.hpp
@@ -24,6 +24,13 @@
     uint32_t x0_bytes, wid_bytes;
     const float* gate;
     FastDiv div_hw;
+    struct Link {
+        const void* x;
+        const void* w;
+        const float* scale;
+        const float* shift;
+        int act, post;
+    } link[2];
     uint32_t* ovf;
 };
 
@@ -31,17 +38,21 @@
     asm volatile("s_waitcnt vmcnt(%0)" ::"n"(N) : "memory");
 }
 
-template <int DT, int PB, bool IDC = false, bool GATE = false>
+template <int DT, int PB, bool IDC = false, bool GATE = false, int CH = 0, bool ST1 = true, bool G2 = true>
 __global__ __launch_bounds__(256, PB == 4 ? 1 : 2) void pair1x1_kernel(const PairParams p) {
 #if defined(__HIP_DEVICE_COMPILE__)
     constexpr int K1 = 64, C1 = 256, C2 = 64, P = 16 * PB;
     constexpr int NXQ = PB / 2;
     constexpr int NIP = PB / 2;
     constexpr int XB = P * K1 * 2;
+    constexpr bool PHASED = CH > 0 || !ST1 || !G2;
+    static_assert(!PHASED || (PB == 2 && !GATE), "skip chain: 32-pixel tiles, ungated");
+    static_assert(ST1 || G2, "a launch that neither stores y1 nor runs the second convolution has no output");
     typedef typename Mma<DT>::frag frag;
     extern __shared__ __attribute__((aligned(16))) char smem[];
-    char* const x0ring = smem + 3 * XB;
-    char* const red = smem + (IDC ? 6 : 3) * XB;
+    char* const lring = smem + 3 * XB;
+    char* const x0ring = smem + 3 * (1 + CH) * XB;
+    char* const red = smem + 3 * (1 + CH + (IDC ? 1 : 0)) * XB;
 
     const int tid = threadIdx.x;
     const int lane = tid & 63;
@@ -60,6 +71,8 @@
     const __amdgpu_buffer_rsrc_t w2rsrc = __builtin_amdgcn_make_buffer_rsrc(const_cast<void*>(p.w2), 0, p.w2_bytes, 0x00020000);
     const __amdgpu_buffer_rsrc_t x0rsrc = __builtin_amdgcn_make_buffer_rsrc(const_cast<void*>(IDC ? p.x0 : p.x), 0, IDC ? p.x0_bytes : p.x_bytes, 0x00020000);
     const __amdgpu_buffer_rsrc_t widrsrc = __builtin_amdgcn_make_buffer_rsrc(const_cast<void*>(IDC ? p.wid : p.w1), 0, IDC ? p.wid_bytes : p.w1_bytes, 0x00020000);
+    const __amdgpu_buffer_rsrc_t lx0rsrc = __builtin_amdgcn_make_buffer_rsrc(const_cast<void*>(CH > 0 ? p.link[0].x : p.x), 0, p.x_bytes, 0x00020000);
+    const __amdgpu_buffer_rsrc_t lx1rsrc = __builtin_amdgcn_make_buffer_rsrc(const_cast<void*>(CH > 1 ? p.link[1].x : p.x), 0, p.x_bytes, 0x00020000);
 
     frag a1[4][2];
     frag a2[4][2];
@@ -69,10 +82,10 @@
         for (int ks = 0; ks < 2; ++ks) {
             const u32x4 v1 = __builtin_amdgcn_raw_buffer_load_b128(
                 w1rsrc, (uint32_t)(((64 * wave + 16 * i + fr) * K1 + ks * 32 + 8 * fq) * 2), 0, 0);
-            const u32x4 v2 = __builtin_amdgcn_raw_buffer_load_b128(
-                w2rsrc, (uint32_t)(((16 * i + fr) * C1 + (2 * wave + ks) * 32 + 8 * fq) * 2), 0, 0);
             a1[i][ks] = __builtin_bit_cast(frag, v1);
-            a2[i][ks] = __builtin_bit_cast(frag, v2);
+            if constexpr (G2)
+                a2[i][ks] = __builtin_bit_cast(frag, __builtin_amdgcn_raw_buffer_load_b128(
+                    w2rsrc, (uint32_t)(((16 * i + fr) * C1 + (2 * wave + ks) * 32 + 8 * fq) * 2), 0, 0));
         }
     frag aid[IDC ? 4 : 1][2];
     if constexpr (IDC) {
@@ -83,15 +96,35 @@
                 aid[i][ks] = __builtin_bit_cast(frag, __builtin_amdgcn_raw_buffer_load_b128(
                     widrsrc, (uint32_t)(((64 * wave + 16 * i + fr) * K1 + ks * 32 + 8 * fq) * 2), 0, 0));
     }
+    frag al[CH > 0 ? CH : 1][4][2];
+#pragma unroll
+    for (int k = 0; k < CH; ++k) {
+        const __amdgpu_buffer_rsrc_t lwrsrc = __builtin_amdgcn_make_buffer_rsrc(const_cast<void*>(p.link[k].w), 0, p.w1_bytes, 0x00020000);
+#pragma unroll
+        for (int i = 0; i < 4; ++i)
+#pragma unroll
+            for (int ks = 0; ks < 2; ++ks)
+                al[k][i][ks] = __builtin_bit_cast(frag, __builtin_amdgcn_raw_buffer_load_b128(
+                    lwrsrc, (uint32_t)(((64 * wave + 16 * i + fr) * K1 + ks * 32 + 8 * fq) * 2), 0, 0));
+    }
     float sc1[2][8], sf1[2][8], sc2[NIP][8], sf2[NIP][8];
-    float* const tscid = reinterpret_cast<float*>(red + 16 * 1024 * PB);
+    float* const tscid = reinterpret_cast<float*>(red + (G2 ? 16 * 1024 * PB : 0));
     float* const tsfid = tscid + C1;
     float* const tsc1 = tsfid + C1;
     float* const tsf1 = tsc1 + C1;
-    if constexpr (IDC) {
+    float* const tlink = tsf1 + C1;
+    float* const tc2 = tlink + 2 * C1 * CH;
+    if constexpr (IDC || PHASED) {
         for (int i = tid; i < C1; i += 256) {
-            tscid[i] = p.scale_id[i]; tsfid[i] = p.shift_id[i];
+            if constexpr (IDC) { tscid[i] = p.scale_id[i]; tsfid[i] = p.shift_id[i]; }
             tsc1[i] = p.scale1[i]; tsf1[i] = p.shift1[i];
+#pragma unroll
+            for (int k = 0; k < CH; ++k) {
+                tlink[2 * C1 * k + i] = p.link[k].scale[i];
+                tlink[2 * C1 * k + C1 + i] = p.link[k].shift[i];
+            }
+            if constexpr (PHASED && G2)
+                if (i < C2) { tc2[i] = p.scale2[i]; tc2[C2 + i] = p.shift2[i]; }
         }
         __syncthreads();
     }
@@ -100,16 +133,16 @@
 #pragma unroll
         for (int e = 0; e < 8; ++e) {
             const int c1 = 64 * wave + 32 * ip + 8 * fq + e;
-            sc1[ip][e] = IDC ? 0.f : p.scale1[c1];
-            sf1[ip][e] = IDC ? 0.f : p.shift1[c1];
+            sc1[ip][e] = (IDC || PHASED) ? 0.f : p.scale1[c1];
+            sf1[ip][e] = (IDC || PHASED) ? 0.f : p.shift1[c1];
         }
 #pragma unroll
     for (int k = 0; k < NIP; ++k)
 #pragma unroll
         for (int e = 0; e < 8; ++e) {
             const int c2 = 32 * ((wave / PB) * NIP + k) + 8 * fq + e;
-            sc2[k][e] = p.scale2[c2];
-            sf2[k][e] = p.shift2[c2];
+            sc2[k][e] = PHASED ? 0.f : p.scale2[c2];
+            sf2[k][e] = PHASED ? 0.f : p.shift2[c2];
         }
     const ActClamp act1 = make_act(p.act1), post1 = make_act(p.post1), act2 = make_act(p.act2);
 
@@ -126,6 +159,10 @@
             const long pix = (long)t * P + xrow[q];
             const uint32_t off = (t < p.nTiles && pix < p.M) ? (uint32_t)((pix * K1 + xchunk[q] * 8) * 2) : 0x80000000u;
             __builtin_amdgcn_raw_ptr_buffer_load_lds(xrsrc, PCV_LDS(smem + slot * XB + (NXQ * wave + q) * 1024), 16, off, 0, 0, 0);
+            if constexpr (CH > 0)
+                __builtin_amdgcn_raw_ptr_buffer_load_lds(lx0rsrc, PCV_LDS(lring + slot * XB + (NXQ * wave + q) * 1024), 16, off, 0, 0, 0);
+            if constexpr (CH > 1)
+                __builtin_amdgcn_raw_ptr_buffer_load_lds(lx1rsrc, PCV_LDS(lring + (3 + slot) * XB + (NXQ * wave + q) * 1024), 16, off, 0, 0, 0);
             if constexpr (IDC)
                 __builtin_amdgcn_raw_ptr_buffer_load_lds(x0rsrc, PCV_LDS(x0ring + slot * XB + (NXQ * wave + q) * 1024), 16, off, 0, 0, 0);
         }
@@ -154,11 +191,11 @@
     issue_x(tile, 0);
     issue_x(tile + tstride, 1);
     load_res(tile, resr[0]);
-    load_res(tile + tstride, resr[1]);
+    if constexpr (!PHASED) load_res(tile + tstride, resr[1]);
     pair_wait_vmcnt<0>();
     bool first = true;
 
-    F16Guard<DT> guard;
+    F16Guard<DT, PHASED> guard;
     auto step = [&](auto KC) -> bool {
         constexpr int slot = decltype(KC)::value;
         constexpr int slot2 = (slot + 2) % 3;
@@ -325,10 +362,150 @@
         tile += tstride;
         return tile < p.nTiles;
     };
+
+    auto conv_half = [&](const char* xb, const frag (&w)[4][2], int ip, f32x4 (&acc)[2][PB]) {
+#pragma unroll
+        for (int h = 0; h < 2; ++h)
+#pragma unroll
+            for (int j = 0; j < PB; ++j) acc[h][j] = (f32x4){0.f, 0.f, 0.f, 0.f};
+#pragma unroll
+        for (int ks = 0; ks < 2; ++ks) {
+            frag b[PB];
+#pragma unroll
+            for (int j = 0; j < PB; ++j) b[j] = *reinterpret_cast<const frag*>(xb + xfrag[j][ks]);
+#pragma unroll
+            for (int h = 0; h < 2; ++h)
+#pragma unroll
+                for (int j = 0; j < PB; ++j) acc[h][j] = Mma<DT>::run(w[2 * ip + h][ks], b[j], acc[h][j]);
+        }
+    };
+    auto epi_half = [&](auto SKIP, const f32x4 (&acc)[2][PB], const float* tsc, int ip, const ActClamp& act, const ActClamp& post,
+                        F16Guard<DT, PHASED>& guard, const u32x4 (&skip)[PB], u32x4 (&out)[PB]) {
+        const int ch = 64 * wave + 32 * ip + 8 * fq;
+        const f32x4 s0 = *reinterpret_cast<const f32x4*>(tsc + ch), s1 = *reinterpret_cast<const f32x4*>(tsc + ch + 4);
+        const f32x4 h0 = *reinterpret_cast<const f32x4*>(tsc + C1 + ch), h1 = *reinterpret_cast<const f32x4*>(tsc + C1 + ch + 4);
+#pragma unroll
+        for (int j = 0; j < PB; ++j) {
+            float v[8], r8[8];
+#pragma unroll
+            for (int e = 0; e < 4; ++e) {
+                v[e] = acc[0][j][e] * s0[e] + h0[e];
+                v[4 + e] = acc[1][j][e] * s1[e] + h1[e];
+            }
+            if constexpr (decltype(SKIP)::value) {
+                apply_act8(v, act);
+#pragma unroll
+                for (int e = 0; e < 4; ++e) unpack2<DT>(skip[j][e], r8[2 * e], r8[2 * e + 1]);
+#pragma unroll
+                for (int e = 0; e < 8; ++e) v[e] += r8[e];
+                apply_act8(v, post);
+            }
+            guard.see(v);
+#pragma unroll
+            for (int e = 0; e < 4; ++e) out[j][e] = pack2<DT>(v[2 * e], v[2 * e + 1]);
+        }
+    };
+    auto step_phased = [&](auto KC) -> bool {
+        constexpr int slot = decltype(KC)::value;
+        constexpr int slot2 = (slot + 2) % 3;
+        u32x4 (&resc)[2][PB] = resr[slot];
+        if (!first) pair_wait_vmcnt<NXQ * (1 + CH + (IDC ? 1 : 0)) + (IDC ? 0 : 2 * PB) + (ST1 ? 2 * PB : 0) + (G2 ? NIP : 0)>();
+        first = false;
+        __syncthreads();
+        f32x4 acc[2][PB];
+        u32x4 o[2][PB];
+#pragma unroll
+        for (int ip = 0; ip < 2; ++ip) {
+            if constexpr (IDC) {
+                conv_half(x0ring + slot * XB, aid, ip, acc);
+                epi_half(std::false_type{}, acc, tscid, ip, act1, act1, guard, resc[ip], resc[ip]);
+                __builtin_amdgcn_sched_barrier(0);
+            }
+#pragma unroll
+            for (int k = 0; k < CH; ++k) {
+                conv_half(lring + (3 * k + slot) * XB, al[k], ip, acc);
+                epi_half(std::true_type{}, acc, tlink + 2 * C1 * k, ip, make_act(p.link[k].act), make_act(p.link[k].post), guard, resc[ip], resc[ip]);
+                __builtin_amdgcn_sched_barrier(0);
+            }
+            conv_half(smem + slot * XB, a1, ip, acc);
+            epi_half(std::true_type{}, acc, tsc1, ip, act1, post1, guard, resc[ip], o[ip]);
+            if constexpr (ST1) {
+#pragma unroll
+                for (int j = 0; j < PB; ++j) __builtin_amdgcn_raw_buffer_store_b128(o[ip][j], y1rsrc, off_c1(tile, ip, j), 0, 0);
+            }
+            __builtin_amdgcn_sched_barrier(0);
+        }
+        issue_x(tile + 2 * tstride, slot2);
+        load_res(tile + tstride, resr[(slot + 1) % 3]);
+        if constexpr (G2) {
+            __builtin_amdgcn_sched_barrier(0);
+            f32x4 acc2[4][PB];
+#pragma unroll
+            for (int i = 0; i < 4; ++i)
+#pragma unroll
+                for (int j = 0; j < PB; ++j) acc2[i][j] = (f32x4){0.f, 0.f, 0.f, 0.f};
+#pragma unroll
+            for (int ip = 0; ip < 2; ++ip)
+#pragma unroll
+                for (int i = 0; i < 4; ++i)
+#pragma unroll
+                    for (int j = 0; j < PB; ++j)
+                        acc2[i][j] = Mma<DT>::run(a2[i][ip], __builtin_bit_cast(frag, o[ip][j]), acc2[i][j]);
+#pragma unroll
+            for (int i = 0; i < 4; ++i)
+#pragma unroll
+                for (int j = 0; j < PB; ++j)
+                    *reinterpret_cast<f32x4*>(red + (((wave * 4 + i) * PB + j) * 64 + lane) * 16) = acc2[i][j];
+            __syncthreads();
+            const int jz = wave % PB, ip0 = (wave / PB) * NIP;
+            f32x4 z[2 * NIP];
+#pragma unroll
+            for (int k = 0; k < 2 * NIP; ++k) {
+                const int i = 2 * ip0 + k;
+                z[k] = *reinterpret_cast<const f32x4*>(red + (((0 * 4 + i) * PB + jz) * 64 + lane) * 16);
+#pragma unroll
+                for (int v = 1; v < 4; ++v) {
+                    const f32x4 t = *reinterpret_cast<const f32x4*>(red + (((v * 4 + i) * PB + jz) * 64 + lane) * 16);
+                    z[k] += t;
+                }
+            }
+            __syncthreads();
+#pragma unroll
+            for (int k = 0; k < NIP; ++k) {
+                const int ip = ip0 + k;
+                const float* t2 = tc2 + 32 * ip + 8 * fq;
+                const f32x4 s0 = *reinterpret_cast<const f32x4*>(t2), s1 = *reinterpret_cast<const f32x4*>(t2 + 4);
+                const f32x4 h0 = *reinterpret_cast<const f32x4*>(t2 + C2), h1 = *reinterpret_cast<const f32x4*>(t2 + C2 + 4);
+                float v[8];
+#pragma unroll
+                for (int e = 0; e < 4; ++e) {
+                    v[e] = z[2 * k][e] * s0[e] + h0[e];
+                    v[4 + e] = z[2 * k + 1][e] * s1[e] + h1[e];
+                }
+                apply_act8(v, act2);
+                guard.see(v);
+                u32x4 q;
+#pragma unroll
+                for (int e = 0; e < 4; ++e) q[e] = pack2<DT>(v[2 * e], v[2 * e + 1]);
+                const long pix = (long)tile * P + 16 * jz + fr;
+                const uint32_t off = pix < p.M ? (uint32_t)((pix * C2 + 32 * ip + 8 * fq) * 2) : 0x80000000u;
+                __builtin_amdgcn_raw_buffer_store_b128(q, y2rsrc, off, 0, 0);
+            }
+        }
+        guard.commit(p.ovf);
+        tile += tstride;
+        return tile < p.nTiles;
+    };
     while (true) {
-        if (!step(std::integral_constant<int, 0>{})) break;
-        if (!step(std::integral_constant<int, 1>{})) break;
-        if (!step(std::integral_constant<int, 2>{})) break;
+        if constexpr (PHASED) {
+            if (!step_phased(std::integral_constant<int, 0>{})) break;
+            if (!step_phased(std::integral_constant<int, 1>{})) break;
+            if (!step_phased(std::integral_constant<int, 2>{})) break;
+        } else {
+            if (!step(std::integral_constant<int, 0>{})) break;
+            if (!step(std::integral_constant<int, 1>{})) break;
+            if (!step(std::integral_constant<int, 2>{})) break;
+        }
     }
 #endif
 }
diff --git a/pytorchcv_amd/csrc/pcv_api.hip b/pytorchcv_amd/csrc/pcv_api.hip
--- a/pytorchcv_amd/csrc/pcv_api.hip
+++ b/pytorchcv_amd/csrc/pcv_api.hip
@@ -105,6 +105,7 @@
     int stem_bpc[2] = {1, 1};
     int pair_bpc[2] = {1, 1};
     int pair_idc_bpc = 1;
+    int pair_chain_bpc[2][5] = {{1, 1, 1, 1, 1}, {1, 1, 1, 1, 1}};
     int wpair_bpc[4] = {1, 1, 1, 1};
 };
 
@@ -498,8 +499,23 @@
     {kernel_of(pair1x1_kernel<DT, 4>, 256, pair_lds(4)), kernel_of(pair1x1_kernel<DT, 2>, 256, pair_lds(2)),                  \
      kernel_of(pair1x1_kernel<DT, 2, false, true>, 256, pair_lds(2)), kernel_of(pair1x1_kernel<DT, 2, true>, 256, pair_lds(2, true))}
 static const Kernel kPair[2][4] = {PAIR_ROW(PCV_BF16), PAIR_ROW(PCV_F16)};
+enum PairChainForm { CHAIN_0_NOSTORE = 0, CHAIN_1 = 1, CHAIN_1_NOSTORE = 2, CHAIN_1_TAIL = 3, CHAIN_2_TAIL = 4 };
+static int pair_chain_lds(bool idc, int links, bool conv2) {
+    return 3 * (1 + links + (idc ? 1 : 0)) * 4096 + (conv2 ? 32 * 1024 : 0) + 4096 + 2048 * links + 512;
+}
+#define PAIR_CHAIN_ROW(DT, IDC)                                                                                                \
+    {kernel_of(pair1x1_kernel<DT, 2, IDC, false, 0, false, true>, 256, pair_chain_lds(IDC, 0, true)),                           \
+     kernel_of(pair1x1_kernel<DT, 2, IDC, false, 1, true, true>, 256, pair_chain_lds(IDC, 1, true)),                            \
+     kernel_of(pair1x1_kernel<DT, 2, IDC, false, 1, false, true>, 256, pair_chain_lds(IDC, 1, true)),                           \
+     kernel_of(pair1x1_kernel<DT, 2, IDC, false, 1, true, false>, 256, pair_chain_lds(IDC, 1, false)),                          \
+     kernel_of(pair1x1_kernel<DT, 2, IDC, false, 2, true, false>, 256, pair_chain_lds(IDC, 2, false))}
+static const Kernel kPairChain[2][2][5] = {{PAIR_CHAIN_ROW(PCV_BF16, false), PAIR_CHAIN_ROW(PCV_BF16, true)},
+                                           {PAIR_CHAIN_ROW(PCV_F16, false), PAIR_CHAIN_ROW(PCV_F16, true)}};
 static int g_wpair_mask = 3;
 static int g_mbw_wide = 1;
+static const int kPairRematDefault = 2;
+static int g_pair_remat = -1;
+static int pair_remat_level() { return g_pair_remat < 0 ? kPairRematDefault : g_pair_remat; }
 struct WPairLaunch { Kernel k; int tileP; bool gate_in_lds; };
 template <int CM, int C1> static WPairLaunch wpair_launch_for(int dt, bool gated) {
     typedef WPairCfg<CM, C1> G;
@@ -647,6 +663,11 @@
         on(kPair[0][form]);
         on(kPair[1][form], form == PAIR_GATED ? nullptr : form == PAIR_IDCONV ? &ctx->pair_idc_bpc : &ctx->pair_bpc[form]);
     }
+    for (int idc = 0; idc < 2; ++idc)
+        for (int form = 0; form < 5; ++form) {
+            on(kPairChain[0][idc][form]);
+            on(kPairChain[1][idc][form], &ctx->pair_chain_bpc[idc][form]);
+        }
     for (int cfg = 0; cfg < 4; ++cfg)
         for (int gated = 0; gated < 2; ++gated) {
             on(wpair_launch(cfg, PCV_BF16, gated != 0).k);
@@ -797,6 +818,7 @@
         }
     if (k == "mbw_wide") g_mbw_wide = value;
     else if (k == "wpair") g_wpair_mask = value;
+    else if (k == "pair_remat") g_pair_remat = value;
     else if (k == "dbg") {
 #ifdef PCV_DBG_FLAGS
         ctx->dbg_flags = value;
@@ -2043,6 +2065,104 @@
     return launch(ctx, kPair[d1->dtype == PCV_BF16 ? 0 : 1][PAIR_IDCONV], grid, (hipStream_t)stream, p);
 }
 
+static const char* pair_first_unsupported(const pcv_conv_desc& a) {
+    if (desc_stale(a)) return kStaleDesc;
+    if (!plain_1x1(a)) return "the convolution must be plain 1x1 stride 1";
+    if (a.dtype != PCV_BF16 && a.dtype != PCV_F16) return "16-bit storage only";
+    if (!a.has_residual) return "the convolution must carry the residual";
+    if ((long)a.N * a.H * a.W * a.Cout * 2 >= (1L << 31)) return kTensorTooLarge;
+    return nullptr;
+}
+static const char* pair_chain_unsupported(const pcv_conv_desc* di, const pcv_conv_desc* const* dl, int n_links, const pcv_conv_desc& a,
+                                          const pcv_conv_desc* b, bool store_y1, int* form_out) {
+    if (const char* why = b ? pair_unsupported(a, *b) : pair_first_unsupported(a)) return why;
+    if (a.Cin != 64 || a.Cout != 256) return "skip chain: only the 64 -> 256 (-> 64) shapes are instantiated";
+    if (n_links < 0 || n_links > 2 || (n_links > 0 && !dl)) return "skip chain: at most two links";
+    int form = -1;
+    if (n_links == 0 && !store_y1 && b) form = CHAIN_0_NOSTORE;
+    else if (n_links == 1 && b) form = store_y1 ? CHAIN_1 : CHAIN_1_NOSTORE;
+    else if (n_links >= 1 && !b && store_y1) form = n_links == 1 ? CHAIN_1_TAIL : CHAIN_2_TAIL;
+    if (form < 0) return "skip chain: this combination of links and outputs is not instantiated";
+    const int level = (form == CHAIN_0_NOSTORE || form == CHAIN_1) ? 1 : 2;
+    if (pair_remat_level() < level) return "skip chain: switched off (pcv_set_tuning \"pair_remat\")";
+    for (int k = 0; k < n_links; ++k) {
+        if (!dl[k]) return "skip chain: NULL link descriptor";
+        const pcv_conv_desc& l = *dl[k];
+        if (const char* why = pair_first_unsupported(l)) return why;
+        if (l.dtype != a.dtype || l.N != a.N || l.H != a.H || l.W != a.W || l.Cin != 64 || l.Cout != 256) return "skip chain: link shapes do not match";
+    }
+    if (di) {
+        if (desc_stale(*di)) return kStaleDesc;
+        if (!plain_1x1(*di) || di->dtype != a.dtype) return "identity convolution must be a plain 1x1 stride 1 of the same dtype";
+        if (di->N != a.N || di->H != a.H || di->W != a.W || di->Cin != 64 || di->Cout != a.Cout) return "identity convolution shapes do not match";
+        if (di->act != PCV_ACT_NONE || di->has_residual || di->post_act != PCV_ACT_NONE) return "identity convolution must have no activation";
+    }
+    if (form_out) *form_out = form;
+    return nullptr;
+}
+
+int pcv_conv1x1_pair_chain_supported(const pcv_conv_desc* d_id, const pcv_conv_desc* const* d_links, int n_links,
+                                     const pcv_conv_desc* d1, const pcv_conv_desc* d2, int store_y1) {
+    return (d1 && pair_chain_unsupported(d_id, d_links, n_links, *d1, d2, store_y1 != 0, nullptr) == nullptr) ? 1 : 0;
+}
+
+int pcv_conv1x1_pair_chain_fused(pcv_ctx* ctx, const pcv_conv_desc* d_id, const void* x0, const void* packed_id, const float* scale_id,
+                                 const float* shift_id, const void* residual, const pcv_pair_link* links, int n_links,
+                                 const pcv_conv_desc* d1, const void* x, const void* packed1, const float* scale1, const float* shift1,
+                                 void* y1, const pcv_conv_desc* d2, const void* packed2, const float* scale2, const float* shift2,
+                                 void* y2, void* stream) {
+    if (!ctx) return PCV_ERR_INVALID;
+    DeviceGuard device_guard(ctx->device);
+    static const char* const fn = "pcv_conv1x1_pair_chain_fused: ";
+    if (!d1 || !x || !packed1 || !scale1 || !shift1 || n_links < 0 || n_links > 2 || (n_links > 0 && !links))
+        return fail(ctx, PCV_ERR_INVALID, std::string(fn) + "NULL argument");
+    if (d_id ? (!x0 || !packed_id || !scale_id || !shift_id) : !residual) return fail(ctx, PCV_ERR_INVALID, std::string(fn) + "the skip tensor needs either the identity convolution or `residual`");
+    if (d2 && (!packed2 || !scale2 || !shift2 || !y2)) return fail(ctx, PCV_ERR_INVALID, std::string(fn) + "NULL argument of the second convolution");
+    const pcv_conv_desc* dl[2] = {nullptr, nullptr};
+    for (int k = 0; k < n_links; ++k) {
+        if (!links[k].d || !links[k].x || !links[k].packed || !links[k].scale || !links[k].shift)
+            return fail(ctx, PCV_ERR_INVALID, std::string(fn) + "NULL link argument");
+        dl[k] = links[k].d;
+    }
+    int form = -1;
+    if (const char* why = pair_chain_unsupported(d_id, dl, n_links, *d1, d2, y1 != nullptr, &form)) return fail(ctx, PCV_ERR_INVALID, std::string(fn) + why);
+    if (!aligned16(x) || !aligned16(packed1) || !aligned16(y1) || !aligned16(x0) || !aligned16(packed_id) || !aligned16(residual) ||
+        !aligned16(packed2) || !aligned16(y2))
+        return fail(ctx, PCV_ERR_INVALID, std::string(fn) + "pointers must be 16-byte aligned");
+    PairParams p;
+    std::memset(&p, 0, sizeof(p));
+    const long M = (long)d1->N * d1->H * d1->W;
+    auto weights = [&](const pcv_conv_desc& d, const void* packed, int rows, int kpad, const void** w) -> const char* {
+        ConvPlan P;
+        if (const char* why = plan_conv(d, P, false)) return why;
+        if (P.wrows != rows || P.Kpad != kpad || P.ngb != 1) return "unexpected packed layout";
+        *w = static_cast<const char*>(packed) + P.ktab_bytes;
+        return nullptr;
+    };
+    const char* why = weights(*d1, packed1, 256, 64, &p.w1);
+    if (!why && d2) why = weights(*d2, packed2, 64, 256, &p.w2);
+    if (!why && d_id) why = weights(*d_id, packed_id, 256, 64, &p.wid);
+    for (int k = 0; k < n_links && !why; ++k) {
+        if (!aligned16(links[k].x) || !aligned16(links[k].packed)) why = "pointers must be 16-byte aligned";
+        else why = weights(*links[k].d, links[k].packed, 256, 64, &p.link[k].w);
+        p.link[k].x = links[k].x; p.link[k].scale = links[k].scale; p.link[k].shift = links[k].shift;
+        p.link[k].act = links[k].d->act; p.link[k].post = links[k].d->post_act;
+    }
+    if (why) return fail(ctx, PCV_ERR_INVALID, std::string(fn) + why);
+    p.x = x; p.res = d_id ? nullptr : residual; p.y1 = y1; p.y2 = d2 ? y2 : nullptr; p.x0 = x0; p.ovf = ctx->ovf;
+    p.scale1 = scale1; p.shift1 = shift1; p.scale2 = scale2; p.shift2 = shift2; p.scale_id = scale_id; p.shift_id = shift_id;
+    p.x_bytes = p.x0_bytes = (uint32_t)(M * 64 * 2);
+    p.res_bytes = d_id ? 0 : (uint32_t)(M * 256 * 2);
+    p.y1_bytes = y1 ? (uint32_t)(M * 256 * 2) : 0;
+    p.y2_bytes = d2 ? (uint32_t)(M * 64 * 2) : 0;
+    p.w1_bytes = p.wid_bytes = 256 * 64 * 2; p.w2_bytes = 64 * 256 * 2;
+    p.M = (int)M; p.nTiles = (int)((M + 31) / 32);
+    p.act1 = d1->act; p.post1 = d1->post_act; p.act2 = d2 ? d2->act : PCV_ACT_NONE;
+    const int idc = d_id ? 1 : 0;
+    const unsigned grid = (unsigned)std::min<long>(p.nTiles, (long)block_slots(ctx, ctx->pair_chain_bpc[idc][form]));
+    return launch(ctx, kPairChain[d1->dtype == PCV_BF16 ? 0 : 1][idc][form], grid, (hipStream_t)stream, p);
+}
+
 int pcv_channel_slice(pcv_ctx* ctx, const void* x, void* y, long rows, int C, int offset, int x_cpitch, int y_cpitch, int dtype,
                       void* stream) {
     if (!ctx) return PCV_ERR_INVALID;
diff --git a/pytorchcv_amd/engine.py b/pytorchcv_amd/engine.py
--- a/pytorchcv_amd/engine.py
+++ b/pytorchcv_amd/engine.py
@@ -104,10 +104,11 @@
 
 
 class _ShapeOnly(object):
-    __slots__ = ("N", "H", "W", "C", "dtype", "wpitch", "cpitch")
-
-    def __init__(self, N, H, W, C, dtype):
+    __slots__ = ("N", "H", "W", "C", "dtype", "wpitch", "cpitch", "device")
+
+    def __init__(self, N, H, W, C, dtype, device=None):
         self.N, self.H, self.W, self.C, self.dtype, self.wpitch, self.cpitch = N, H, W, C, dtype, W, round8(C)
+        self.device = device
 
 
 def _stream(device) -> ctypes.c_void_p:
@@ -448,6 +449,58 @@
                                                    _ptr(self.scale), _ptr(self.shift), _ptr(t1), _ptr(nxt.packed), _ptr(nxt.scale),
                                                    _ptr(nxt.shift), _ptr(t2), st), ctx)
         return y1, NHWC(t2, x.N, x.H, x.W, nxt.conv.out_channels, cpitch=d2.Cout)
+
+    def run_pair_chain(self, x, act: int, post_act: int, idr, x0, residual, links, nxt, nxt_act: int, store: bool, probe=False):
+        runners = [self] + [r for r in (idr, nxt) if r is not None] + [l[0] for l in links]
+        if not FUSE_UNITS or any(r.depthwise or r.pad4 is not None for r in runners):
+            return False if probe else None
+        if any(r.bn is not None and r.bn.training for r in runners):
+            raise RuntimeError("pytorchcv_amd is an inference path: call net.eval() first (BatchNorm is folded)")
+        shape = (x.N, x.H, x.W)
+        skip = x0 if idr is not None else residual
+        if skip is None or not skip.dense or skip.dtype != x.dtype or (skip.N, skip.H, skip.W) != shape:
+            return False if probe else None
+        c = self.conv
+        L = _lib.lib()
+        di = idr.desc(x0, 0, 0, False) if idr is not None else None
+        d1 = self.desc(x, act, post_act, True)
+        d2 = nxt.desc(_ShapeOnly(x.N, x.H, x.W, c.out_channels, x.dtype), nxt_act, 0, False) if nxt is not None else None
+        dls = [r.desc(lx if lx is not None else x, a, pa, True) for (r, lx, a, pa) in links]
+        dl_ptrs = (ctypes.POINTER(ConvDesc) * max(len(dls), 1))(*[ctypes.pointer(d) for d in dls])
+        ok = L.pcv_conv1x1_pair_chain_supported(ctypes.byref(di) if di is not None else None, dl_ptrs, len(dls), ctypes.byref(d1),
+                                                ctypes.byref(d2) if d2 is not None else None, 1 if store else 0)
+        if probe:
+            return bool(ok)
+        if not ok:
+            return None
+        if idr is None and tuple(residual.t.shape) != (x.N, x.H, x.W, d1.Cout):
+            raise RuntimeError("residual shape/dtype mismatch")
+        for (_, lx, _, _) in links:
+            if not lx.dense or lx.dtype != x.dtype or (lx.N, lx.H, lx.W, lx.cpitch) != shape + (x.cpitch,):
+                raise RuntimeError("skip chain: a link's input does not match the unit's")
+        ctx, st = _ctx(x.device), _stream(x.device)
+        t1 = torch.empty((x.N, x.H, x.W, d1.Cout), dtype=x.dtype, device=x.device) if store else None
+        t2 = torch.empty((x.N, x.H, x.W, d2.Cout), dtype=x.dtype, device=x.device) if nxt is not None else None
+        if idr is not None:
+            idr.prepare(x0, di)
+        self.prepare(x, d1)
+        if nxt is not None:
+            nxt.prepare(_ShapeOnly(x.N, x.H, x.W, c.out_channels, x.dtype, x.device), d2)
+        larr = (_lib.PairLink * max(len(links), 1))()
+        for k, ((r, lx, _, _), d) in enumerate(zip(links, dls)):
+            r.prepare(lx, d)
+            larr[k].d, larr[k].x, larr[k].packed = ctypes.pointer(d), _ptr(lx.t), _ptr(r.packed)
+            larr[k].scale, larr[k].shift = _ptr(r.scale), _ptr(r.shift)
+        _lib.check(L.pcv_conv1x1_pair_chain_fused(
+            ctx, ctypes.byref(di) if di is not None else None, _ptr(x0.t) if idr is not None else None,
+            _ptr(idr.packed) if idr is not None else None, _ptr(idr.scale) if idr is not None else None,
+            _ptr(idr.shift) if idr is not None else None, _ptr(residual.t) if idr is None else None, larr, len(links),
+            ctypes.byref(d1), _ptr(x.t), _ptr(self.packed), _ptr(self.scale), _ptr(self.shift), _ptr(t1),
+            ctypes.byref(d2) if d2 is not None else None, _ptr(nxt.packed) if nxt is not None else None,
+            _ptr(nxt.scale) if nxt is not None else None, _ptr(nxt.shift) if nxt is not None else None, _ptr(t2), st), ctx)
+        y1 = NHWC(t1, x.N, x.H, x.W, c.out_channels, cpitch=d1.Cout) if store else None
+        y2 = NHWC(t2, x.N, x.H, x.W, nxt.conv.out_channels, cpitch=d2.Cout) if nxt is not None else None
+        return y1, y2
 
     def _launch(self, x: NHWC, d: ConvDesc, residual, out=None, gate=None):
         c = self.conv
diff --git a/pytorchcv_amd/models/common/conv.py b/pytorchcv_amd/models/common/conv.py
--- a/pytorchcv_amd/models/common/conv.py
+++ b/pytorchcv_amd/models/common/conv.py
@@ -1,7 +1,7 @@
 
 __all__ = ['conv1x1', 'conv3x3', 'depthwise_conv3x3', 'ConvBlock', 'conv1x1_block', 'conv3x3_block', 'conv5x5_block',
            'conv7x7_block', 'dwconv_block', 'dwconv3x3_block', 'dwconv5x5_block', 'DwsConvBlock', 'dwsconv3x3_block', 'BareConv', 'PreConvBlock',
-           'pre_conv1x1_block', 'pre_conv3x3_block', 'conv_block_pair', 'conv_block_maxpool', 'mbconv_chain']
+           'pre_conv1x1_block', 'pre_conv3x3_block', 'conv_block_pair', 'conv_block_pair_chain', 'conv_block_maxpool', 'mbconv_chain']
 
 import torch.nn as nn
 from .activ import lambda_relu, create_activation_layer
@@ -93,6 +93,22 @@
                                       engine.act_code(second.activ) if second.activate else 0)
 
 
+def conv_block_pair_chain(first, x, post_act, second, links, id_block=None, x0=None, residual=None, store=True, probe=False):
+    blocks = [first] + [b for b in (second, id_block) if b is not None] + [l[0] for l in links]
+    if not all(isinstance(b, ConvBlock) for b in blocks) or (id_block is not None and id_block.activate):
+        return False if probe else None
+    for blk in blocks:
+        if blk._pcv_runner is None:
+            blk._pcv_runner = engine.ConvRunner(blk.conv, blk.bn if blk.normalize else None, pad4=blk._pad4)
+
+    def code(blk):
+        return engine.act_code(blk.activ) if blk.activate else 0
+    return first._pcv_runner.run_pair_chain(
+        x, code(first), engine.act_code(post_act), id_block._pcv_runner if id_block is not None else None, x0, residual,
+        [(b._pcv_runner, lx, code(b), engine.act_code(pa)) for (b, lx, pa) in links],
+        second._pcv_runner if second is not None else None, code(second) if second is not None else 0, store, probe=probe)
+
+
 def mbconv_chain(exp_block, dw_block, proj_block, x, residual=None, post_act=None):
     blocks = [b for b in (exp_block, dw_block, proj_block) if b is not None]
     if not isinstance(x, engine.NHWC) or not all(isinstance(b, ConvBlock) for b in blocks):
diff --git a/pytorchcv_amd/models/resnet.py b/pytorchcv_amd/models/resnet.py
--- a/pytorchcv_amd/models/resnet.py
+++ b/pytorchcv_amd/models/resnet.py
@@ -1,12 +1,13 @@
 
 __all__ = ['ResNet', 'resnet10', 'resnet12', 'resnet14', 'resnetbc14b', 'resnet16', 'resnet18', 'resnet26', 'resnetbc26b',
            'resnet34', 'resnetbc38b', 'resnet50', 'resnet50b', 'resnet101', 'resnet101b', 'resnet152', 'resnet152b',
-           'ResBlock', 'ResBottleneck', 'ResUnit', 'ResStage', 'ResInitBlock', 'get_resnet']
-
+           'ResBlock', 'ResBottleneck', 'ResUnit', 'SkipChain', 'ResStage', 'ResInitBlock', 'get_resnet']
+
+import torch
 import torch.nn as nn
 from .common.activ import lambda_relu
 from .common.norm import lambda_batchnorm2d
-from .common.conv import conv1x1_block, conv3x3_block, conv7x7_block, conv_block_pair, conv_block_maxpool
+from .common.conv import conv1x1_block, conv3x3_block, conv7x7_block, conv_block_pair, conv_block_pair_chain, conv_block_maxpool
 from ._tail import MaxPool2dNHWC, AvgPool2dNHWC, LinearHead, run_net, maybe_load_pretrained, init_conv_params, DEFAULT_ROOT
 from .. import engine
 
@@ -64,9 +65,9 @@
         identity = self.identity_conv(a) if self.resize_identity else a
         return self.body(a, residual=identity, post_act=self.activ)
 
-    def run_chained(self, a, conv1_out=None, next_unit=None):
+    def run_chained(self, a, conv1_out=None, next_unit=None, conv2_done=False):
         body = self.body
-        y = body.conv2(conv1_out if conv1_out is not None else body.conv1(a))
+        y = conv1_out if conv2_done else body.conv2(conv1_out if conv1_out is not None else body.conv1(a))
         if next_unit is not None and self.resize_identity:
             pair = conv_block_pair(body.conv3, y, None, self.activ, next_unit.body.conv1, id_block=self.identity_conv, x0=a)
             if pair is not None:
@@ -78,8 +79,56 @@
                 return pair
         return body.conv3(y, residual=identity, post_act=self.activ), None
 
+    def run_remat(self, a, conv1_out, rest, chain):
+        body = self.body
+        nxt = rest[0] if rest else None
+        c3 = body.conv3.conv
+        if chain is None and (nxt is None or (c3.in_channels, c3.out_channels) != (64, 256)):
+            return self.run_chained(a, conv1_out, nxt) + (None,)
+        y = body.conv2(conv1_out if conv1_out is not None else body.conv1(a))
+        if chain is None:
+            chain = SkipChain(self.identity_conv if self.resize_identity else None, a)
+        here = chain.extended(body.conv3, y, self.activ)
+        skip = dict(id_block=chain.id_block, x0=chain.x if chain.id_block is not None else None,
+                    residual=chain.x if chain.id_block is None else None)
+        if nxt is not None and here.consumable(rest, engine._ShapeOnly(y.N, y.H, y.W, y.C, y.dtype)):
+            pair = conv_block_pair_chain(body.conv3, y, self.activ, nxt.body.conv1, chain.links, store=False, **skip)
+            if pair is not None:
+                return None, pair[1], here
+        if chain.links:
+            pair = conv_block_pair_chain(body.conv3, y, self.activ, nxt.body.conv1 if nxt is not None else None, chain.links,
+                                         store=True, **skip)
+            if pair is None:
+                raise RuntimeError("skip chain: the unit in front left its output to a launch that is not covered")
+            return pair[0], pair[1], None
+        pair = self.run_chained(a, y, nxt, conv2_done=True)
+        return pair + (None,)
+
     def forward(self, x):
         return engine.boundary(self, x, self._run)
+
+
+class SkipChain(object):
+    __slots__ = ("id_block", "x", "links")
+
+    def __init__(self, id_block, x, links=()):
+        self.id_block, self.x, self.links = id_block, x, list(links)
+
+    def extended(self, block, x, post_act):
+        return SkipChain(self.id_block, self.x, self.links + [(block, x, post_act)])
+
+    def consumable(self, rest, shape):
+        unit, after = rest[0], rest[1:]
+        if unit.resize_identity or not isinstance(unit.body, ResBottleneck):
+            return False
+        links = [(b, None, pa) for (b, _, pa) in self.links]
+        kw = dict(links=links, id_block=self.id_block, x0=self.x if self.id_block is not None else None,
+                  residual=self.x if self.id_block is None else None, probe=True)
+        second = after[0].body.conv1 if after else None
+        if conv_block_pair_chain(unit.body.conv3, shape, unit.activ, second, store=True, **kw):
+            return True
+        return bool(after) and conv_block_pair_chain(unit.body.conv3, shape, unit.activ, second, store=False, **kw) and \
+            self.extended(unit.body.conv3, None, unit.activ).consumable(after, shape)
 
 
 class ResStage(nn.Sequential):
@@ -89,6 +138,11 @@
         if not isinstance(x, engine.NHWC) or not chainable:
             return super(ResStage, self).forward(x)
         conv1_out = None
+        if all(type(u) is ResUnit and isinstance(u.body, ResBottleneck) for u in units) and x.dense and x.dtype != torch.float32:
+            chain = None
+            for i, unit in enumerate(units):
+                x, conv1_out, chain = unit.run_remat(x, conv1_out, units[i + 1:], chain)
+            return x
         for i, unit in enumerate(units):
             x, conv1_out = unit.run_chained(x, conv1_out, units[i + 1] if i + 1 < len(units) else None)
         return x
```

Result: slower. 85240 images/sec (-8.5%).
